# NealLiufighting/hpmpc

Hardware: AMD Instinct MI355X
Metric: Riccati factorisations/sec + IP iters/sec, fp64, N=100 nx=12 nu=4 batch=1024 (higher is better)
Workload: dtype f64

## Files before the change

### hpmpc_amd/build.py

```python
from __future__ import annotations

import os
import subprocess

ROOT = os.path.dirname(os.path.dirname(os.path.abspath(__file__)))
CSRC = os.path.join(ROOT, "hpmpc_amd", "csrc")
LIBDIR = os.path.join(ROOT, "hpmpc_amd", "lib")
HIPCC = os.environ.get("HIPCC", "/opt/rocm/bin/hipcc")
ARCH = os.environ.get("HPMPC_ARCH", "gfx950")
SOURCES = ["hpmpc_kernels.hip", "hk_wide.hip", "hk_wide_ipm.hip", "hk_soft.hip", "hk_soft_ipm.hip", "hk_ocp.hip", "hk_kkt.hip", "hpmpc_capi.cpp",
           "hpmpc_capi_queue.cpp", "hpmpc_capi_dropin.cpp", "hpmpc_capi_soft.cpp", "hpmpc_capi_soft_batch.cpp",
           "hpmpc_capi_wide.cpp", "hpmpc_capi_wide_ipm.cpp", "hpmpc_capi_iface.cpp", "hpmpc_capi_mpc.cpp",
           "hpmpc_capi_ocp.cpp", "hpmpc_capi_kkt.cpp"]
HEADERS = ["hpmpc_api.h", "hk_ipm_body.h", "hk_prims.h", "hk_riccati.h", "hk_ipm.h", "hk_mw.h", "hpmpc_kargs.h", "hk_wide_args.h", "hk_wide_core.h", "hk_wide_host.h", "hk_soft_args.h", "hk_soft_body.h", "hk_launch_guard.h", "hk_launch.h", "hk_host.h", "hk_plan.h", "hk_ocp_args.h", "hk_kkt_args.h", "hk_kkt_body.h"]
KFLAGS = ["-mllvm", "-amdgpu-mfma-vgpr-form"] + os.environ.get("HK_EXTRA_FLAGS", "").split()
SRC_FLAGS = {"hpmpc_kernels.hip": ["-mllvm", "-amdgpu-sched-strategy=max-memory-clause"],
             "hk_kkt.hip": ["-mllvm", "-amdgpu-sched-strategy=max-memory-clause"]}


EXPORTS = os.path.join(CSRC, "exports.map")


def _newer(out, deps):
    if not os.path.exists(out):
# ... 11 lines not shown
            text = open(path).read()
        except OSError:
            continue
        for name in re.findall(r'^\s*#\s*include\s+"([^"]+)"', text, re.M):
            for cand in (os.path.join(os.path.dirname(path), name), os.path.join(CSRC, name),
                         os.path.join(ROOT, "include", os.path.basename(name))):
                if os.path.exists(cand) and cand not in seen:
                    seen.add(cand)
                    todo.append(cand)
                    break
    return sorted(seen | {h for h in hdrs_all if os.path.basename(h) == "hpmpc_mi355x.h"})


def build_hip(force: bool = False, verbose: bool = False, variant: str | None = None, extra=(), sources=()) -> str:
    os.makedirs(LIBDIR, exist_ok=True)
    objdir = os.path.join(ROOT, "build", "obj" if variant is None else f"obj_{variant}")
    os.makedirs(objdir, exist_ok=True)
    out = os.path.join(LIBDIR, "libhpmpc_mi355x.so")
    if variant is not None:
        os.makedirs(os.path.join(LIBDIR, "ab"), exist_ok=True)
        out = os.path.join(LIBDIR, "ab", f"lib{variant}.so")
    hdrs_all = [os.path.join(CSRC, h) for h in HEADERS] + [os.path.join(ROOT, "include", "hpmpc_mi355x.h")]
    common = [HIPCC, f"--offload-arch={ARCH}", "-O3", "-std=c++17", "-fPIC", "-fvisibility=hidden", "-Wall",
              "-Wno-unused-function"] + KFLAGS + list(extra)
    objs, procs = [], []
    for src in SOURCES + list(sources):
        obj = os.path.join(objdir, src + ".o")
        objs.append(obj)
        if force or not _newer(obj, [os.path.join(CSRC, src)] + _deps(src, hdrs_all)):
            cmd = common + SRC_FLAGS.get(src, []) + ["-c", os.path.join(CSRC, src), "-o", obj]
            if verbose:
                print(" ".join(cmd), flush=True)
            procs.append((src, subprocess.Popen(cmd)))
    for src, pr in procs:
        if pr.wait() != 0:
            raise subprocess.CalledProcessError(pr.returncode, src)
    if procs or force or not _newer(out, objs + [EXPORTS]):
        cmd = [HIPCC, f"--offload-arch={ARCH}", "-shared", "-fPIC", f"-Wl,--version-script={EXPORTS}"] + objs + \
              ["-o", out]
        if verbose:
            print(" ".join(cmd), flush=True)
        subprocess.run(cmd, check=True)
    return out


def build_stamps(verbose: bool = False, force: bool = False) -> str:
    out = build_hip(force=force, verbose=verbose, variant="stamps", extra=["-DHK_STAMPS"])
    dst = os.path.join(LIBDIR, "libhpmpc_mi355x_stamps.so")
    if not _newer(dst, [out]):
        import shutil

        shutil.copy2(out, dst)
    return dst


def build_ric2(verbose: bool = False, force: bool = False) -> str:
    return build_hip(force=force, verbose=verbose, variant="ric2", extra=["-DHK_RIC2"], sources=["hk_ric2.hip"])


def build_calib(verbose: bool = False) -> str:
    os.makedirs(LIBDIR, exist_ok=True)
    out = os.path.join(LIBDIR, "libhbm_calib.so")
    src = os.path.join(ROOT, "tools", "hbm_calib.hip")
    if _newer(out, [src, os.path.join(CSRC, "hk_prims.h")]):
        return out
    cmd = [HIPCC, f"--offload-arch={ARCH}", "-O3", "-std=c++17", "-fPIC", "-shared", src, "-o", out]
    if verbose:
        print(" ".join(cmd), flush=True)
    subprocess.run(cmd, check=True)
    return out


def build_oracle(force: bool = False) -> None:
    odir = os.path.join(ROOT, "oracle")
    targets = ["oracle", "oracle_fma"]
    if os.path.isdir(os.environ.get("HPMPC_REF", "/root/reference")):
        targets += ["ref", "ref_avx"]
    subprocess.run(["make", "-s", "-C", odir] + (["-B"] if force else []) + targets, check=True)
    if "ref" in targets:
        subprocess.run(["make", "-s", "-C", os.path.join(ROOT, "tools", "relink"), "drivers"], check=True)


def build_all(force: bool = False, verbose: bool = False) -> None:
    build_hip(force=force, verbose=verbose)
    build_stamps(verbose=verbose, force=force)
    build_ric2(verbose=verbose, force=force)
    build_calib(verbose=verbose)
    build_oracle(force=force)


if __name__ == "__main__":
    build_all(force=True, verbose=True)
```

### hpmpc_amd/csrc/hk_ipm.h

```cpp
#pragma once
#include "hk_riccati.h"

namespace hk {

struct BoxTab {
    const signed char* tileslot;
    const signed char* slotvar;
};

#define HK_FOR_BOX(io, KV, ...)                                                       \
    for (int j4_ = 0; j4_ <= (io).N; j4_ += 4) {                                       \
        const int KV = j4_ + (lane_id() >> 4);                                         \
        const int slot = lane_id() & 15;                                               \
        if (KV <= (io).N) {                                                            \
            const int nb_ = (io).st[KV].nb, pnb_ = (io).st[KV].pnb;                    \
            if (slot < nb_) {                                                          \
                const int lo = KV * V32 + slot, up = KV * V32 + pnb_ + slot;           \
                (void)lo; (void)up;                                                    \
                __VA_ARGS__                                                            \
            }                                                                          \
        }                                                                              \
    }

#define HK_FOR_GEN(io, KV, ...)                                                       \
    for (int j4_ = 0; j4_ <= (io).N; j4_ += 4) {                                       \
        const int KV = j4_ + (lane_id() >> 4);                                         \
        const int gl_ = lane_id() & 15;                                                \
        if (KV <= (io).N) {                                                            \
            const int ng_ = (io).st[KV].ng, pnb_ = (io).st[KV].pnb;                    \
            if (gl_ < ng_) {                                                           \
                const int png_ = (ng_ + 3) & ~3;                                       \
                const int lo = KV * V32 + 2 * pnb_ + gl_, up = lo + png_;               \
                const int s16 = KV * V16 + pnb_ + gl_;                                 \
                (void)lo; (void)up; (void)s16;                                         \
                __VA_ARGS__                                                            \
            }                                                                          \
        }                                                                              \
    }

struct QuadLane {
    int lo, up;
    bool ok;
    bool box;
};

__device__ __forceinline__ QuadLane quad_lane(const RicIO& io, int q) {
    const int l = lane_id(), g = l >> 4, c = l & 15;
    const int k = 4 * q + g;
    const bool kv = k <= io.N;
    const int kc = kv ? k : io.N;
    const StageInfo& s = io.st[kc];
    QuadLane b;
    b.ok = kv && c < s.nb + s.ng;
    b.box = c < s.nb;
    const int png = (s.ng + 3) & ~3;
    b.lo = kc * V32 + (b.box ? c : 2 * s.pnb + (c - s.nb));
    b.up = b.lo + (b.box ? s.pnb : png);
    return b;
}

typedef __attribute__((address_space(3))) double lds_f64;

struct MwSplit {
    int w;
    lds_f64* red;
};

template <int NW>
__device__ __forceinline__ double mw_quad_sum(const MwSplit& ms, int nq_pad, double ms_local) {
    if constexpr (NW == 1) {
        return ms_local;
    } else {
        const int l = lane_id();
        __syncthreads();
        double m = 0.0;
        for (int q = 0; q < nq_pad; q++) m += ms.red[q * 64 + l];
        __syncthreads();
        return m;
    }
}

template <int CH>
__device__ double mu_aff_pass(const RicIO& io, const BoxCtx& bc, double alpha, double mu_scal) {
    const int nq = (io.N + 4) / 4;
    double ms = 0.0;
    for (int q0 = 0; q0 < nq; q0 += CH) {
        double v[CH][8];
#pragma unroll
        for (int j = 0; j < CH; j++) {
            const QuadLane b = quad_lane(io, q0 + j);
            v[j][0] = gld(bc.lam, b.lo, b.ok);
            v[j][1] = gld(bc.dlam, b.lo, b.ok);
            v[j][2] = gld(bc.t, b.lo, b.ok);
            v[j][3] = gld(bc.dt, b.lo, b.ok);
            v[j][4] = gld(bc.lam, b.up, b.ok);
            v[j][5] = gld(bc.dlam, b.up, b.ok);
            v[j][6] = gld(bc.t, b.up, b.ok);
            v[j][7] = gld(bc.dt, b.up, b.ok);
        }
#pragma unroll
        for (int j = 0; j < CH; j++)
            ms += (v[j][0] + alpha * v[j][1]) * (v[j][2] + alpha * v[j][3]) +
                  (v[j][4] + alpha * v[j][5]) * (v[j][6] + alpha * v[j][7]);
    }
    return wave_sum(ms) * mu_scal;
}

template <int CH, int NW = 1>
__device__ double update_p1_pass(const RicIO& io, const BoxCtx& bc, double alpha, double mu_scal, double* ux,
                                 double* pi, const double* dux, const double* dpi, double* ux_bkp, double* pi_bkp,
                                 double* lam_bkp, double* t_bkp, const MwSplit& mws = MwSplit{0, nullptr}) {
    const int l = lane_id(), g = l >> 4, c = l & 15;
    const int nq = (io.N + 4) / 4;
    double ms = 0.0;
    for (int q0 = NW > 1 ? mws.w * CH : 0; q0 < nq; q0 += NW * CH) {
        double v[CH][12];
        int i16[CH];
        bool oku[CH], okp[CH];
        QuadLane bl[CH];
#pragma unroll
        for (int j = 0; j < CH; j++) {
            const int k = 4 * (q0 + j) + g;
            const bool kv = k <= io.N;
            const StageInfo& s = io.st[kv ? k : io.N];
            i16[j] = (kv ? k : io.N) * V16 + c;
            oku[j] = kv && c < s.nu + s.nx;
            okp[j] = kv && k < io.N && c < s.nx1;
            bl[j] = quad_lane(io, q0 + j);
            const QuadLane& b = bl[j];
            v[j][0] = gld(ux, i16[j], oku[j]);
            v[j][1] = gld(dux, i16[j], oku[j]);
            v[j][2] = gld(pi, i16[j], okp[j]);
            v[j][3] = gld(dpi, i16[j], okp[j]);
            v[j][4] = gld(bc.lam, b.lo, b.ok);
            v[j][5] = gld(bc.dlam, b.lo, b.ok);
            v[j][6] = gld(bc.t, b.lo, b.ok);
            v[j][7] = gld(bc.dt, b.lo, b.ok);
            v[j][8] = gld(bc.lam, b.up, b.ok);
            v[j][9] = gld(bc.dlam, b.up, b.ok);
            v[j][10] = gld(bc.t, b.up, b.ok);
            v[j][11] = gld(bc.dt, b.up, b.ok);
        }
#pragma unroll
        for (int j = 0; j < CH; j++) {
            const QuadLane& b = bl[j];
            const double x = v[j][0], y = v[j][2];
            gst(ux_bkp, i16[j], x, oku[j]);
            gst(ux, i16[j], x + alpha * (v[j][1] - x), oku[j]);
            gst(pi_bkp, i16[j], y, okp[j]);
            gst(pi, i16[j], y + alpha * (v[j][3] - y), okp[j]);
            gst(lam_bkp, b.lo, v[j][4], b.ok);
            gst(lam_bkp, b.up, v[j][8], b.ok);
            gst(t_bkp, b.lo, v[j][6], b.ok);
            gst(t_bkp, b.up, v[j][10], b.ok);
            const double ll = v[j][4] + alpha * v[j][5], lu = v[j][8] + alpha * v[j][9];
            const double tl = v[j][6] + alpha * v[j][7], tu = v[j][10] + alpha * v[j][11];
            gst(bc.lam, b.lo, ll, b.ok);
            gst(bc.lam, b.up, lu, b.ok);
            gst(bc.t, b.lo, tl, b.ok);
            gst(bc.t, b.up, tu, b.ok);
            const double mc = b.ok ? ll * tl + lu * tu : 0.0;
            if constexpr (NW > 1)
                mws.red[(q0 + j) * 64 + l] = mc;
            else
                ms += mc;
        }
    }
    ms = mw_quad_sum<NW>(mws, (nq + CH - 1) / CH * CH, ms);
    return wave_sum(ms) * mu_scal;
}

template <int CH, bool UPD, bool BKP = true, int NW = 1>
__device__ double update_p2_pass(const RicIO& io, const BoxCtx& bc, const signed char* slotvar, double alpha,
                                 double mu_scal, double* ux, double* pi, const double* dux, const double* dpi,
                                 double* ux_bkp, double* pi_bkp, double* lam_bkp, double* t_bkp, double* res_d,
                                 double* res_m, const MwSplit& mws = MwSplit{0, nullptr}) {
    const int l = lane_id(), g = l >> 4, c = l & 15;
    const int nq = (io.N + 4) / 4;
    double ms = 0.0;
    for (int q0 = NW > 1 ? mws.w * CH : 0; q0 < nq; q0 += NW * CH) {
        double v[CH][16];
        int i16[CH], iv[CH];
        bool oku[CH], okp[CH];
        QuadLane bl[CH];
#pragma unroll
        for (int j = 0; j < CH; j++) {
            const int k = 4 * (q0 + j) + g;
            const bool kv = k <= io.N;
// ... 50 lines not shown
            }
            const double rml = ll * tl, rmu = lu * tu;
            gst(res_d, b.lo, v[j][14] - x + tl, b.ok && b.box);
            gst(res_d, b.up, v[j][15] - x - tu, b.ok && b.box);
            if (BKP) {
                gst(res_m, b.lo, rml, b.ok);
                gst(res_m, b.up, rmu, b.ok);
            }
            const double mc = b.ok ? rml + rmu : 0.0;
            if constexpr (NW > 1)
                mws.red[(q0 + j) * 64 + l] = mc;
            else
                ms += mc;
        }
    }
    ms = mw_quad_sum<NW>(mws, (nq + CH - 1) / CH * CH, ms);
    return wave_sum(ms) * mu_scal;
}

struct ResIO {
    const double *bsrc, *qsrc;
    double *ux, *pi;
    const double *dux, *dpi;
    double *ux_bkp, *pi_bkp;
    double *lam_bkp, *t_bkp;
    double *rq, *rb, *rd, *rm;
    double alpha;
};

template <bool UPD>
struct ResFrag {
    d4 Mi;
    double q;
    d4 bop;
    d4 bt;
    double bval;
    double uc, duc;
    double ur[4], dur[4];
    double pr[4], dpr[4];
    double pc, dpc;
    double x1, dx1;
    double bx[10];
    BoxLane bl;
};

template <bool UPD, class SH>
__device__ __forceinline__ void res_fetch(const RicIO& io, const SH& si, const BoxCtx& bc, const ResIO& ro, int k,
                                          ResFrag<UPD>& f) {
    const int l = lane_id(), g = l >> 4, c = l & 15;
    const int nu = si.nu, nx = si.nx, xo = si.xo, nux = nu + nx;
    const double* R = stage_R(io, si);
    const int vc = tile_var(c, nu, nx, xo);
    const bool live = SH::fixed || k < io.N;
#pragma unroll
    for (int r = 0; r < 4; r++) {
        const int vi = tile_var(g + 4 * r, nu, nx, xo);
        const int hi = vi > vc ? vi : vc, lo = vi > vc ? vc : vi;
        f.Mi[r] = ldsel(R, lib4_idx(si.sdR, hi, lo), vi >= 0 && vc >= 0);
        f.ur[r] = ldsel(ro.ux, k * V16 + vi, vi >= 0);
        f.dur[r] = UPD ? ldsel(ro.dux, k * V16 + vi, vi >= 0) : 0.0;
    }
    f.q = ro.qsrc ? ldsel(ro.qsrc, k * V16 + vc, vc >= 0) : ldsel(R, lib4_idx(si.sdR, nux, vc), vc >= 0);
    f.uc = ldsel(ro.ux, k * V16 + vc, vc >= 0);
    f.duc = UPD ? ldsel(ro.dux, k * V16 + vc, vc >= 0) : 0.0;
    const double* Bk = stage_B(io, si);
    const int nx1 = si.nx1, xo1 = si.xo1;
    const int s = c - xo1;
    const bool oks = live && s >= 0 && s < nx1;
#pragma unroll
    for (int r = 0; r < 4; r++) {
        const int sr = g + 4 * r - xo1;
        const bool okr = live && sr >= 0 && sr < nx1;
        const int vi = tile_var(g + 4 * r, nu, nx, xo);
        f.bop[r] = ldsel(Bk, lib4_idx(si.sdB, vc, sr), okr && vc >= 0);
        f.bt[r] = ldsel(Bk, lib4_idx(si.sdB, vi, s), oks && vi >= 0);
        f.pr[r] = ldsel(ro.pi, k * V16 + sr, okr);
        f.dpr[r] = UPD ? ldsel(ro.dpi, k * V16 + sr, okr) : 0.0;
    }
    f.bval = ro.bsrc ? ldsel(ro.bsrc, k * V16 + s, oks) : ldsel(Bk, lib4_idx(si.sdB, nux, s), oks);
    f.pc = ldsel(ro.pi, k * V16 + s, oks);
    f.dpc = UPD ? ldsel(ro.dpi, k * V16 + s, oks) : 0.0;
    f.x1 = ldsel(ro.ux, (k + 1) * V16 + si.nu1 + s, oks);
    f.dx1 = UPD ? ldsel(ro.dux, (k + 1) * V16 + si.nu1 + s, oks) : 0.0;
    const BoxLane b = box_lane(io.tileslot, si.pnb, k);
    f.bl = b;
    f.bx[0] = ldsel(bc.d, b.lo, b.ok);
    f.bx[1] = ldsel(bc.d, b.up, b.ok);
    f.bx[2] = ldsel(bc.lam, b.lo, b.ok);
    f.bx[3] = ldsel(bc.lam, b.up, b.ok);
    f.bx[4] = ldsel(bc.t, b.lo, b.ok);
    f.bx[5] = ldsel(bc.t, b.up, b.ok);
    f.bx[6] = UPD ? ldsel(bc.dlam, b.lo, b.ok) : 0.0;
    f.bx[7] = UPD ? ldsel(bc.dlam, b.up, b.ok) : 0.0;
    f.bx[8] = UPD ? ldsel(bc.dt, b.lo, b.ok) : 0.0;
    f.bx[9] = UPD ? ldsel(bc.dt, b.up, b.ok) : 0.0;
}

template <bool UPD, class SH>
__device__ __forceinline__ void res_step(const RicIO& io, const SH& sh, int k, const ResFrag<UPD>& cur,
                                         const BoxCtx& bc, const ResIO& ro, double& pim1, double& ms) {
    const int l = lane_id(), g = l >> 4, c = l & 15;
    const double al = ro.alpha;
    const bool live = SH::fixed || k < io.N;
    const int nu = sh.nu;
    const int vc = tile_var(c, sh.nu, sh.nx, sh.xo);
    const int s = c - sh.xo1;
    const bool oks = live && s >= 0 && s < sh.nx1;
    const double ucn = UPD ? cur.uc + al * cur.duc : cur.uc;
    double urn[4], prn[4];
#pragma unroll
    for (int r = 0; r < 4; r++) {
        urn[r] = UPD ? cur.ur[r] + al * cur.dur[r] : cur.ur[r];
        prn[r] = UPD ? cur.pr[r] + al * cur.dpr[r] : cur.pr[r];
    }
    const double pcn = UPD ? cur.pc + al * cur.dpc : cur.pc;
    const double x1n = UPD ? cur.x1 + al * cur.dx1 : cur.x1;
    const BoxLane& b = cur.bl;
    const double lml = UPD ? cur.bx[2] + al * cur.bx[6] : cur.bx[2];
    const double lmu = UPD ? cur.bx[3] + al * cur.bx[7] : cur.bx[3];
    const double tl = UPD ? cur.bx[4] + al * cur.bx[8] : cur.bx[4];
    const double tu = UPD ? cur.bx[5] + al * cur.bx[9] : cur.bx[5];
    const bool st0 = g == 0;
    if (UPD) {
        gst(ro.ux_bkp, k * V16 + vc, cur.uc, st0 && vc >= 0);
        gst(ro.ux, k * V16 + vc, ucn, st0 && vc >= 0);
        gst(ro.pi_bkp, k * V16 + s, cur.pc, st0 && oks);
        gst(ro.pi, k * V16 + s, pcn, st0 && oks);
        gst(ro.lam_bkp, b.lo, cur.bx[2], st0 && b.ok);
        gst(ro.lam_bkp, b.up, cur.bx[3], st0 && b.ok);
        gst(ro.t_bkp, b.lo, cur.bx[4], st0 && b.ok);
        gst(ro.t_bkp, b.up, cur.bx[5], st0 && b.ok);
        gst(bc.lam, b.lo, lml, st0 && b.ok);
        gst(bc.lam, b.up, lmu, st0 && b.ok);
        gst(bc.t, b.lo, tl, st0 && b.ok);
        gst(bc.t, b.up, tu, st0 && b.ok);
    }
    double h = cur.q;
    if (k > 0 && vc >= nu) h -= pim1;
    if (b.ok) h += -lml + lmu;
    double part = 0.0;
#pragma unroll
    for (int r = 0; r < 4; r++) part += cur.Mi[r] * urn[r];
    h += xrow_sum(part);
    double p2 = 0.0, p3 = 0.0;
#pragma unroll
    for (int r = 0; r < 4; r++) {
        p2 += cur.bop[r] * prn[r];
        p3 += cur.bt[r] * urn[r];
    }
    const double bpi = xrow_sum(p2);
    const double atu = xrow_sum(p3);
    if (live) h += bpi;
    gst(ro.rq, k * V16 + vc, h, st0 && vc >= 0);
    gst(ro.rb, k * V16 + s, cur.bval - x1n + atu, st0 && oks);
    const double x = ucn;
    const double rml = lml * tl, rmu = lmu * tu;
    gst(ro.rd, b.lo, cur.bx[0] - x + tl, st0 && b.ok);
    gst(ro.rd, b.up, cur.bx[1] - x - tu, st0 && b.ok);
    gst(ro.rm, b.lo, rml, st0 && b.ok);
    gst(ro.rm, b.up, rmu, st0 && b.ok);
    ms += (st0 && b.ok) ? rml + rmu : 0.0;
    if constexpr (!SH::fixed) {
        if (sh.ng > 0) {
            static_assert(!UPD || SH::fixed, "the update pass handles general slots element-wise");
            const double tq = gen_rq(io, sh, k, bc.lam);
            gst(ro.rq, k * V16 + vc, h + tq, st0 && vc >= 0);
            double dg[4];
            gen_dg(io, sh, dg);
#pragma unroll
            for (int lc = 0; lc < 4; lc++) {
                if (4 * lc >= sh.ng) continue;
                const GenLane q = gen_lane(k, sh.pnb, sh.ng, lc);
                const bool st = q.ok && c == 0;
                const double dx = row_sum16(dg[lc] * x);
                const double tgl = gld(bc.t, q.lo, q.ok), tgu = gld(bc.t, q.up, q.ok);
                const double lgl = gld(bc.lam, q.lo, q.ok), lgu = gld(bc.lam, q.up, q.ok);
                gst(ro.rd, q.lo, gld(bc.d, q.lo, q.ok) - dx + tgl, st);
                gst(ro.rd, q.up, gld(bc.d, q.up, q.ok) - dx - tgu, st);
                const double gml = lgl * tgl, gmu = lgu * tgu;
                gst(ro.rm, q.lo, gml, st);
                gst(ro.rm, q.up, gmu, st);
                ms += st ? gml + gmu : 0.0;
            }
        }
    }
    pim1 = pcn;
}

template <bool UPD, class FX>
__device__ bool residual_pass(const RicIO& io, const BoxCtx& bc, const ResIO& ro, double& mu_out) {
    double ms = 0.0, pim1 = 0.0;
    int nbt = 0;
    ResFrag<UPD> cur, nxt;
    {
        const StageRef s0{io.st, 0};
        with_shape<FX>(s0, [&](const auto& sh) { res_fetch<UPD>(io, sh, bc, ro, 0, cur); });
    }
    for (int k = 0; k <= io.N; k++) {
        const int kn = k < io.N ? k + 1 : io.N;
        const StageRef sn{io.st, kn};
        with_shape<FX>(sn, [&](const auto& sh) { res_fetch<UPD>(io, sh, bc, ro, kn, nxt); });
        asm volatile("" ::: "memory");
        const StageRef si{io.st, k};
        nbt += srd(si, &StageInfo::nb) + srd(si, &StageInfo::ng);
        with_shape<FX>(si, [&](const auto& sh) { res_step<UPD>(io, sh, k, cur, bc, ro, pim1, ms); });
        cur = nxt;
    }
    ms = wave_sum(ms);
    if (nbt != 0) {
        mu_out = ms / (2.0 * nbt);
        return true;
    }
    return false;
}

}
```

### hpmpc_amd/csrc/hk_ipm_body.h

```cpp
#pragma once
#include "hk_ipm.h"
#include "hk_launch_guard.h"
#include "hpmpc_kargs.h"

using namespace hk;

#ifndef HK_WAVES
#define HK_WAVES 2
#endif
#define HK_TWO_WAVES __attribute__((amdgpu_waves_per_eu(HK_WAVES)))

namespace {

struct Ws {
    double *F, *dux, *dpi, *Pb, *Qx, *qx, *res_q, *res_b, *ux_bkp, *pi_bkp;
    double *dlam, *dt, *t_inv, *lamt, *res_d, *res_m, *t_bkp, *lam_bkp;
    double* state;
    double* cert;
};

enum { S_MU = 0, S_ALPHA, S_SIGMA, S_SMU, S_KK, S_PHASE, S_ACTIVE, S_MUSCAL, S_RET };

__device__ __forceinline__ Ws carve(double* W, int N) {
    Ws w;
    const long n1 = N + 1, a = n1 * V16, b = n1 * V32;
    w.F = W;
    W += n1 * FSTRIDE;
    w.dux = W;
    w.dpi = W + a;
    w.Pb = W + 2 * a;
    w.Qx = W + 3 * a;
    w.qx = W + 4 * a;
    w.res_q = W + 5 * a;
    w.res_b = W + 6 * a;
    w.ux_bkp = W + 7 * a;
    w.pi_bkp = W + 8 * a;
    W += 9 * a;
    w.dlam = W;
    w.dt = W + b;
    w.t_inv = W + 2 * b;
    w.lamt = W + 3 * b;
    w.res_d = W + 4 * b;
    w.res_m = W + 5 * b;
    w.t_bkp = W + 6 * b;
    w.lam_bkp = W + 7 * b;
    w.state = W + 8 * b;
    w.cert = w.state + 16;
    return w;
}

extern __shared__ __attribute__((aligned(16))) char hk_smem[];

struct LdsTabs {
    Scratch* sm;
    const StageInfo* st;
    const signed char* tileslot;
    const signed char* slotvar;
    double* gc;
};

__device__ __forceinline__ LdsTabs lds_tables(const KArgs& a) {
    LdsTabs T;
    T.sm = reinterpret_cast<Scratch*>(hk_smem);
    StageInfo* st = reinterpret_cast<StageInfo*>(hk_smem + sizeof(Scratch));
    signed char* ts = reinterpret_cast<signed char*>(st + (a.N + 1));
    signed char* sv = ts + (a.N + 1) * 16;
    const int l = lane_id(), n1 = a.N + 1;
    const int* gst = reinterpret_cast<const int*>(a.st);
    int* lst = reinterpret_cast<int*>(st);
    for (int i = l; i < n1 * 16; i += 64) lst[i] = gst[i];
    const int* gts = reinterpret_cast<const int*>(a.tileslot);
    const int* gsv = reinterpret_cast<const int*>(a.slotvar);
    int* lts = reinterpret_cast<int*>(ts);
    int* lsv = reinterpret_cast<int*>(sv);
    for (int i = l; i < n1 * 4; i += 64) {
        lts[i] = gts[i];
        lsv[i] = gsv[i];
    }
    __syncthreads();
    T.st = st;
    T.tileslot = ts;
    T.slotvar = sv;
    T.gc = reinterpret_cast<double*>(sv + n1 * 16);
    return T;
}

__device__ __forceinline__ RicIO make_io(const KArgs& a, const LdsTabs& T, int p, double* F) {
    RicIO io;
    io.N = a.N;
    io.st = T.st;
    io.tileslot = T.tileslot;
    io.BAbt = a.BAbt + (long)p * a.sB;
    io.RSQ = a.RSQ + (long)p * a.sR;
    io.BAbtS = a.BAbt;
    io.RSQS = a.RSQ;
    io.F = F;
    io.DCt = a.DCt ? a.DCt + (long)p * a.sG : a.RSQ;
    return io;
}

__device__ __forceinline__ void wsync() { __syncthreads(); }

}

namespace {

template <int CH>
__device__ void init_var(const RicIO& io, const double* dv, double* ux, double* pi, double* dpi, double* lam,
                         double* t, double mu0, int warm_start) {
    const int l = lane_id(), g = l >> 4, c = l & 15;
    const double thr0 = 0.1;
    const int nq = (io.N + 4) / 4;
    for (int q0 = 0; q0 < nq; q0 += CH) {
        double dl[CH], du[CH], xv[CH];
        int lo[CH], up[CH], iv[CH];
        bool kv[CH], bx[CH], kp[CH];
#pragma unroll
        for (int j = 0; j < CH; j++) {
            const int k = 4 * (q0 + j) + g;
            kv[j] = k <= io.N;
            kp[j] = k < io.N;
            const int kc = kv[j] ? k : io.N;
            const StageInfo& si = io.st[kc];
            const bool okv = c < si.nu + si.nx;
            const int tile = c < si.nu ? c : si.xo + (c - si.nu);
            const int slot = okv ? io.tileslot[kc * 16 + (okv ? tile : 0)] : -1;
            bx[j] = kv[j] && slot >= 0;
            lo[j] = kc * V32 + (slot >= 0 ? slot : 0);
            up[j] = lo[j] + si.pnb;
            iv[j] = kc * V16 + c;
            dl[j] = gld(dv, lo[j], bx[j]);
            du[j] = gld(dv, up[j], bx[j]);
            xv[j] = warm_start ? gld(ux, iv[j], kv[j]) : 0.0;
        }
#pragma unroll
        for (int j = 0; j < CH; j++) {
            double x = xv[j];
            double tl = -dl[j] + x, tu = du[j] - x;
            if (tl < thr0) {
                if (tu < thr0) {
                    x = (-du[j] + dl[j]) * 0.5;
                    tl = thr0;
                    tu = thr0;
                } else {
                    tl = thr0;
                    x = dl[j] + thr0;
                }
            } else if (tu < thr0) {
                tu = thr0;
                x = du[j] - thr0;
            }
            x = bx[j] ? x : xv[j];
            gst(ux, iv[j], x, kv[j]);
            gst(pi, iv[j], 0.0, kp[j]);
            gst(dpi, iv[j], 0.0, kv[j]);
            gst(t, lo[j], tl, bx[j]);
            gst(t, up[j], tu, bx[j]);
            gst(lam, lo[j], mu0 / tl, bx[j]);
            gst(lam, up[j], mu0 / tu, bx[j]);
        }
    }
}

__device__ void init_var_gen(const RicIO& io, const double* dv, const double* ux, double* lam, double* t,
                             double mu0) {
    const int l = lane_id(), c = l & 15;
    const double thr0 = 0.1;
    for (int k = 0; k <= io.N; k++) {
        const StageInfo si = load_stage(io.st, k);
        if (si.ng == 0) continue;
        const DynSh sh(si);
        const int vc = tile_var(c, sh.nu, sh.nx, sh.xo);
        const double x = gld(ux, k * V16 + vc, vc >= 0);
        double dg[4];
        gen_dg(io, sh, dg);
#pragma unroll
        for (int lc = 0; lc < 4; lc++) {
            if (4 * lc >= sh.ng) continue;
            const GenLane q = gen_lane(k, sh.pnb, sh.ng, lc);
            const bool st = q.ok && c == 0;
            const double dx = row_sum16(dg[lc] * x);
            const double tl = fmax(thr0, dx + (-gld(dv, q.lo, q.ok)));
            const double tu = fmax(thr0, -dx + gld(dv, q.up, q.ok));
            gst(t, q.lo, tl, st);
            gst(t, q.up, tu, st);
            gst(lam, q.lo, mu0 / tl, st);
            gst(lam, q.up, mu0 / tu, st);
        }
    }
}

__device__ __forceinline__ BoxCtx box_ctx(const Ws& w, const double* dv, double* lam, double* t) {
    BoxCtx bc{};
    bc.d = dv;
    bc.lam = lam;
    bc.t = t;
    bc.dlam = w.dlam;
    bc.dt = w.dt;
    bc.t_inv = w.t_inv;
    bc.lamt = w.lamt;
    bc.res_d = w.res_d;
    bc.res_m = w.res_m;
    bc.qxs = w.qx;
    bc.Qx = w.Qx;
    bc.qx = w.qx;
    bc.cert = w.cert;
    bc.cert_out = w.cert;
    bc.cert_new = 0;
    bc.res_q = w.res_q;
    bc.res_b = w.res_b;
    return bc;
}

}

namespace {

struct IpmView {
    int N, q, l;
    Ws w;
    RicIO io;
    BoxTab bt;
    double *ux, *pi, *lam, *t, *stat;
    const double* dv;
    BoxCtx bc;
};

__device__ __forceinline__ int* qcount(const KArgs& a, int p) { return a.qctl + 2 + a.nslots + p; }
__device__ __forceinline__ int* qlist(const KArgs& a, int p) { return a.qctl + 4 + a.nslots + p * a.nslots; }
__device__ __forceinline__ void qlist_push(const KArgs& a, int p, int s) {
    if (lane_id() == 0) qlist(a, p)[atomicAdd(qcount(a, p), 1)] = s;
}

struct Who {
    int s, q, d;
};

__device__ __forceinline__ bool who_am_i(const KArgs& a, Who& w) {
    if (a.nq == 0) {
        const int p = blockIdx.x + a.p0;
        w.s = w.q = w.d = p;
        return p < a.nprob;
    }
    const int n = __builtin_amdgcn_readfirstlane(*qcount(a, a.qpar));
    if ((int)blockIdx.x >= n) return false;
    w.s = __builtin_amdgcn_readfirstlane(qlist(a, a.qpar)[blockIdx.x]);
    w.q = __builtin_amdgcn_readfirstlane(a.qctl[2 + w.s]);
    w.d = w.q >= 0 ? w.q % a.nprob : 0;
    return w.q >= 0;
}

__device__ __forceinline__ bool slot_active(const KArgs& a, const Who& who) {
    return carve(a.ws + (long)who.s * a.sW, a.N).state[S_ACTIVE] != 0.0;
}

__device__ __forceinline__ IpmView ipm_view(const KArgs& a, const LdsTabs& T, const Who& who) {
    IpmView v;
    v.N = a.N;
    v.q = who.q;
    v.l = lane_id();
    v.w = carve(a.ws + (long)who.s * a.sW, a.N);
    v.io = make_io(a, T, who.d, v.w.F);
    v.bt = BoxTab{T.tileslot, T.slotvar};
    const long o16 = (long)who.q * a.sV16, o32 = (long)who.q * a.sV32;
    v.ux = a.ux + o16;
    v.pi = a.pi + o16;
    v.lam = a.lam + o32;
    v.t = a.t + o32;
    v.dv = a.d + (long)who.d * a.sV32;
    v.stat = a.stat + (long)who.q * 5 * a.k_max;
    v.bc = box_ctx(v.w, v.dv, v.lam, v.t);
    v.bc.ux = v.ux;
    v.bc.pi = v.pi;
    return v;
}

__device__ __forceinline__ ResIO res_io(const IpmView& v) {
    ResIO ro{};
    ro.ux = v.ux;
    ro.pi = v.pi;
    ro.dux = v.w.dux;
    ro.dpi = v.w.dpi;
    ro.ux_bkp = v.w.ux_bkp;
    ro.pi_bkp = v.w.pi_bkp;
    ro.lam_bkp = v.w.lam_bkp;
    ro.t_bkp = v.w.t_bkp;
    ro.rq = v.w.res_q;
    ro.rb = v.w.res_b;
    ro.rd = v.w.res_d;
    ro.rm = v.w.res_m;
    return ro;
}

template <class FX, int CI, int NW = 1>
__device__ double p2_start(const KArgs& a, IpmView& v, const MwSplit& mws = MwSplit{0, nullptr}) {
    const double mu = update_p2_pass<CI, false, true, NW>(v.io, v.bc, v.bt.slotvar, 0.0, 1.0 / (2.0 * a.nbt), v.ux,
                                                          v.pi, nullptr, nullptr, nullptr, nullptr, nullptr, nullptr,
                                                          v.w.res_d, v.w.res_m, mws);
    wsync();
    return mu;
}

template <class FX, int CI, int NW = 1>
__device__ bool ipm_continue(const KArgs& a, IpmView& v, int kk, double mu, double alpha, double sigma, int phase,
                             const MwSplit& mws = MwSplit{0, nullptr}) {
    const bool sn = a.single_newton != 0;
    bool active;
    if (a.phase1_only) {
        active = kk < a.k_max && mu > a.mu_tol && alpha >= a.alpha_min;
    } else {
        if (phase == 1) {
            const double mu_tol_low = a.mu_tol < 1e-5 ? 1e-5 : a.mu_tol;
            if (!(kk < a.k_max && mu > mu_tol_low && alpha >= a.alpha_min)) {
                mu = p2_start<FX, CI, NW>(a, v, mws);
                phase = 2;
            }
        }
        active = phase == 1;
        if (phase == 2) active = kk < a.k_max && (sn || (mu > a.mu_tol && alpha >= a.alpha_min));
    }
    int ret = 0;
    if (!active) {
        if (!sn && mu <= a.mu_tol)
            ret = 0;
        else if (kk >= a.k_max)
            ret = 1;
        else if (alpha < a.alpha_min)
            ret = 2;
        else
            ret = -1;
    }
    if (v.l == 0) {
        double* st = v.w.state;
        st[S_MU] = mu;
        st[S_ALPHA] = alpha;
        st[S_SIGMA] = sigma;
        st[S_KK] = kk;
        st[S_PHASE] = phase;
        st[S_ACTIVE] = active ? 1.0 : 0.0;
        if (!active) {
            a.kk[v.q] = kk;
            a.ret[v.q] = ret;
        }
    }
    return active;
}

template <class FX, int CI, bool SHORTCUT>
__device__ bool ipm_start(const KArgs& a, const LdsTabs& T, IpmView& v) {
    Scratch& sm = *T.sm;
    const int N = v.N, l = v.l;
    const int nbt = a.nbt;
    if (!SHORTCUT && nbt == 0) return false;
    if (SHORTCUT && nbt == 0 && a.phase1_only) {
        ric_backward<true, BX_NONE, FX>(v.io, &sm, 0, nullptr, 0, nullptr, v.bc, 1, v.w.Pb);
        wsync();
        ric_forward_sv<FX>(v.io, &sm, 0, nullptr, v.w.dux, a.compute_mult, v.w.dpi);
        if (l == 0) {
            v.w.state[S_ACTIVE] = 0.0;
            a.kk[v.q] = 0;
            a.ret[v.q] = 0;
        }
        return false;
    }
    if (SHORTCUT && nbt == 0) {
        ric_backward<true, BX_NONE, FX>(v.io, &sm, 0, nullptr, 0, nullptr, v.bc, 1, v.w.Pb);
        wsync();
        ric_forward_sv<FX>(v.io, &sm, 0, nullptr, v.ux, a.compute_mult, v.pi);
        wsync();
        for (int i = l; i < (N + 1) * V16; i += 64) {
            v.w.ux_bkp[i] = v.ux[i];
            v.w.pi_bkp[i] = v.pi[i];
        }
        if (l == 0) {
            v.w.state[S_ACTIVE] = 0.0;
            a.kk[v.q] = 0;
            a.ret[v.q] = 0;
        }
        return false;
    }
    const bool sn = a.single_newton != 0;
    if (!sn) {
        init_var<CI>(v.io, v.dv, v.ux, v.pi, v.w.dpi, v.lam, v.t, a.mu0, a.warm_start);
        if (a.ngt) {
            wsync();
            init_var_gen(v.io, v.dv, v.ux, v.lam, v.t, a.mu0);
        }
    } else {
        for (int i = l; i < (N + 1) * V16; i += 64) v.w.dpi[i] = 0.0;
    }
    if (l == 0) v.w.state[S_MUSCAL] = 1.0 / (2.0 * nbt);
    wsync();
    double mu = a.mu0;
    if (sn) mu = p2_start<FX, CI>(a, v);
    return ipm_continue<FX, CI>(a, v, 0, mu, 1.0, 0.0, sn ? 2 : 1);
}

template <class FX, int CI, bool SHORTCUT>
__device__ bool ipm_refill(const KArgs& a, const LdsTabs& T, int s) {
    const bool l0 = lane_id() == 0;
    for (;;) {
        int q = 0;
        if (l0) q = atomicAdd(a.qnext, 1);
        q = __builtin_amdgcn_readfirstlane(q);
        if (q >= a.nq) {
            if (l0) a.qctl[2 + s] = -1;
            return false;
        }
        if (l0) a.qctl[2 + s] = q;
        const Who who{s, q, q % a.nprob};
        IpmView v = ipm_view(a, T, who);
        if (ipm_start<FX, CI, SHORTCUT>(a, T, v)) return true;
        if (l0) atomicAdd(&a.qctl[1], 1);
    }
}

}

namespace {

template <class FX>
__device__ __forceinline__ void fact_body(const KArgs& a, const LdsTabs& T, IpmView& v) {
    Scratch& sm = *T.sm;
    const double* st = v.w.state;
    const bool sn = a.single_newton != 0;
    const bool first = st[S_KK] == 0.0;
    if (first && st[S_PHASE] != 1.0) {
        cert_pass(v.io, v.w.cert);
        wsync();
    }
    if (!first || st[S_PHASE] != 1.0)
        for (int i = v.l; i <= v.N; i += 64) T.gc[i] = v.w.cert[i];
    wsync();
    v.bc.cert = T.gc;
    if (st[S_PHASE] == 1.0) {
        if (first)
            ric_backward<true, BX_P1, FX, CERT_FORM>(v.io, &sm, 0, nullptr, 0, nullptr, v.bc, 1, v.w.Pb);
        else
            ric_backward<true, BX_P1, FX, CERT_LOAD>(v.io, &sm, 0, nullptr, 0, nullptr, v.bc, 1, v.w.Pb);
    } else {
        v.bc.res_rhs = !sn;
        v.bc.no_tinv = a.no_bkp;
        ric_backward<true, BX_P2R, FX, CERT_LOAD>(v.io, &sm, 0, nullptr, 0, nullptr, v.bc, 1, v.w.Pb);
    }
}

template <class FX>
__device__ __forceinline__ void pred_body(const KArgs& a, const LdsTabs& T, IpmView& v) {
    Scratch& sm = *T.sm;
    double* st = v.w.state;
    const bool sn = a.single_newton != 0;
    const int phase = (int)st[S_PHASE], kk = (int)st[S_KK];
    const double mu = st[S_MU];
    double sigma = st[S_SIGMA];
    double al = 1.0;
    if (phase == 1) {
        v.bc.pred = 1;
        ric_forward<0, BX_P1, FX, true>(v.io, &sm, nullptr, 0, v.w.dux, 0, v.w.dpi, v.bc, al);
    } else {
        ric_forward<0, BX_P2, FX, true>(v.io, &sm, v.w.res_b, !sn, v.w.dux, 0, v.w.dpi, v.bc, al);
    }
    al = wave_min(al);
    wsync();
    const double alpha = al * 0.995;
    const double mu_aff = mu_aff_pass<7>(v.io, v.bc, alpha, st[S_MUSCAL]);
    double smu = a.mu0;
    if (!sn) {
        sigma = mu_aff / mu;
        sigma = sigma * sigma * sigma;
        smu = sigma * mu;
    }
    if (v.l == 0) {
        v.stat[5 * kk] = st[S_SIGMA];
        v.stat[5 * kk + 1] = al;
        v.stat[5 * kk + 2] = mu_aff;
        st[S_SIGMA] = sigma;
        st[S_SMU] = smu;
    }
}

template <class FX>
__device__ __forceinline__ void corr_body(const KArgs& a, const LdsTabs& T, IpmView& v) {
    Scratch& sm = *T.sm;
    double* st = v.w.state;
    const int phase = (int)st[S_PHASE], kk = (int)st[S_KK];
    v.bc.smu = st[S_SMU];
    double al = 1.0;
    if (phase == 1)
        ric_trs<BX_P1, BX_P1, FX, false>(v.io, &sm, nullptr, nullptr, v.bc, v.w.dux, a.compute_mult, v.w.dpi, 0, v.w.Pb,
                                         al);
    else
        ric_trs<BX_P2, BX_P2, FX, false>(v.io, &sm, v.w.res_b, v.w.res_q, v.bc, v.w.dux, a.compute_mult, v.w.dpi, 0,
                                         v.w.Pb, al);
    al = wave_min(al);
    if (v.l == 0) {
        v.stat[5 * kk] = st[S_SIGMA];
        v.stat[5 * kk + 3] = al;
        st[S_ALPHA] = al * 0.995;
    }
}

template <class FX, int CI>
__device__ __forceinline__ bool update_body(const KArgs& a, IpmView& v) {
    double* st = v.w.state;
    const int phase = (int)st[S_PHASE];
    int kk = (int)st[S_KK];
    const double alpha = st[S_ALPHA];
    double mu;
    if (phase == 1) {
        mu = update_p1_pass<CI>(v.io, v.bc, alpha, st[S_MUSCAL], v.ux, v.pi, v.w.dux, v.w.dpi, v.w.ux_bkp,
                                v.w.pi_bkp, v.w.lam_bkp, v.w.t_bkp);
    } else {
        if (a.no_bkp)
            mu = update_p2_pass<CI, true, false>(v.io, v.bc, v.bt.slotvar, alpha, st[S_MUSCAL], v.ux, v.pi, v.w.dux,
                                                 v.w.dpi, v.w.ux_bkp, v.w.pi_bkp, v.w.lam_bkp, v.w.t_bkp, v.w.res_d,
                                                 v.w.res_m);
        else
            mu = update_p2_pass<CI, true>(v.io, v.bc, v.bt.slotvar, alpha, st[S_MUSCAL], v.ux, v.pi, v.w.dux, v.w.dpi,
                                          v.w.ux_bkp, v.w.pi_bkp, v.w.lam_bkp, v.w.t_bkp, v.w.res_d, v.w.res_m);
    }
    wsync();
    if (v.l == 0) v.stat[5 * kk + 4] = mu;
    kk++;
    return ipm_continue<FX, CI>(a, v, kk, mu, alpha, st[S_SIGMA], phase);
}

}
```

### hpmpc_amd/csrc/hk_kkt_body.h

```cpp
#pragma once
#include "hk_ipm_body.h"

namespace {

struct KktIO {
    const double *vb, *vq;
    long o16;
    const double* d;
    double *ux, *pi, *lam, *t;
};

template <class FX, bool NULLABLE>
__device__ __forceinline__ void kkt_body(const KArgs& a, const RicIO& io, Scratch* sm, const BoxTab& bt, const Ws& w,
                                         const KktIO& v) {
    const int N = a.N;
    double* ux = v.ux;
    double* pi = v.pi;
    double* lam = v.lam;
    double* t = v.t;
    const int l = lane_id();
    BoxCtx bc = box_ctx(w, v.d, lam, t);
    for (int i = l; i < (N + 1) * V16; i += 64) {
        ux[i] = w.ux_bkp[i];
        pi[i] = w.pi_bkp[i];
    }
    for (int i = l; i < (N + 1) * V32; i += 64) {
        t[i] = w.t_bkp[i];
        lam[i] = w.lam_bkp[i];
    }
    wsync();
    double mu = 0.0;
    ResIO ro{};
    ro.bsrc = v.vb + v.o16;
    ro.qsrc = v.vq + v.o16;
    if constexpr (NULLABLE) {
        if (!v.vb) ro.bsrc = nullptr;
        if (!v.vq) ro.qsrc = nullptr;
    }
    ro.ux = ux;
    ro.pi = pi;
    ro.rq = w.res_q;
    ro.rb = w.res_b;
    ro.rd = w.res_d;
    ro.rm = w.res_m;
    residual_pass<false, FX>(io, bc, ro, mu);
    wsync();
    HK_FOR_BOX(io, k, {
        w.qx[k * V16 + slot] = w.t_inv[lo] * (w.res_m[lo] - lam[lo] * w.res_d[lo]) -
                               w.t_inv[up] * (w.res_m[up] + lam[up] * w.res_d[up]);
    });
    HK_FOR_GEN(io, k, {
        w.qx[s16] = w.t_inv[lo] * (w.res_m[lo] - lam[lo] * w.res_d[lo]) -
                    w.t_inv[up] * (w.res_m[up] + lam[up] * w.res_d[up]);
    });
    wsync();
    double al = 1.0;
    ric_trs<BX_GIVEN, BX_NONE, FX>(io, sm, w.res_b, w.res_q, bc, w.dux, a.compute_mult, w.dpi, 1, w.Pb, al);
    wsync();
    HK_FOR_BOX(io, k, {
        const int vi = bt.slotvar[k * 16 + slot];
        const double x = w.dux[k * V16 + vi];
        const double dtl = x - w.res_d[lo], dtu = -x + w.res_d[up];
        const double dll = -w.t_inv[lo] * (lam[lo] * dtl + w.res_m[lo]);
        const double dlu = -w.t_inv[up] * (lam[up] * dtu + w.res_m[up]);
        w.dt[lo] = dtl;
        w.dt[up] = dtu;
        w.dlam[lo] = dll;
        w.dlam[up] = dlu;
    });
    if (a.ngt) {
        for (int k = 0; k <= N; k++) {
            const StageInfo si = load_stage(io.st, k);
            if (si.ng == 0) continue;
            const DynSh sh(si);
            const int vc = tile_var(l & 15, sh.nu, sh.nx, sh.xo);
            double dummy = 1.0;
            gen_alpha<BX_P2>(io, sh, k, bc, gld(w.dux, k * V16 + vc, vc >= 0), dummy);
        }
    }
    wsync();
    for (int k = 0; k <= N; k++) {
        const StageInfo si = load_stage(io.st, k);
        if (l < si.nu + si.nx) ux[k * V16 + l] += 1.0 * w.dux[k * V16 + l];
        if (k < N && l < si.nx1) pi[k * V16 + l] += 1.0 * w.dpi[k * V16 + l];
    }
    HK_FOR_BOX(io, k, {
        lam[lo] += 1.0 * w.dlam[lo];
        lam[up] += 1.0 * w.dlam[up];
        t[lo] += 1.0 * w.dt[lo];
        t[up] += 1.0 * w.dt[up];
    });
    HK_FOR_GEN(io, k, {
        lam[lo] += 1.0 * w.dlam[lo];
        lam[up] += 1.0 * w.dlam[up];
        t[lo] += 1.0 * w.dt[lo];
        t[up] += 1.0 * w.dt[up];
    });
}

}
```

### hpmpc_amd/csrc/hk_mw.h

```cpp
#pragma once
#include "hk_ipm.h"

namespace hk {

constexpr int MW_WAVES = 4, MW_HELP = 3;
constexpr int MW_D = 6;
constexpr int MW_SLOT = 16;
constexpr int MW_DP = 6;
constexpr int MW_NMAX = 300;
constexpr int MW_RED = ((MW_NMAX + 4) / 4 + 3) / 4 * 4;
constexpr int HK_MW_ERR = -20;

struct MwShared {
    double ring[MW_D][MW_SLOT][64];
    double red[MW_RED][64];
    Scratch sm[MW_WAVES];
    double al[MW_WAVES];
    int full[MW_D], freed[MW_D];
    int freedB[MW_D];
    double ringP[MW_DP][10][64];
    int fullP[MW_DP], freedP[MW_DP];
    int xfacP[MW_DP];
    int err;
    int dbg[4];
// ... 337 lines not shown
        double part = 0.0;
        if (!all) {
#pragma unroll
            for (int r = 0; r < 4; r++) part += (g + 4 * r >= sh.xo) ? lowS(cur.S, r, g, c) * xrow[r] : 0.0;
        }
        const double rc = -rhs - xrow_sum(part);
        double rrow[4];
        col2row(sm, rc, rrow);
#pragma unroll
        for (int r = 0; r < 4; r++) ur[r] = all ? 0.0 : xrow[r];
        solve_lt(sh, cur.S, cur.invd, rrow, ur, all);
    }
    ucol = row2col(sm, ur);
    double gp = 0.0;
#pragma unroll
    for (int r = 0; r < 4; r++) gp += cur.bt[r] * ur[r];
    const int s = c - sh.xo1;
    const bool ok = s >= 0 && s < sh.nx1;
    const double x1 = cur.bval + xrow_sum(gp);
    xcol = ok ? x1 : 0.0;
}

template <int MODE, int FM, class FX, bool PRED = false>
__device__ __forceinline__ int ric_forward_mw(const RicIO& io, int tb, int w, const double* bsrc, int use_bsrc,
                               double* ux, int compute_pi_, double* pi, const BoxCtx& bc, double& al_out) {
    const int N = io.N, l = lane_id(), g = l >> 4, c = l & 15;
    const int compute_pi = PRED ? 0 : compute_pi_;
    Scratch* sm = &hk_mw.sm[w];
    double al = 1.0;
    if (w == 0) {
        double xcol = 0.0;
        FwdFrag f0, f1, f2;
        fwd_fetch_chain_k<MODE, FX>(io, 0, bsrc, use_bsrc, ux, compute_pi, f0);
        fwd_fetch_chain_k<MODE, FX>(io, 1 <= N ? 1 : N, bsrc, use_bsrc, ux, compute_pi, f1);
        auto stage = [&](int k, const FwdFrag& fa, const FwdFrag& fb, FwdFrag& fc) __attribute__((always_inline)) {
            fwd_fetch_chain_k<MODE, FX>(io, k + 2 <= N ? k + 2 : N, bsrc, use_bsrc, ux, compute_pi, fc);
            const StageInfo si = load_stage(io.st, k);
            double ucol = 0.0, p1 = 0.0;
            with_shape<FX>(si, [&](const auto& sh) {
                fwd_chain<MODE>(sm, sh, k, fa, xcol, ucol);
                if (MODE == 1) {
                    const int s = c - sh.xo1;
                    const bool ok = s >= 0 && s < sh.nx1;
                    p1 = std::remove_reference_t<decltype(sh)>::fixed ? (ok ? fb.hc : 0.0) : fa.pk;
                }
            });
            mw_acquire(tb, k);
            mw_put(k, 0, ucol);
            mw_put(k, 1, xcol);
            mw_put(k, 2, p1);
            mw_post(k % MW_D, tb + k + 1);
        };
        for (int k = 0;;) {
            if (k >= N) break;
            stage(k, f0, f1, f2);
            if (++k >= N) break;
            stage(k, f1, f2, f0);
            if (++k >= N) break;
            stage(k, f2, f0, f1);
            ++k;
        }
        mw_acquire(tb, N);
        mw_put(N, 0, xcol);
        mw_put(N, 1, 0.0);
        mw_put(N, 2, 0.0);
        mw_post(N % MW_D, tb + N + 1);
    } else {
        auto fetch = [&](int k, FwdFrag& fc, FwdFrag& fn) __attribute__((always_inline)) {
            fwd_fetch_k<MODE, FM, FX, PRED>(io, k, bsrc, use_bsrc, ux, 0, bc, fc);
            if (compute_pi && k < N) fwd_fetch_k<MODE, FM, FX, PRED>(io, k + 1, bsrc, use_bsrc, ux, compute_pi, bc, fn);
        };
        auto work = [&](int k, const FwdFrag& fc, const FwdFrag& fn) __attribute__((always_inline)) {
            mw_wait(k % MW_D, tb + k + 1);
            const double ucol = mw_get(k, 0), x1 = mw_get(k, 1), p1 = mw_get(k, 2);
            mw_post(MW_D + k % MW_D, tb + k + 1);
            if (k < N) {
                const StageInfo si = load_stage(io.st, k);
                with_shape<FX>(si, [&](const auto& sh) {
                    using SHT = std::remove_reference_t<decltype(sh)>;
                    const int vcs = tile_var(c, sh.nu, sh.nx, sh.xo);
                    if (!PRED) gst(ux, k * V16 + vcs, ucol, g == 0 && vcs >= 0);
                    box_alpha<FM, PRED>(bc, fc, ucol, al);
                    if constexpr (!SHT::fixed && FM != BX_NONE) {
                        if (sh.ng > 0) gen_alpha<FM>(io, sh, k, bc, ucol, al);
                    }
                    const int s = c - sh.xo1;
                    const bool ok = s >= 0 && s < sh.nx1;
                    double pv = 0.0;
                    if (compute_pi) {
                        double x1row[4];
                        col2row(sm, x1, x1row);
                        pv = pi_from_x(fn.S, sh.xo1, x1row, MODE == 0 ? fn.lc : p1);
                    }
                    gst(pi, k * V16 + s, pv, compute_pi && g == 0 && ok);
                });
            } else {
                const StageInfo sN = load_stage(io.st, N);
                const int v = tile_var(c, sN.nu, sN.nx, sN.xo);
                if (!PRED) gst(ux, N * V16 + v, ucol, g == 0 && v >= 0);
                box_alpha<FM, PRED>(bc, fc, ucol, al);
                if (FM != BX_NONE && sN.ng > 0) gen_alpha<FM>(io, DynSh(sN), N, bc, ucol, al);
            }
        };
        FwdFrag ca, na, cb, nb;
        int k = w - 1;
        if (k <= N) fetch(k, ca, na);
        for (;;) {
            if (k > N) break;
            if (k + MW_HELP <= N) fetch(k + MW_HELP, cb, nb);
            work(k, ca, na);
            k += MW_HELP;
            if (k > N) break;
            if (k + MW_HELP <= N) fetch(k + MW_HELP, ca, na);
            work(k, cb, nb);
            k += MW_HELP;
        }
    }
    al = wave_min(al);
    if (l == 0) hk_mw.al[w] = al;
    __syncthreads();
    al_out = fmin(fmin(hk_mw.al[0], hk_mw.al[1]), fmin(hk_mw.al[2], hk_mw.al[3]));
    return tb + N + 2;
}

template <int TM, int FM, class FX>
__device__ __forceinline__ int ric_trs_mw(const RicIO& io, int tb, int w, const double* hb, const double* hq,
                           const BoxCtx& bc, double* ux, int compute_pi, double* pi, double* Pb, double& al) {
    const int N = io.N, l = lane_id(), g = l >> 4, c = l & 15;
    Scratch* sm = &hk_mw.sm[w];
    if (w > 0) {
        auto fetch = [&](int j, TrsFrag& f) __attribute__((always_inline)) {
            const int k = N - j;
            const StageInfo si = load_stage(io.st, k);
            with_shape<FX>(si, [&](const auto& sh) { trs_fetch<TM, false>(io, sh, k, hb, hq, bc, 0, Pb, f); });
        };
        auto work = [&](int j, const TrsFrag& f) __attribute__((always_inline)) {
            const int k = N - j;
            const StageInfo si = load_stage(io.st, k);
            double hpre = 0.0;
            with_shape<FX>(si, [&](const auto& sh) {
                using SHT = std::remove_reference_t<decltype(sh)>;
                hpre = f.h0 + box_gradient<TM>(bc, f);
                if constexpr (!SHT::fixed) {
                    if (sh.ng > 0) hpre += gen_gradient<TM>(io, sh, k, bc);
                }
            });
            mw_acquire(tb, j);
            mw_put(j, 0, hpre);
#pragma unroll
            for (int r = 0; r < 4; r++) {
                mw_put(j, 1 + r, f.bop[r]);
                mw_put(j, 5 + r, f.S[r]);
            }
            mw_put(j, 9, f.invd);
            mw_put(j, 10, f.pbc);
            mw_post(j % MW_D, tb + j + 1);
        };
        TrsFrag fa, fb;
        int j = w - 1;
        if (j <= N) fetch(j, fa);
        for (;;) {
            if (j > N) break;
            if (j + MW_HELP <= N) fetch(j + MW_HELP, fb);
            work(j, fa);
            j += MW_HELP;
            if (j > N) break;
            if (j + MW_HELP <= N) fetch(j + MW_HELP, fa);
            work(j, fb);
            j += MW_HELP;
        }
    } else {
        double pcol = 0.0;
        double hn, invdn, pbcn;
        d4 bopn, Sn;
        auto take = [&](int j) __attribute__((always_inline)) {
            mw_wait(j % MW_D, tb + j + 1);
            hn = mw_get(j, 0);
#pragma unroll
            for (int r = 0; r < 4; r++) {
                bopn[r] = mw_get(j, 1 + r);
                Sn[r] = mw_get(j, 5 + r);
            }
            invdn = mw_get(j, 9);
            pbcn = mw_get(j, 10);
// ... 44 lines not shown
```

### hpmpc_amd/csrc/hk_plan.h

```cpp
#pragma once
#include <mutex>
#include <vector>

#include "hk_host.h"
#include "hk_soft_args.h"
#include "hpmpc_kargs.h"

struct StageInfoH {
    int nu, nx, nb, ng, xo, nx1, nu1, xo1, sdB, sdR, oB, oR, oD, pnb, r0, oG;
};

struct hpmpc_mi355x_plan {
    int N = 0;
    std::vector<int> nx, nu, nb, ng;
    std::vector<std::vector<int>> idxb;
    std::vector<StageInfoH> st;
    std::vector<signed char> tileslot, slotvar;
    std::vector<long long> offB, offR;
    long long packB = 0, packR = 0;
    void* d_st = nullptr;
    signed char *d_tileslot = nullptr, *d_slotvar = nullptr;
    struct LayoutTable {
        std::vector<StageInfoH> st;
        void* d = nullptr;
    };
    std::vector<LayoutTable> ltabs;
    std::mutex ltabs_mu;
    int fixcls = 0;
    int nbt = 0;
    int ngt = 0;
    std::vector<long long> offG;
    long long packG = 0;
};

inline long long ws_doubles(int N) {
    const long long n = (long long)(N + 1) * (FSTRIDE + 9 * V16 + 8 * V32 + 1) + 16;
    return (n + 31) / 32 * 32;
}

bool plan_supported(int N, const int* nx, const int* nu, const int* nb, const int* const* idxb, const int* ng,
                    const char** why);
KArgs base_args(const hpmpc_mi355x_plan* P, int nprob, int p0);
bool layout_apply(hpmpc_mi355x_plan* P, const hpmpc_mi355x_layout* lay, KArgs& a);
bool layout_set(hpmpc_mi355x_plan* P, const hpmpc_mi355x_layout* lay, KArgs& a);
int launch(int which, const KArgs* a, int count, hipStream_t s);
int ipm_run(KArgs& a, int count, const double* BAbt, const double* RSQrq, const double* d, double* ux, double* pi,
            double* lam, double* t, double* ws, int k_max, double mu0, double mu_tol, double alpha_min, int warm_start,
            int compute_mult, int* kk, int* ret, double* stat, int which, void* stream);
hpmpc_mi355x_plan* thread_plan(int N, const int* nx, const int* nu, const int* nb, int** idxb, const int* ng);

struct Arena {
    size_t BAbt, RSQ, DCt, d, ux, pi, lam, t, ws, vb, vq, vQx, vqx, vPb, stat, ints, qctl, total;
};
Arena arena(const hpmpc_mi355x_plan* P, int k_max);
KArgs arena_args(const hpmpc_mi355x_plan* P, const Arena& A, double* dev);
void stage_BAbt(const hpmpc_mi355x_plan* P, double* H, const Arena& A, double** hpBAbt);
void stage_RSQ(const hpmpc_mi355x_plan* P, double* H, const Arena& A, double** hpQ);
bool run(int which, const KArgs& a, const char* name);
enum VecKind { VEC_UX, VEC_PI, VEC_CV };
void vec_in(const hpmpc_mi355x_plan* P, VecKind kind, double* H, size_t off, double** v);
void vec_out(const hpmpc_mi355x_plan* P, VecKind kind, double** v, const double* H, size_t off);

struct SoftLayout {
    std::vector<SoftStage> st;
    long sC = 0, sD = 0, sZ = 0;
    long sF = 0;
};
const char* soft_unsupported(int N, const int* nx, const int* nu, const int* ng);
const char* soft_layout(int N, const int* nx, const int* nu, const int* nb, const int* ns, SoftLayout& L);
```

### hpmpc_amd/csrc/hk_ric2.hip

```cpp
#include "hk_mw.h"
#include "hk_launch.h"
#include "hk_launch_guard.h"
#include "hpmpc_kargs.h"

using namespace hk;

namespace {

constexpr int R2_D = 3;
constexpr int R2_ROWS = 10;
constexpr int R2_DP = 2;
constexpr int R2_PROWS = 10;
constexpr int R2_H = 6;

struct R2Shared {
    union {
        double mring[R2_D][R2_ROWS][64];
        double fring[2 * R2_H][2][64];
    };
    double pring[R2_DP][R2_PROWS][64];
    Scratch sm[2];
    double mgc[R2_D];
    int xfac[R2_DP];
};
// ... 251 lines not shown
        auto stage = [&](int k, const FwdFrag& fa, FwdFrag& fc) __attribute__((always_inline)) {
            fwd_fetch_chain_k<0, FX>(io, k + 2 <= N ? k + 2 : N, bsrc, update_b, ux, compute_pi, fc);
            const double xk = xcol;
            double ucol = 0.0;
            with_shape<FX>(StageRef{io.st, k}, [&](const auto& sh) { fwd_chain<0>(sm, sh, k, fa, xcol, ucol); });
            put(k, ucol, xk);
        };
        R2_T0(tp);
        int k = 0, r = 0;
        for (int b = 0; b <= nblk; b++) {
            const int kend = (b + 1) * R2_H < N + 1 ? (b + 1) * R2_H : N + 1;
            for (; k < kend; k++) {
                if (k == N) {
                    put(N, xcol, xcol);
                } else if (r == 0) {
                    stage(k, f0, f2);
                } else if (r == 1) {
                    stage(k, f1, f0);
                } else {
                    stage(k, f2, f1);
                }
                r = r == 2 ? 0 : r + 1;
            }
            R2_STEP_BAR(tp, 5);
        }
    } else {
        Scratch* sm = &r2.sm[1];
        struct PiFrag {
            d4 S;
            double lc;
        };
        auto fetch = [&](int k, PiFrag& f) __attribute__((always_inline)) {
            const double* Fk = io.F + (long)k * FSTRIDE;
            with_shape<FX>(StageRef{io.st, k < N ? k : N - 1}, [&](const auto& sh) {
                using SHT = std::remove_reference_t<decltype(sh)>;
                if constexpr (SHT::fixed) {
                    f.S[0] = 0.0;
                    load_p_fixed<SHT::nx>(Fk, f.S, compute_pi && k > 0);
                    f.lc = gld(Fk, FXR_L + c);
                } else {
#pragma unroll
                    for (int r = 0; r < 4; r++) f.S[r] = gld(Fk, r * 64 + l, compute_pi && k > 0);
                    f.lc = gld(Fk, 256 + c);
                }
            });
        };
        auto work = [&](int k, const PiFrag& f) __attribute__((always_inline)) {
            const int s = k % (2 * R2_H);
            const double ucol = r2.fring[s][0][l], xk = r2.fring[s][1][l];
            const DynSh sk(StageRef{io.st, k});
            if (compute_pi && k > 0) {
                double xrow[4];
                col2row(sm, xk, xrow);
                fwd_pi<0>(sk.xo, sk.nx, k, f.S, xrow, f.lc, compute_pi, pi);
            }
            const int v = tile_var(c, sk.nu, sk.nx, sk.xo);
            gst(ux, k * V16 + v, k < N ? ucol : xk, g == 0 && v >= 0);
        };
        R2_T0(tp);
        PiFrag fa, fb;
        fetch(0, fa);
        int k = 0;
        bool alt = false;
        for (int b = 0; b <= nblk; b++) {
            const int kend = b * R2_H < N + 1 ? b * R2_H : N + 1;
            for (; k < kend; k++) {
                if (!alt) {
                    if (k + 1 <= N) fetch(k + 1, fb);
                    work(k, fa);
                } else {
                    if (k + 1 <= N) fetch(k + 1, fa);
                    work(k, fb);
                }
                alt = !alt;
            }
            R2_STEP_BAR(tp, 7);
        }
    }
}

__device__ __forceinline__ RicIO r2_io(const KArgs& a, const R2Tabs& T, int p) {
    RicIO io;
    io.N = a.N;
    io.st = T.st;
    io.tileslot = T.tileslot;
    io.BAbt = a.BAbt + (long)p * a.sB;
    io.RSQ = a.RSQ + (long)p * a.sR;
    io.BAbtS = a.BAbt;
    io.RSQS = a.RSQ;
    io.F = a.ws + (long)p * a.sW;
    io.DCt = a.DCt ? a.DCt + (long)p * a.sG : a.RSQ;
    return io;
}

}

template <class FX>
__global__ __launch_bounds__(128) __attribute__((amdgpu_waves_per_eu(2))) void hk_ric_sv2(KArgs a) {
    const R2Tabs T = r2_tables(a);
    const int p = blockIdx.x + a.p0;
    if (p >= a.nprob) return;
    const int w = threadIdx.x >> 6;
    const RicIO io = r2_io(a, T, p);
    const long o16 = (long)p * a.sV16;
    const double* b = a.vb ? a.vb + o16 : nullptr;
    const double* q = a.vq ? a.vq + o16 : nullptr;
    BoxCtx bc{};
    bc.Qx = a.vQx ? a.vQx + o16 : nullptr;
    bc.qx = a.vqx ? a.vqx + o16 : nullptr;
    double* Pb = a.vPb ? a.vPb + o16 : nullptr;
    if (a.use_box)
        ric_backward2<BX_GIVEN, FX>(io, w, a.update_b, b, a.update_q, q, bc, a.compute_Pb, Pb);
    else
        ric_backward2<BX_NONE, FX>(io, w, a.update_b, b, a.update_q, q, bc, a.compute_Pb, Pb);
    __syncthreads();
    ric_forward2<FX>(io, w, a.update_b, b, a.ux + o16, a.compute_pi, a.pi + o16);
}

template <class FX>
static int launch2_t(const KArgs* a, int count, hipStream_t stream) {
#ifdef HK_STAMPS
    (void)hipMemcpyToSymbol(HIP_SYMBOL(r2_dbg), &a->dbg, sizeof(a->dbg));
#endif
    static const HkKernelLimits lim(reinterpret_cast<const void*>(&hk_ric_sv2<FX>));
    const size_t lds = r2_lds_bytes(a->N);
    if (lim.check(lds, 128) != 0) return HK_LAUNCH_REFUSED;
    hipLaunchKernelGGL(hk_ric_sv2<FX>, dim3(count), dim3(128), lds, stream, *a);
    return (int)hipGetLastError();
}

extern "C" int hk_launch_ric2(int which, const KArgs* a, int count, hipStream_t stream) {
    if (count <= 0) return 0;
    if (which != K_SV) return HK_LAUNCH_REFUSED;
    switch (a->fixcls) {
        case 1: return launch2_t<FixSh<4, 12>>(a, count, stream);
        case 2: return launch2_t<FixSh<3, 8>>(a, count, stream);
        default: return launch2_t<NoFix>(a, count, stream);
    }
}
```

### hpmpc_amd/csrc/hk_riccati.h

```cpp
#pragma once

#include "hk_prims.h"
#include "hpmpc_kargs.h"

namespace hk {

struct StageInfo {
    int nu, nx, nb, ng;
    int xo;
    int nx1, nu1, xo1;
    int sdB, sdR;
    int oB, oR, oD;
    int pnb;
    int r0;
    int oG;
};

using ::FSTRIDE;
using ::V16;
using ::V32;

__device__ __forceinline__ bool tile_active(int t, int nu, int nx, int xo) {
    return t < nu || (t >= xo && t < xo + nx);
}
// ... 291 lines not shown

__device__ __forceinline__ void xblocks_chol_row(const d4& L, double invd, double& ml, int nx, int xo) {
    const int hi = xo + nx;
    if (0 >= xo && 0 < hi) chol_block_row<0, true, false>(L, invd, ml, nullptr);
    if (4 >= xo && 4 < hi) chol_block_row<1, true, false>(L, invd, ml, nullptr);
    if (8 >= xo && 8 < hi) chol_block_row<2, true, false>(L, invd, ml, nullptr);
    if (12 >= xo && 12 < hi) chol_block_row<3, true, false>(L, invd, ml, nullptr);
}

struct XFac {
    d4 L;
    double invd;
};

template <bool AUG, bool KGEN = false>
__device__ __forceinline__ void stage_chol(d4& M, double& ml, double& invd, int nu, int nx, int xo, bool full,
                                           bool transpose, double* kg = nullptr, int kdbg = -1, bool xfac = false,
                                           XFac* xf = nullptr) {
    const int l = lane_id(), g = l >> 4, c = l & 15;
    (void)kdbg;
    invd = 0.0;
    const int hi = full ? xo + nx : nu;
    if (0 < nu || (full && 3 >= xo && 0 < hi)) chol_block<0, AUG, KGEN>(M, ml, invd, kg, kdbg);
    HK_STAMP(16, kdbg);
    if (4 < nu || (full && 7 >= xo && 4 < hi)) chol_block<1, AUG>(M, ml, invd, nullptr, kdbg);
    HK_STAMP(18, kdbg);
    if (8 < nu || (full && 11 >= xo && 8 < hi)) chol_block<2, AUG>(M, ml, invd, nullptr, kdbg);
    HK_STAMP(20, kdbg);
    if (12 < nu || (full && 15 >= xo && 12 < hi)) chol_block<3, AUG>(M, ml, invd, nullptr, kdbg);
    HK_STAMP(22, kdbg);
    const bool xf_now = xfac;
#ifdef HK_COUNT_NOFALLBACK
    asm volatile("" ::"s"(__builtin_amdgcn_readfirstlane((int)xf_now)));
    if (false) {
#else
    if (!full && xf_now) {
#endif
        d4 L = M;
        double lx = ml, ivx = invd;
        xblocks_chol<AUG>(L, lx, ivx, nx, xo);
        pform_eff_tile(L, nx, xo, M);
        if (AUG) pform_eff_row(L, lx, nx, xo, ml);
        if (xf) {
            xf->L = L;
            xf->invd = ivx;
        }
    }
    if (!transpose) return;
    const d4 z = {0.0, 0.0, 0.0, 0.0};
    d4 T0 = mfma(M[0], (c == g) ? 1.0 : 0.0, z);
    d4 T1 = mfma(M[1], (c == 4 + g) ? 1.0 : 0.0, z);
    T0 = mfma(M[2], (c == 8 + g) ? 1.0 : 0.0, T0);
    T1 = mfma(M[3], (c == 12 + g) ? 1.0 : 0.0, T1);
    const d4 T = T0 + T1;
#pragma unroll
    for (int r = 0; r < 4; r++) M[r] = (g + 4 * r > c) ? T[r] : M[r];
}

template <class SH>
__device__ __forceinline__ double cert_g_shift(const d4& Mi, const SH& sh) {
    const int l = lane_id(), g = l >> 4, c = l & 15;
    const bool act = tile_active(c, sh.nu, sh.nx, sh.xo);
    const double dm = -wave_min((diag_lane() && act) ? -diag_sel(Mi) : 0.0);
    const double tau = dm * 0x1p-10;
    d4 A = Mi;
#pragma unroll
    for (int r = 0; r < 4; r++) A[r] -= (g + 4 * r == c && act) ? tau : 0.0;
    double ml = 0.0, invd = 0.0;
    stage_chol<false, false>(A, ml, invd, sh.nu, sh.nx, sh.xo, true, false);
    const bool ok = dm > 0.0 && __builtin_amdgcn_ballot_w64(act && !(invd > 0.0)) == 0;
    return ok ? tau - 1e-12 * dm : -1.0;
}

template <class SH>
__device__ __forceinline__ double cert_g(const d4& Mi, const SH& sh) {
    const double g = cert_g_gersh(Mi, sh);
#ifdef HK_COUNT_NOSHIFT
    return g;
#endif
    if (g > 0.0) return g;
    return cert_g_shift(Mi, sh);
}

struct RicIO {
    int N;
    const StageInfo* st;
    const signed char* tileslot;
    const double* BAbt;
    const double* RSQ;
    const double* BAbtS;
    const double* RSQS;
    double* F;
    const double* DCt;
};

__device__ __forceinline__ StageInfo load_stage(const StageInfo* st, int k) {
    const StageInfo v = st[k];
    StageInfo u;
    u.nu = __builtin_amdgcn_readfirstlane(v.nu);
    u.nx = __builtin_amdgcn_readfirstlane(v.nx);
    u.nb = __builtin_amdgcn_readfirstlane(v.nb);
    u.ng = __builtin_amdgcn_readfirstlane(v.ng);
    u.xo = __builtin_amdgcn_readfirstlane(v.xo);
    u.nx1 = __builtin_amdgcn_readfirstlane(v.nx1);
    u.nu1 = __builtin_amdgcn_readfirstlane(v.nu1);
    u.xo1 = __builtin_amdgcn_readfirstlane(v.xo1);
    u.sdB = __builtin_amdgcn_readfirstlane(v.sdB);
    u.sdR = __builtin_amdgcn_readfirstlane(v.sdR);
    u.oB = __builtin_amdgcn_readfirstlane(v.oB);
    u.oR = __builtin_amdgcn_readfirstlane(v.oR);
    u.oD = __builtin_amdgcn_readfirstlane(v.oD);
    u.pnb = __builtin_amdgcn_readfirstlane(v.pnb);
    u.r0 = __builtin_amdgcn_readfirstlane(v.r0);
    u.oG = __builtin_amdgcn_readfirstlane(v.oG);
    return u;
}

struct StageRef {
    const StageInfo* p;
    int k;
};
__device__ __forceinline__ int srd(const StageRef& s, int StageInfo::*m) {
    return __builtin_amdgcn_readfirstlane(s.p[s.k].*m);
}

struct DynSh {
    static constexpr bool fixed = false;
    int nu, nx, xo, nx1, nu1, xo1, sdB, sdR, nb, pnb, oB, oR, ng, oG, fl;
    __device__ __forceinline__ explicit DynSh(const StageInfo& s)
        : nu(s.nu), nx(s.nx), xo(s.xo), nx1(s.nx1), nu1(s.nu1), xo1(s.xo1), sdB(s.sdB), sdR(s.sdR), nb(s.nb),
          pnb(s.pnb), oB(s.oB), oR(s.oR), ng(s.ng), oG(s.oG), fl(s.r0) {}
    __device__ __forceinline__ explicit DynSh(const StageRef& s)
        : nu(srd(s, &StageInfo::nu)), nx(srd(s, &StageInfo::nx)), xo(srd(s, &StageInfo::xo)),
          nx1(srd(s, &StageInfo::nx1)), nu1(srd(s, &StageInfo::nu1)), xo1(srd(s, &StageInfo::xo1)),
          sdB(srd(s, &StageInfo::sdB)), sdR(srd(s, &StageInfo::sdR)), nb(srd(s, &StageInfo::nb)),
          pnb(srd(s, &StageInfo::pnb)), oB(srd(s, &StageInfo::oB)), oR(srd(s, &StageInfo::oR)),
          ng(srd(s, &StageInfo::ng)), oG(srd(s, &StageInfo::oG)), fl(srd(s, &StageInfo::r0)) {}
};

template <int NU, int NX>
struct FixSh {
    static constexpr bool fixed = true, enabled = true;
    static constexpr int nu = NU, nx = NX, xo = (NU + 3) / 4 * 4, nx1 = NX, nu1 = NU, xo1 = xo,
                         sdB = (NX + 1) / 2 * 2, sdR = (NU + NX + 1) / 2 * 2;
    int nb, pnb, oB, oR, fl;
    __device__ __forceinline__ explicit FixSh(const StageInfo& s)
        : nb(s.nb), pnb(s.pnb), oB(s.oB), oR(s.oR), fl(s.r0) {}
    __device__ __forceinline__ explicit FixSh(const StageRef& s)
        : nb(srd(s, &StageInfo::nb)), pnb(srd(s, &StageInfo::pnb)), oB(srd(s, &StageInfo::oB)),
          oR(srd(s, &StageInfo::oR)), fl(srd(s, &StageInfo::r0)) {}
};


__device__ __forceinline__ int stage_flags(const StageInfo& s) { return s.r0; }
template <class SH>
__device__ __forceinline__ int stage_flags(const SH& s) { return s.fl; }
template <class SH>
__device__ __forceinline__ const double* stage_B(const RicIO& io, const SH& sh) {
    return ((stage_flags(sh) & 2) ? io.BAbtS : io.BAbt) + sh.oB;
}
template <class SH>
__device__ __forceinline__ const double* stage_R(const RicIO& io, const SH& sh) {
    return ((stage_flags(sh) & 4) ? io.RSQS : io.RSQ) + sh.oR;
}

struct NoFix {
    static constexpr bool enabled = false;
    __device__ __forceinline__ explicit NoFix(const StageInfo&) {}
// ... 25 lines not shown
        }
    }
    f(DynSh(s));
}

__device__ __forceinline__ double lowS(const d4& S, int r, int g, int c) { return (g + 4 * r >= c) ? S[r] : 0.0; }

__device__ __forceinline__ void load_factor(const double* Fk, d4& S, double& lc, double& invd) {
    const int l = lane_id(), c = l & 15;
#pragma unroll
    for (int r = 0; r < 4; r++) S[r] = Fk[r * 64 + l];
    lc = Fk[256 + c];
    invd = Fk[272 + c];
}

__device__ __forceinline__ void store_factor(double* Fk, const d4& S, double lc, double invd, double kg,
                                             bool ok = true) {
    const int l = lane_id(), g = l >> 4, c = l & 15;
#pragma unroll
    for (int r = 0; r < 4; r++) gst(Fk, r * 64 + l, S[r], ok);
    gst(Fk, 256 + 16 * g + c, g == 0 ? lc : invd, ok && g < 2);
    gst(Fk, 288 + l, kg, ok);
}

constexpr int FXR_L = 64, FXR_INVD = 80, FXR_KG = 96, FXR_P = 160;

__device__ __forceinline__ int fxr_pidx(int i, int j) {
    const int a = i > j ? i : j, b = i > j ? j : i;
    return FXR_P + (a * (a + 1) >> 1) + b;
}

template <int NX>
__device__ __forceinline__ void store_factor_fixed(double* Fk, const d4& S, double lc, double invd, double kg,
                                                   bool ok) {
    const int l = lane_id(), g = l >> 4, c = l & 15;
    gst(Fk, l, S[0], false);
    gst(Fk, FXR_L + 16 * g + c, g == 0 ? lc : invd, ok && g < 2);
    gst(Fk, FXR_KG + l, kg, ok);
    const int j = c - 4;
#pragma unroll
    for (int r = 1; r < 4; r++) {
        const int i = g + 4 * r - 4;
        gst(Fk, fxr_pidx(i, j), S[r], ok && j >= 0 && j <= i && i < NX);
    }
}

template <int NX>
__device__ __forceinline__ void load_p_fixed(const double* Fk, d4& S, bool ok) {
    const int l = lane_id(), g = l >> 4, c = l & 15;
    const int j = c - 4;
#pragma unroll
    for (int r = 1; r < 4; r++) {
        const int i = g + 4 * r - 4;
        S[r] = gld(Fk, fxr_pidx(i, j), ok && j >= 0 && i < NX && j < NX);
    }
}

enum BoxMode { BX_NONE = 0, BX_GIVEN = 1, BX_P1 = 2, BX_P2 = 3, BX_P2R = 4 };

constexpr bool cert_loaded(int bm) { return bm == BX_P1 || bm == BX_P2 || bm == BX_P2R; }

struct BoxCtx {
    const double* d;
    double *lam, *t;
    double *dlam, *dt, *t_inv, *lamt, *res_d, *res_m;
    double* qxs;
    const double *Qx, *qx;
    double smu;
    int pred;
    const double *ux, *pi;
    double *res_q, *res_b;
    int res_rhs;
    int no_tinv;
    const double* cert;
    double* cert_out;
    int cert_new;
};

struct BoxLane {
    int lo, up, s16;
    bool ok;
};

__device__ __forceinline__ BoxLane box_lane(const signed char* tileslot, int pnb, int k) {
    const int c = lane_id() & 15;
    const int slot = tileslot[k * 16 + c];
    BoxLane b;
    b.ok = slot >= 0;
    b.lo = k * V32 + slot;
    b.up = b.lo + pnb;
    b.s16 = k * V16 + slot;
    return b;
}

__device__ __forceinline__ void ld_lu(const double* p, const BoxLane& b, double& vlo, double& vup) {
    const bool odd = (lane_id() & 16) != 0;
    const int m = -(int)odd;
    const double x = gld(p, (b.up & m) | (b.lo & ~m), b.ok);
    const int xl = __double2loint(x), xh = __double2hiint(x);
    const auto cl = __builtin_amdgcn_permlane16_swap(xl, xl, false, false);
    const auto ch = __builtin_amdgcn_permlane16_swap(xh, xh, false, false);
    vlo = mk((int)ch[0], (int)cl[0]);
    vup = mk((int)ch[1], (int)cl[1]);
}

__device__ __forceinline__ void fetch_pair(const double* p, const BoxLane& b, double& e0, double& e1) {
    e0 = gld(p, b.lo, b.ok);
    e1 = gld(p, b.up, b.ok);
}
__device__ __forceinline__ void use_pair(double e0, double e1, double& vlo, double& vup) {
    vlo = e0;
    vup = e1;
}

__device__ __forceinline__ void st_lu(double* p, const BoxLane& b, double vlo, double vup, bool ok) {
    const bool odd = (lane_id() & 16) != 0;
    const int m = -(int)odd;
    gst(p, (b.up & m) | (b.lo & ~m), odd ? vup : vlo, ok && lane_id() < 32);
}

__device__ __forceinline__ void alpha_rule(double& al, double v, double dv) {
    const double cand = -v * rcp_nr(dv);
    al = (-al * dv > v) ? cand : al;
}


struct GenLane {
    int lo, up, s16;
    bool ok;
};

__device__ __forceinline__ GenLane gen_lane(int k, int pnb, int ng, int lc) {
    const int gl = 4 * lc + (lane_id() >> 4);
    const int png = (ng + 3) & ~3;
    GenLane q;
    q.ok = gl < ng;
    q.lo = k * V32 + 2 * pnb + gl;
    q.up = q.lo + png;
    q.s16 = k * V16 + pnb + gl;
    return q;
}

__device__ __forceinline__ void gen_dg(const RicIO& io, const DynSh& sh, double dg[4]) {
    const int l = lane_id(), g = l >> 4, c = l & 15;
    const int vc = tile_var(c, sh.nu, sh.nx, sh.xo);
    const int cng = (sh.ng + 1) & ~1;
    const double* D = io.DCt + sh.oG;
#pragma unroll
    for (int lc = 0; lc < 4; lc++) {
        const int gl = 4 * lc + g;
        dg[lc] = (4 * lc < sh.ng) ? gld(D, lib4_idx(cng, vc, gl), vc >= 0 && gl < sh.ng) : 0.0;
    }
}

template <int BM>
__device__ void gen_hessian(const RicIO& io, const DynSh& sh, int k, const BoxCtx& bc, double x, d4& M, double& ml,
                            bool aug) {
    const int c = lane_id() & 15;
    double dg[4];
    gen_dg(io, sh, dg);
    double part = 0.0;
#pragma unroll
    for (int lc = 0; lc < 4; lc++) {
        if (4 * lc >= sh.ng) continue;
        const GenLane q = gen_lane(k, sh.pnb, sh.ng, lc);
        const bool st = q.ok && c == 0;
        double Q = 0.0, qv = 0.0;
        if (BM == BX_GIVEN) {
            Q = gld(bc.Qx, q.s16, q.ok);
            qv = aug ? gld(bc.qx, q.s16, q.ok) : 0.0;
        } else if (BM == BX_P1) {
            const double lml = gld(bc.lam, q.lo, q.ok), lmu = gld(bc.lam, q.up, q.ok);
            const double tl = gld(bc.t, q.lo, q.ok), tu = gld(bc.t, q.up, q.ok);
            const double dl = gld(bc.d, q.lo, q.ok), du = gld(bc.d, q.up, q.ok);
            const double til = rcp_nr(tl), tiu = rcp_nr(tu);
            const double ltl = lml * til, ltu = lmu * tiu;
            const double dll = til * 0.0, dlu = tiu * 0.0;
            qv = lmu - ltu * du + dlu - lml - ltl * dl - dll;
            Q = ltl + ltu;
            gst(bc.t_inv, q.lo, til, st);
            gst(bc.t_inv, q.up, tiu, st);
            gst(bc.lamt, q.lo, ltl, st);
            gst(bc.lamt, q.up, ltu, st);
            gst(bc.qxs, q.s16, qv, st);
        } else if (BM == BX_P2 || BM == BX_P2R) {
            const double lml = gld(bc.lam, q.lo, q.ok), lmu = gld(bc.lam, q.up, q.ok);
            const double tl = gld(bc.t, q.lo, q.ok), tu = gld(bc.t, q.up, q.ok);
            const double rml = gld(bc.res_m, q.lo, q.ok), rmu = gld(bc.res_m, q.up, q.ok);
            double rdl, rdu;
            if (BM == BX_P2R) {
                const double dx = row_sum16(dg[lc] * x);
                rdl = gld(bc.d, q.lo, q.ok) - dx + tl;
                rdu = gld(bc.d, q.up, q.ok) - dx - tu;
                gst(bc.res_d, q.lo, rdl, st);
                gst(bc.res_d, q.up, rdu, st);
            } else {
                rdl = gld(bc.res_d, q.lo, q.ok);
                rdu = gld(bc.res_d, q.up, q.ok);
            }
            const double til = rcp_nr(tl), tiu = rcp_nr(tu);
            qv = til * (rml - lml * rdl) - tiu * (rmu + lmu * rdu);
            Q = til * lml + tiu * lmu;
            gst(bc.t_inv, q.lo, til, st);
            gst(bc.t_inv, q.up, tiu, st);
        }
        Q = q.ok ? Q : 0.0;
        qv = q.ok ? qv : 0.0;
        M = mfma(dg[lc] * Q, dg[lc], M);
        part += dg[lc] * qv;
    }
    if (aug) ml += xrow_sum(part);
}

__device__ double gen_rq(const RicIO& io, const DynSh& sh, int k, const double* lam) {
    double dg[4];
    gen_dg(io, sh, dg);
    double part = 0.0;
#pragma unroll
    for (int lc = 0; lc < 4; lc++) {
        if (4 * lc >= sh.ng) continue;
        const GenLane q = gen_lane(k, sh.pnb, sh.ng, lc);
        const double w = gld(lam, q.up, q.ok) - gld(lam, q.lo, q.ok);
        part += dg[lc] * (q.ok ? w : 0.0);
    }
    return xrow_sum(part);
}

template <int FM>
__device__ void gen_alpha(const RicIO& io, const DynSh& sh, int k, const BoxCtx& bc, double x, double& al) {
    if (FM == BX_NONE) return;
    const int c = lane_id() & 15;
    double dg[4];
    gen_dg(io, sh, dg);
#pragma unroll
    for (int lc = 0; lc < 4; lc++) {
        if (4 * lc >= sh.ng) continue;
        const GenLane q = gen_lane(k, sh.pnb, sh.ng, lc);
        const bool st = q.ok && c == 0;
        const double dx = row_sum16(dg[lc] * x);
        const double lml = gld(bc.lam, q.lo, q.ok), lmu = gld(bc.lam, q.up, q.ok);
        const double tl = gld(bc.t, q.lo, q.ok), tu = gld(bc.t, q.up, q.ok);
        double dtl, dtu, dll, dlu;
        if (FM == BX_P1) {
            dtl = dx - gld(bc.d, q.lo, q.ok) - tl;
            dtu = -dx + gld(bc.d, q.up, q.ok) - tu;
            const double d0l = gld(bc.dlam, q.lo, q.ok && !bc.pred), d0u = gld(bc.dlam, q.up, q.ok && !bc.pred);
            dll = d0l - (gld(bc.lamt, q.lo, q.ok) * dtl + lml);
            dlu = d0u - (gld(bc.lamt, q.up, q.ok) * dtu + lmu);
        } else {
            dtl = dx - gld(bc.res_d, q.lo, q.ok);
            dtu = -dx + gld(bc.res_d, q.up, q.ok);
            dll = -gld(bc.t_inv, q.lo, q.ok) * (lml * dtl + gld(bc.res_m, q.lo, q.ok));
            dlu = -gld(bc.t_inv, q.up, q.ok) * (lmu * dtu + gld(bc.res_m, q.up, q.ok));
        }
        gst(bc.dt, q.lo, dtl, st);
        gst(bc.dt, q.up, dtu, st);
        gst(bc.dlam, q.lo, dll, st);
        gst(bc.dlam, q.up, dlu, st);
        if (q.ok) {
            alpha_rule(al, lml, dll);
            alpha_rule(al, lmu, dlu);
            alpha_rule(al, tl, dtl);
            alpha_rule(al, tu, dtu);
        }
    }
}

template <int TM>
__device__ double gen_gradient(const RicIO& io, const DynSh& sh, int k, const BoxCtx& bc) {
    if (TM == BX_NONE) return 0.0;
    const int c = lane_id() & 15;
    double dg[4];
    gen_dg(io, sh, dg);
    double part = 0.0;
#pragma unroll
    for (int lc = 0; lc < 4; lc++) {
        if (4 * lc >= sh.ng) continue;
        const GenLane q = gen_lane(k, sh.pnb, sh.ng, lc);
        const bool st = q.ok && c == 0;
        double qv = 0.0;
        if (TM == BX_GIVEN) {
            qv = gld(bc.qx, q.s16, q.ok);
        } else if (TM == BX_P1) {
            const double dll = gld(bc.t_inv, q.lo, q.ok) * (bc.smu - gld(bc.dlam, q.lo, q.ok) * gld(bc.dt, q.lo, q.ok));
            const double dlu = gld(bc.t_inv, q.up, q.ok) * (bc.smu - gld(bc.dlam, q.up, q.ok) * gld(bc.dt, q.up, q.ok));
            gst(bc.dlam, q.lo, dll, st);
            gst(bc.dlam, q.up, dlu, st);
            qv = gld(bc.qxs, q.s16, q.ok) + (dlu - dll);
        } else if (TM == BX_P2) {
            const double rml = gld(bc.res_m, q.lo, q.ok) + (gld(bc.dt, q.lo, q.ok) * gld(bc.dlam, q.lo, q.ok) - bc.smu);
            const double rmu = gld(bc.res_m, q.up, q.ok) + (gld(bc.dt, q.up, q.ok) * gld(bc.dlam, q.up, q.ok) - bc.smu);
            gst(bc.res_m, q.lo, rml, st);
            gst(bc.res_m, q.up, rmu, st);
            qv = gld(bc.t_inv, q.lo, q.ok) * (rml - gld(bc.lam, q.lo, q.ok) * gld(bc.res_d, q.lo, q.ok)) -
                 gld(bc.t_inv, q.up, q.ok) * (rmu + gld(bc.lam, q.up, q.ok) * gld(bc.res_d, q.up, q.ok));
        }
        part += dg[lc] * (q.ok ? qv : 0.0);
    }
    return xrow_sum(part);
}

struct BwdFrag {
    d4 Mi;
    double mlq;
    d4 bop;
    d4 brow;
    double bx[8];
    BoxLane bl;
    double uc, pc, pim1;
    double gc;
};

template <class SH>
__device__ __forceinline__ void load_rsq_tile(const double* R, const SH& sh, d4& Mi) {
    const int l = lane_id(), g = l >> 4, c = l & 15;
    const int vc = tile_var(c, sh.nu, sh.nx, sh.xo);
#pragma unroll
    for (int r = 0; r < 4; r++) {
        const int vi = tile_var(g + 4 * r, sh.nu, sh.nx, sh.xo);
        const int hi = vi > vc ? vi : vc, lo = vi > vc ? vc : vi;
        Mi[r] = ldsel(R, lib4_idx(sh.sdR, hi, lo), vi >= 0 && vc >= 0);
    }
}

__device__ void cert_pass(const RicIO& io, double* cert) {
    const int l = lane_id(), g = l >> 4, c = l & 15;
    for (int k0 = 0; k0 <= io.N; k0 += 8) {
        d4 Mi[8], bop[8];
#pragma unroll
        for (int j = 0; j < 8; j++) {
            const int k = k0 + j <= io.N ? k0 + j : io.N;
            const DynSh sh(StageRef{io.st, k});
            load_rsq_tile(stage_R(io, sh), sh, Mi[j]);
            const int vc = tile_var(c, sh.nu, sh.nx, sh.xo);
            const double* Bk = stage_B(io, sh);
#pragma unroll
            for (int r = 0; r < 4; r++) {
                const int s = 4 * r + g - sh.xo1;
                bop[j][r] = ldsel(Bk, lib4_idx(sh.sdB, vc, s), k < io.N && s >= 0 && s < sh.nx1 && vc >= 0);
            }
        }
#pragma unroll
        for (int j = 0; j < 8; j++) {
            const int k = k0 + j <= io.N ? k0 + j : io.N;
            const DynSh sh(StageRef{io.st, k});
            const double tau = cert_form(Mi[j], 0.0, sh);
            gst(cert, k0 + j, tau, lane_id() == 0 && k0 + j <= io.N);
        }
    }
}

template <bool AUG, int BM, class SH>
__device__ __forceinline__ void bwd_fetch(const RicIO& io, const SH& sh, int k, int update_b, const double* bsrc,
                                          int update_q, const double* qsrc, const BoxCtx& bc, BwdFrag& f) {
    const int l = lane_id(), g = l >> 4, c = l & 15;
    const int nux = sh.nu + sh.nx;
    const double* R = stage_R(io, sh);
    const int vc = tile_var(c, sh.nu, sh.nx, sh.xo);
    load_rsq_tile(R, sh, f.Mi);
    f.mlq = 0.0;
    if (AUG) {
        const double* qp = update_q ? qsrc + k * V16 : R;
        const int qi = update_q ? vc : lib4_idx(sh.sdR, nux, vc);
        f.mlq = ldsel(qp, qi, vc >= 0);
    }
    const BoxLane b = box_lane(io.tileslot, sh.pnb, k);
    f.bl = b;
    f.gc = cert_loaded(BM) ? bc.cert[k] : 0.0;
#pragma unroll
    for (int i = 0; i < 8; i++) f.bx[i] = 0.0;
    if (BM == BX_GIVEN) {
        f.bx[0] = ldsel(bc.Qx, b.s16, b.ok);
        f.bx[1] = AUG ? ldsel(bc.qx, b.s16, b.ok) : 0.0;
    } else if (BM == BX_P1) {
        f.bx[0] = ldsel(bc.lam, b.lo, b.ok);
        f.bx[1] = ldsel(bc.lam, b.up, b.ok);
        f.bx[2] = ldsel(bc.t, b.lo, b.ok);
        f.bx[3] = ldsel(bc.t, b.up, b.ok);
        f.bx[4] = ldsel(bc.d, b.lo, b.ok);
        f.bx[5] = ldsel(bc.d, b.up, b.ok);
    } else if (BM == BX_P2 || BM == BX_P2R) {
        ld_lu(bc.lam, b, f.bx[0], f.bx[1]);
        ld_lu(bc.t, b, f.bx[2], f.bx[3]);
        if (BM == BX_P2) ld_lu(bc.res_m, b, f.bx[4], f.bx[5]);
        ld_lu(bc.res_d, b, f.bx[6], f.bx[7]);
    }
    const bool live = SH::fixed || k < io.N;
    const double* Bk = stage_B(io, sh);
    const double* bp = update_b ? bsrc + k * V16 : Bk;
#pragma unroll
    for (int r = 0; r < 4; r++) {
        const int s = 4 * r + g - sh.xo1;
        const bool ok = live && s >= 0 && s < sh.nx1;
        f.bop[r] = ldsel(Bk, lib4_idx(sh.sdB, vc, s), ok && vc >= 0);
        if (BM != BX_P2R) f.brow[r] = AUG ? ldsel(bp, update_b ? s : lib4_idx(sh.sdB, nux, s), ok) : 0.0;
    }
    if (BM == BX_P2R) {
        static_assert(BM != BX_P2R || AUG, "residual right-hand sides need the augmented row");
        const int sc = c - sh.xo1;
        const bool oks = live && sc >= 0 && sc < sh.nx1;
        f.uc = ldsel(bc.ux, k * V16 + vc, vc >= 0);
        f.pc = ldsel(bc.pi, k * V16 + sc, oks);
        f.pim1 = ldsel(bc.pi, (k - 1) * V16 + (vc - sh.nu), k > 0 && vc >= sh.nu);
        f.brow[0] = ldsel(Bk, lib4_idx(sh.sdB, nux, sc), oks);
    }
}

template <bool AUG, int BM>
__device__ __forceinline__ void box_hessian(const BoxCtx& bc, const BwdFrag& f, double& dq, double& qxv) {
    const int g = lane_id() >> 4;
    const BoxLane& b = f.bl;
    const bool st = b.ok && g == 0;
    dq = 0.0;
    qxv = 0.0;
    if (BM == BX_GIVEN) {
        dq = f.bx[0];
        qxv = f.bx[1];
    } else if (BM == BX_P1) {
        const double til = rcp_nr(f.bx[2]), tiu = rcp_nr(f.bx[3]);
        const double ltl = f.bx[0] * til, ltu = f.bx[1] * tiu;
        const double dll = til * 0.0, dlu = tiu * 0.0;
        const double q = f.bx[1] - ltu * f.bx[5] + dlu - f.bx[0] - ltl * f.bx[4] - dll;
        gst(bc.t_inv, b.lo, til, st);
        gst(bc.t_inv, b.up, tiu, st);
        gst(bc.lamt, b.lo, ltl, st);
        gst(bc.lamt, b.up, ltu, st);
        gst(bc.qxs, b.s16, q, st);
        dq = b.ok ? ltl + ltu : 0.0;
        qxv = (AUG && b.ok) ? q : 0.0;
    } else if (BM == BX_P2 || BM == BX_P2R) {
        const double til = rcp_nr(f.bx[2]), tiu = rcp_nr(f.bx[3]);
        const double rml = BM == BX_P2R ? f.bx[0] * f.bx[2] : f.bx[4];
        const double rmu = BM == BX_P2R ? f.bx[1] * f.bx[3] : f.bx[5];
        const double q = til * (rml - f.bx[0] * f.bx[6]) - tiu * (rmu + f.bx[1] * f.bx[7]);
        if (!bc.no_tinv) st_lu(bc.t_inv, b, til, tiu, b.ok);
        dq = b.ok ? til * f.bx[0] + tiu * f.bx[1] : 0.0;
        qxv = (AUG && b.ok) ? q : 0.0;
    }
}

template <class SH>
__device__ __forceinline__ void bwd_residual(const RicIO& io, Scratch* sm, const SH& sh, int k, const BoxCtx& bc,
                                             BwdFrag& f, double x1c, bool store) {
    const int l = lane_id(), g = l >> 4, c = l & 15;
    const bool live = SH::fixed || k < io.N;
    const int vc = tile_var(c, sh.nu, sh.nx, sh.xo);
    const int sc = c - sh.xo1;
    const bool oks = live && sc >= 0 && sc < sh.nx1;
    double h = f.mlq;
// ... 271 lines not shown
        h = (c == p) ? y : ((c > p) ? h - colp * y : h);
    }
    return h;
}

template <class SH>
__device__ __forceinline__ double trs_usolve(const SH& sh, const d4& S, double invd, double h, bool all) {
    if constexpr (SH::fixed) {
        static_assert(SH::xo == 4, "gain form needs the u block in tile block 0");
        const int c = lane_id() & 15;
        const double hg = sel_g(row_bcast<0>(h), row_bcast<1>(h), row_bcast<2>(h), row_bcast<3>(h));
        const double t = xrow_sum(S[0] * hg);
        return c < 4 ? -t : h + t;
    } else {
        return solve_ln(sh, S, invd, h, all);
    }
}

__device__ __forceinline__ double pi_from_x(const d4& S1, int xo1, const double x1row[4], double pcol) {
    (void)xo1;
    double part = 0.0;
#pragma unroll
    for (int r = 0; r < 4; r++) part += S1[r] * x1row[r];
    return xrow_sum(part) + pcol;
}

struct FwdFrag {
    d4 S;
    double lc, invd;
    double kg;
    d4 bt;
    double bval;
    double hc;
    double pk;
    double bx[10];
    BoxLane bl;
};

template <int MODE, int FM, bool PRED, class SH>
__device__ __forceinline__ void fwd_fetch(const RicIO& io, const SH& sh, int k, int pnbk, const double* bsrc,
                                          int use_bsrc, const double* ux, int compute_pi_, const BoxCtx& bc,
                                          FwdFrag& f) {
    const int compute_pi = PRED ? 0 : compute_pi_;
    const int l = lane_id(), g = l >> 4, c = l & 15;
    const double* Fk = io.F + (long)k * FSTRIDE;
    const bool needS = !SH::fixed || compute_pi;
    if constexpr (SH::fixed) {
        f.S[0] = 0.0;
        if (PRED) {
            f.S[1] = f.S[2] = f.S[3] = 0.0;
        } else {
            load_p_fixed<SH::nx>(Fk, f.S, needS);
        }
        f.lc = MODE == 0 ? gld(Fk, FXR_L + c) : 0.0;
        f.invd = 0.0;
        f.kg = gld(Fk, FXR_KG + l);
    } else {
#pragma unroll
        for (int r = 0; r < 4; r++) f.S[r] = gld(Fk, r * 64 + l, needS);
        f.lc = MODE == 0 ? gld(Fk, 256 + c) : 0.0;
        f.invd = gld(Fk, 272 + c);
        f.kg = gld(Fk, 288 + l);
    }
    const int kk = k < io.N ? k : io.N - 1;
    const bool live = k < io.N;
    const double* Bk = stage_B(io, sh);
    const int s = c - sh.xo1;
    const bool ok = live && s >= 0 && s < sh.nx1;
#pragma unroll
    for (int r = 0; r < 4; r++) {
        const int vi = tile_var(g + 4 * r, sh.nu, sh.nx, sh.xo);
        f.bt[r] = ldsel(Bk, lib4_idx(sh.sdB, vi, s), vi >= 0 && ok);
    }
    f.bval = use_bsrc ? ldsel(bsrc + kk * V16, s, ok) : ldsel(Bk, lib4_idx(sh.sdB, sh.nu + sh.nx, s), ok);
    f.hc = 0.0;
    f.pk = 0.0;
    if (MODE == 1) {
        const int vc = tile_var(c, sh.nu, sh.nx, sh.xo);
        f.hc = ldsel(ux + kk * V16, vc, live && vc >= 0);
    }
#pragma unroll
    for (int i = 0; i < 10; i++) f.bx[i] = 0.0;
    if (FM != BX_NONE) {
        const BoxLane b = box_lane(io.tileslot, pnbk, k);
        f.bl = b;
        if (FM == BX_P1) {
            f.bx[0] = ldsel(bc.d, b.lo, b.ok);
            f.bx[1] = ldsel(bc.d, b.up, b.ok);
            f.bx[2] = ldsel(bc.t, b.lo, b.ok);
            f.bx[3] = ldsel(bc.t, b.up, b.ok);
            f.bx[4] = ldsel(bc.lamt, b.lo, b.ok);
            f.bx[5] = ldsel(bc.lamt, b.up, b.ok);
            f.bx[6] = ldsel(bc.lam, b.lo, b.ok);
            f.bx[7] = ldsel(bc.lam, b.up, b.ok);
            f.bx[8] = ldsel(bc.dlam, b.lo, b.ok && !bc.pred);
            f.bx[9] = ldsel(bc.dlam, b.up, b.ok && !bc.pred);
        } else if (FM == BX_P2) {
            fetch_pair(bc.res_d, b, f.bx[0], f.bx[1]);
            fetch_pair(bc.lam, b, f.bx[4], f.bx[5]);
            if (!PRED) fetch_pair(bc.res_m, b, f.bx[6], f.bx[7]);
            fetch_pair(bc.t, b, f.bx[8], f.bx[9]);
        }
    }
}

template <int MODE, int FM, class FX, bool PRED>
__device__ __forceinline__ void fwd_fetch_k(const RicIO& io, int k, const double* bsrc, int use_bsrc,
                                            const double* ux, int compute_pi, const BoxCtx& bc, FwdFrag& f) {
    const int kk = k < io.N ? k : io.N - 1;
    const StageRef sk{io.st, kk};
    const int pnbk = srd(StageRef{io.st, k}, &StageInfo::pnb);
    with_shape<FX>(sk, [&](const auto& sh) {
        fwd_fetch<MODE, FM, PRED>(io, sh, k, pnbk, bsrc, use_bsrc, ux, compute_pi, bc, f);
    });
}

template <int FM, bool PRED>
__device__ __forceinline__ void box_alpha(const BoxCtx& bc, const FwdFrag& f, double x, double& al) {
    if (FM == BX_NONE) return;
    const BoxLane& b = f.bl;
    double dtl, dtu, dll, dlu, lml, lmu, tl, tu;
    if (FM == BX_P1) {
        dtl = x - f.bx[0] - f.bx[2];
        dtu = -x + f.bx[1] - f.bx[3];
        dll = f.bx[8] - (f.bx[4] * dtl + f.bx[6]);
        dlu = f.bx[9] - (f.bx[5] * dtu + f.bx[7]);
        lml = f.bx[6];
        lmu = f.bx[7];
        tl = f.bx[2];
        tu = f.bx[3];
    } else {
        double bx[10];
        use_pair(f.bx[0], f.bx[1], bx[0], bx[1]);
        use_pair(f.bx[4], f.bx[5], bx[4], bx[5]);
        if (!PRED) use_pair(f.bx[6], f.bx[7], bx[6], bx[7]);
        use_pair(f.bx[8], f.bx[9], bx[8], bx[9]);
        const double til = rcp_nr(bx[8]), tiu = rcp_nr(bx[9]);
        const double rml = PRED ? __dmul_rn(bx[4], bx[8]) : bx[6];
        const double rmu = PRED ? __dmul_rn(bx[5], bx[9]) : bx[7];
        dtl = x - bx[0];
        dtu = -x + bx[1];
        dll = -til * (bx[4] * dtl + rml);
        dlu = -tiu * (bx[5] * dtu + rmu);
        lml = bx[4];
        lmu = bx[5];
        tl = bx[8];
        tu = bx[9];
    }
    st_lu(bc.dt, b, dtl, dtu, b.ok);
    st_lu(bc.dlam, b, dll, dlu, b.ok);
    if (b.ok) {
        alpha_rule(al, lml, dll);
        alpha_rule(al, lmu, dlu);
        alpha_rule(al, tl, dtl);
        alpha_rule(al, tu, dtu);
    }
}

template <int MODE>
__device__ __forceinline__ void fwd_pi(int xo, int nx, int k, const d4& S, const double xrow[4], double pc,
                                       int compute_pi, double* pi) {
    const int g = lane_id() >> 4, c = lane_id() & 15;
    const int s = c - xo;
    const bool okp = s >= 0 && s < nx;
    double pv = 0.0;
    if (compute_pi && k > 0) pv = pi_from_x(S, xo, xrow, okp ? pc : 0.0);
    gst(pi, (k - 1) * V16 + s, pv, compute_pi && k > 0 && g == 0 && okp);
}

template <int MODE, int FM, bool PRED, class SH>
__device__ __forceinline__ void fwd_step(const RicIO& io, Scratch* sm, const SH& sh, int k, const FwdFrag& cur,
                                         double& xcol, double* ux, int compute_pi, double* pi, const BoxCtx& bc,
                                         double& al) {
    const int l = lane_id(), g = l >> 4, c = l & 15;
    const bool all = !SH::fixed && k == 0;
    double xrow[4];
    col2row(sm, xcol, xrow);
    if constexpr (!PRED) fwd_pi<MODE>(sh.xo, sh.nx, k, cur.S, xrow, MODE == 0 ? cur.lc : cur.hc, compute_pi, pi);
    const double rhs = (MODE == 0) ? cur.lc : cur.hc;
    double ur[4];
    if constexpr (SH::fixed) {
        const double v = (c < sh.xo) ? rhs : xcol;
        ur[0] = row_sum16(cur.kg * v);
#pragma unroll
        for (int r = 1; r < 4; r++) ur[r] = xrow[r];
        static_assert(SH::xo <= 4, "gain form needs the u block in tile block 0");
    } else {
        double part = 0.0;
        if (!all) {
#pragma unroll
            for (int r = 0; r < 4; r++) part += (g + 4 * r >= sh.xo) ? lowS(cur.S, r, g, c) * xrow[r] : 0.0;
        }
        const double rc = -rhs - xrow_sum(part);
        double rrow[4];
        col2row(sm, rc, rrow);
#pragma unroll
        for (int r = 0; r < 4; r++) ur[r] = all ? 0.0 : xrow[r];
        HK_STAMP(9, k);
        solve_lt(sh, cur.S, cur.invd, rrow, ur, all);
        HK_STAMP(10, k);
    }
    const double ucol = row2col(sm, ur);
    const int vcs = tile_var(c, sh.nu, sh.nx, sh.xo);
    if (!PRED) gst(ux, k * V16 + vcs, ucol, g == 0 && vcs >= 0);
    box_alpha<FM, PRED>(bc, cur, ucol, al);
    if constexpr (!SH::fixed && FM != BX_NONE) {
        if (sh.ng > 0) gen_alpha<FM>(io, sh, k, bc, ucol, al);
    }
    double gp = 0.0;
#pragma unroll
    for (int r = 0; r < 4; r++) gp += cur.bt[r] * ur[r];
    const int s = c - sh.xo1;
    const bool ok = s >= 0 && s < sh.nx1;
    const double x1 = cur.bval + xrow_sum(gp);
    xcol = ok ? x1 : 0.0;
    HK_STAMP(11, k);
}

template <int MODE, int FM, class FX, bool PRED = false>
__device__ void ric_forward(const RicIO& io, Scratch* sm, const double* bsrc, int use_bsrc, double* ux,
                            int compute_pi, double* pi, const BoxCtx& bc, double& al) {
    const int l = lane_id(), g = l >> 4, c = l & 15;
    double xcol = 0.0;
    FwdFrag f0, f1, f2;
    fwd_fetch_k<MODE, FM, FX, PRED>(io, 0, bsrc, use_bsrc, ux, compute_pi, bc, f0);
    fwd_fetch_k<MODE, FM, FX, PRED>(io, 1, bsrc, use_bsrc, ux, compute_pi, bc, f1);
    auto stage = [&](int k, const FwdFrag& fa, const FwdFrag& fb, FwdFrag& fc) __attribute__((always_inline)) {
        (void)fb;
        HK_STAMP(8, k);
        fwd_fetch_k<MODE, FM, FX, PRED>(io, k + 2 <= io.N ? k + 2 : io.N, bsrc, use_bsrc, ux, compute_pi, bc, fc);
        const StageRef si{io.st, k};
        with_shape<FX>(si, [&](const auto& sh) {
            fwd_step<MODE, FM, PRED>(io, sm, sh, k, fa, xcol, ux, compute_pi, pi, bc, al);
        });
        HK_STAMP(12, k);
    };
    auto finish = [&](const FwdFrag& fN) __attribute__((always_inline)) {
        const DynSh sN(StageRef{io.st, io.N});
        const int v = tile_var(c, sN.nu, sN.nx, sN.xo);
        if constexpr (!PRED) {
            double pc = MODE == 0 ? fN.lc : ldsel(ux + io.N * V16, v, compute_pi && v >= 0);
            double xrow[4] = {0.0, 0.0, 0.0, 0.0};
            if (compute_pi) col2row(sm, xcol, xrow);
            fwd_pi<MODE>(sN.xo, sN.nx, io.N, fN.S, xrow, pc, compute_pi, pi);
            gst(ux, io.N * V16 + v, xcol, g == 0 && v >= 0);
        }
        box_alpha<FM, PRED>(bc, fN, xcol, al);
    };
    for (int k = 0;;) {
        if (k >= io.N) { finish(f0); break; }
        stage(k, f0, f1, f2);
        if (++k >= io.N) { finish(f1); break; }
        stage(k, f1, f2, f0);
        if (++k >= io.N) { finish(f2); break; }
        stage(k, f2, f0, f1);
        ++k;
    }
    if (FM != BX_NONE) {
        const DynSh sN(StageRef{io.st, io.N});
        if (sN.ng > 0) gen_alpha<FM>(io, sN, io.N, bc, xcol, al);
    }
}

template <class FX>
__device__ __forceinline__ void ric_forward_sv(const RicIO& io, Scratch* sm, int update_b, const double* bsrc,
                                               double* ux, int compute_pi, double* pi) {
    BoxCtx bc{};
    double al = 1.0;
    ric_forward<0, BX_NONE, FX>(io, sm, bsrc, update_b, ux, compute_pi, pi, bc, al);
}

struct TrsFrag {
    d4 S;
    double invd;
    d4 bop;
    d4 brow;
    double h0;
    double pbc;
    double bx[12];
    BoxLane bl;
};

template <int TM, bool RPB, class SH>
__device__ __forceinline__ void trs_fetch(const RicIO& io, const SH& sh, int k, const double* hb, const double* hq,
                                          const BoxCtx& bc, int compute_Pb_, const double* Pb, TrsFrag& f) {
    const int compute_Pb = RPB ? compute_Pb_ : 0;
    const int l = lane_id(), g = l >> 4, c = l & 15;
    const double* Fk = io.F + (long)k * FSTRIDE;
    if constexpr (SH::fixed) {
        f.S[0] = gld(Fk, FXR_KG + l);
        if (RPB) {
            load_p_fixed<SH::nx>(Fk, f.S, compute_Pb);
        } else {
            f.S[1] = f.S[2] = f.S[3] = 0.0;
        }
        f.invd = 0.0;
    } else {
#pragma unroll
        for (int r = 0; r < 4; r++) f.S[r] = gld(Fk, r * 64 + l);
        f.invd = gld(Fk, 272 + c);
    }
    const int nux = sh.nu + sh.nx;
    const int vc = tile_var(c, sh.nu, sh.nx, sh.xo);
    const double* R = stage_R(io, sh);
    f.h0 = hq ? ldsel(hq + k * V16, vc, vc >= 0) : ldsel(R, lib4_idx(sh.sdR, nux, vc), vc >= 0);
    const BoxLane b = box_lane(io.tileslot, sh.pnb, k);
    f.bl = b;
#pragma unroll
    for (int i = 0; i < 12; i++) f.bx[i] = 0.0;
    if (TM == BX_GIVEN) {
        f.bx[0] = ldsel(bc.qx, b.s16, b.ok);
    } else if (TM == BX_P1) {
        f.bx[0] = ldsel(bc.t_inv, b.lo, b.ok);
        f.bx[1] = ldsel(bc.t_inv, b.up, b.ok);
        f.bx[2] = ldsel(bc.dlam, b.lo, b.ok);
        f.bx[3] = ldsel(bc.dlam, b.up, b.ok);
        f.bx[4] = ldsel(bc.dt, b.lo, b.ok);
        f.bx[5] = ldsel(bc.dt, b.up, b.ok);
        f.bx[6] = ldsel(bc.qxs, b.s16, b.ok);
    } else if (TM == BX_P2) {
        fetch_pair(bc.t, b, f.bx[0], f.bx[1]);
        fetch_pair(bc.dt, b, f.bx[2], f.bx[3]);
        fetch_pair(bc.dlam, b, f.bx[4], f.bx[5]);
        fetch_pair(bc.lam, b, f.bx[8], f.bx[9]);
        fetch_pair(bc.res_d, b, f.bx[10], f.bx[11]);
    }
    const bool live = SH::fixed || k < io.N;
    const double* Bk = stage_B(io, sh);
    const double* bp = hb ? hb + k * V16 : Bk;
#pragma unroll
    for (int r = 0; r < 4; r++) {
        const int sr = g + 4 * r - sh.xo1;
        const bool ok = live && sr >= 0 && sr < sh.nx1;
        f.bop[r] = ldsel(Bk, lib4_idx(sh.sdB, vc, sr), ok && vc >= 0);
        f.brow[r] = RPB ? ldsel(bp, hb ? sr : lib4_idx(sh.sdB, nux, sr), ok && compute_Pb) : 0.0;
    }
    const int s = c - sh.xo1;
    f.pbc = ldsel(Pb + k * V16, s, !compute_Pb && live && s >= 0 && s < sh.nx1);
}

template <int TM>
__device__ __forceinline__ double box_gradient(const BoxCtx& bc, const TrsFrag& f) {
    const int g = lane_id() >> 4;
    const BoxLane& b = f.bl;
    const bool st = b.ok && g == 0;
    if (TM == BX_GIVEN) return f.bx[0];
    if (TM == BX_P1) {
        const double dll = f.bx[0] * (bc.smu - f.bx[2] * f.bx[4]);
        const double dlu = f.bx[1] * (bc.smu - f.bx[3] * f.bx[5]);
        gst(bc.dlam, b.lo, dll, st);
        gst(bc.dlam, b.up, dlu, st);
        return b.ok ? f.bx[6] + (dlu - dll) : 0.0;
    }
    if (TM == BX_P2) {
        double bx[12];
        use_pair(f.bx[0], f.bx[1], bx[0], bx[1]);
        use_pair(f.bx[2], f.bx[3], bx[2], bx[3]);
        use_pair(f.bx[4], f.bx[5], bx[4], bx[5]);
        use_pair(f.bx[8], f.bx[9], bx[8], bx[9]);
        use_pair(f.bx[10], f.bx[11], bx[10], bx[11]);
        const double til = rcp_nr(bx[0]), tiu = rcp_nr(bx[1]);
        const double rml = __dmul_rn(bx[8], bx[0]) + (bx[2] * bx[4] - bc.smu);
        const double rmu = __dmul_rn(bx[9], bx[1]) + (bx[3] * bx[5] - bc.smu);
        st_lu(bc.res_m, b, rml, rmu, b.ok);
        return b.ok ? til * (rml - bx[8] * bx[10]) - tiu * (rmu + bx[9] * bx[11]) : 0.0;
    }
    return 0.0;
}

template <int TM, bool RPB, class SH>
__device__ __forceinline__ void trs_step(const RicIO& io, Scratch* sm, const SH& sh, int k, const TrsFrag& cur,
                                         const BoxCtx& bc, double* ux, int compute_Pb_, double* Pb, d4& S1,
                                         double& pcol) {
    const int compute_Pb = RPB ? compute_Pb_ : 0;
    const int l = lane_id(), g = l >> 4, c = l & 15;
    const int xo1 = sh.xo1, nx1 = sh.nx1;
    const int vc = tile_var(c, sh.nu, sh.nx, sh.xo);
    const int s = c - xo1;
    double pbc = cur.pbc;
    if (compute_Pb) {
        double part = 0.0;
#pragma unroll
        for (int r = 0; r < 4; r++) part += S1[r] * cur.brow[r];
        pbc = xrow_sum(part);
    }
    gst(Pb, k * V16 + s, pbc, compute_Pb && g == 0 && s >= 0 && s < nx1);
    const double wc = (s >= 0 && s < nx1) ? pbc + pcol : 0.0;
    double wrow[4];
    col2row(sm, wc, wrow);
// ... 53 lines not shown
```

### hpmpc_amd/csrc/hpmpc_capi.cpp

```cpp
#include <cstdlib>

#include "hk_launch_guard.h"
#include "hk_plan.h"

thread_local int g_err = 0;
thread_local DevCtx g_dev;

extern "C" void hk_set_error(int code, const char* what) {
    g_err = code;
    if (code) fprintf(stderr, "[hpmpc_mi355x] %s (code %d)\n", what, code);
}

int launch(int which, const KArgs* a, int count, hipStream_t s) {
#ifdef HK_RIC2
    if (which == K_SV) {
        const char* e = getenv("HPMPC_MI355X_RIC_WAVES");
        if (e && e[0] == '2') {
            const int r = hk_launch_ric2(which, a, count, s);
            if (r != HK_LAUNCH_REFUSED) return r;
        }
    }
#endif
    return hk_launch(which, a, count, s);
}
// ... 54 lines not shown
    constexpr size_t kMaxLayouts = 64;
    if (P->ltabs.size() >= kMaxLayouts) {
        hk_set_error(HPMPC_MI355X_EUNSUPPORTED, "more than 64 distinct stage layouts on one plan (create a plan per layout "
                                           "family, or keep the offsets fixed)");
        return nullptr;
    }
    void* d = nullptr;
    if (!hip_ok(hipMalloc(&d, bytes), "layout stage table")) return nullptr;
    if (!hip_ok(hipMemcpy(d, st.data(), bytes, hipMemcpyHostToDevice), "layout stage table")) {
        (void)hipFree(d);
        return nullptr;
    }
    P->ltabs.push_back({std::move(st), d});
    return d;
}

extern "C" hpmpc_mi355x_plan* hpmpc_mi355x_plan_create(int N, const int* nx, const int* nu, const int* nb,
                                                       const int* const* idxb, const int* ng) {
    const char* why = nullptr;
    if (!plan_supported(N, nx, nu, nb, idxb, ng, &why)) {
        hk_set_error(HPMPC_MI355X_EUNSUPPORTED, why);
        return nullptr;
    }
    auto* P = new hpmpc_mi355x_plan();
    P->N = N;
    P->nx.assign(nx, nx + N + 1);
    P->nu.assign(nu, nu + N + 1);
    P->nu[N] = 0;
    P->nb.assign(nb, nb + N + 1);
    P->ng.assign(ng, ng + N + 1);
    P->idxb.resize(N + 1);
    P->st.resize(N + 1);
    P->tileslot.assign((N + 1) * 16, -1);
    P->slotvar.assign((N + 1) * 16, 0);
    P->offB.resize(N);
    P->offR.resize(N + 1);
    P->offG.resize(N + 1);
    for (int k = 0; k <= N; k++) {
        StageInfoH& s = P->st[k];
        s.nu = P->nu[k];
        s.nx = nx[k];
        s.nb = nb[k];
        s.ng = ng[k];
        s.xo = rup(s.nu, 4);
        s.nx1 = k < N ? nx[k + 1] : 0;
        s.nu1 = k + 1 < N ? P->nu[k + 1] : 0;
        s.xo1 = rup(s.nu1, 4);
        s.sdB = rup(s.nx1, NCL);
        s.sdR = rup(s.nu + s.nx, NCL);
        s.pnb = rup(nb[k], BS);
        s.oD = k * V32;
        s.r0 = 0;
        s.oG = (int)P->packG;
        P->offG[k] = P->packG;
        if (ng[k] > 0) P->packG += (long long)rup(s.nu + s.nx, BS) * rup(ng[k], NCL);
        P->nbt += ng[k];
        P->ngt += ng[k];
        const int nux = s.nu + s.nx;
        if (k < N) {
            P->offB[k] = P->packB;
            P->packB += (long long)rup(nux + 1, BS) * s.sdB;
        }
        P->offR[k] = P->packR;
        P->packR += (long long)rup(nux + 1, BS) * s.sdR;
        if (nb[k] > 0) P->idxb[k].assign(idxb[k], idxb[k] + nb[k]);
        P->nbt += nb[k];
        for (int l = 0; l < nb[k]; l++) {
            const int v = idxb[k][l];
            const int t = v < s.nu ? v : s.xo + (v - s.nu);
            P->tileslot[k * 16 + t] = (signed char)l;
            P->slotvar[k * 16 + l] = (signed char)v;
        }
    }
    if (N >= 3) {
        const int nuc = P->nu[1], nxc = nx[1];
        P->fixcls = hk_fixcls(nuc, nxc);
        if (P->fixcls)
            for (int k = 1; k <= N - 2; k++)
                P->st[k].r0 = (P->nu[k] == nuc && nx[k] == nxc && P->nu[k + 1] == nuc && nx[k + 1] == nxc &&
                               ng[k] == 0)
                                  ? 1
                                  : 0;
    }
    for (int k = 0; k <= N; k++) {
        P->st[k].oB = k < N ? (int)P->offB[k] : 0;
        P->st[k].oR = (int)P->offR[k];
    }
    bool ok = hip_ok(hipMalloc(&P->d_st, sizeof(StageInfoH) * (N + 1)), "plan alloc") &&
              hip_ok(hipMalloc((void**)&P->d_tileslot, (N + 1) * 16), "plan alloc") &&
              hip_ok(hipMalloc((void**)&P->d_slotvar, (N + 1) * 16), "plan alloc") &&
              hip_ok(hipMemcpy(P->d_tileslot, P->tileslot.data(), (N + 1) * 16, hipMemcpyHostToDevice), "plan") &&
              hip_ok(hipMemcpy(P->d_slotvar, P->slotvar.data(), (N + 1) * 16, hipMemcpyHostToDevice), "plan") &&
              hip_ok(hipMemcpy(P->d_st, P->st.data(), sizeof(StageInfoH) * (N + 1), hipMemcpyHostToDevice), "plan");
    if (!ok) {
        hpmpc_mi355x_plan_destroy(P);
        return nullptr;
    }
    g_err = 0;
    return P;
}

extern "C" void hpmpc_mi355x_plan_destroy(hpmpc_mi355x_plan* P) {
    if (!P) return;
    if (P->d_st) (void)hipFree(P->d_st);
    for (auto& t : P->ltabs) (void)hipFree(t.d);
    if (P->d_tileslot) (void)hipFree(P->d_tileslot);
    if (P->d_slotvar) (void)hipFree(P->d_slotvar);
    delete P;
}

extern "C" long long hpmpc_mi355x_ws_doubles(const hpmpc_mi355x_plan* P) { return P ? ws_doubles(P->N) : 0; }

extern "C" int hpmpc_mi355x_last_error(void) { return g_err; }

static unsigned long long* g_dbg_buf = nullptr;
#ifdef HK_STAMPS
extern "C" __attribute__((visibility("default"))) void hpmpc_mi355x_debug_buffer(void* dev_ptr) {
    g_dbg_buf = (unsigned long long*)dev_ptr;
}
#endif

extern "C" const char* hpmpc_mi355x_version(void) {
    return "hpmpc_mi355x 0.1 gfx950 (wave-per-problem, f64 MFMA 16x16x4 stage contractions)";
}

KArgs base_args(const hpmpc_mi355x_plan* P, int nprob, int p0) {
    KArgs a;
    memset(&a, 0, sizeof a);
    a.N = P->N;
    a.nprob = nprob;
    a.p0 = p0;
    a.st = P->d_st;
    a.tileslot = P->d_tileslot;
    a.slotvar = P->d_slotvar;
    a.sV16 = (long long)(P->N + 1) * V16;
    a.sV32 = (long long)(P->N + 1) * V32;
    a.sW = ws_doubles(P->N);
    a.fixcls = P->fixcls;
    a.nbt = P->nbt;
    a.ngt = P->ngt;
    a.sG = P->packG;
    a.dbg = g_dbg_buf;
    return a;
}

bool layout_apply(hpmpc_mi355x_plan* P, const hpmpc_mi355x_layout* lay, KArgs& a) {
    if (P->ngt) {
        hk_set_error(HPMPC_MI355X_EUNSUPPORTED, "batched entry points: general constraints (ng > 0) need the "
                                           "reference-named entry points");
        return false;
    }
    return layout_set(P, lay, a);
}

bool layout_set(hpmpc_mi355x_plan* P, const hpmpc_mi355x_layout* lay, KArgs& a) {
    if (lay && lay->BAbt_off && lay->RSQrq_off) {
        a.st = plan_stage_table(P, lay->BAbt_off, lay->RSQrq_off, lay->BAbt_shared, lay->RSQrq_shared);
        if (!a.st) return false;
    }
    a.sB = lay ? lay->BAbt_stride : P->packB;
    a.sR = lay ? lay->RSQrq_stride : P->packR;
    return true;
}

hpmpc_mi355x_plan* thread_plan(int N, const int* nx, const int* nu, const int* nb, int** idxb, const int* ng) {
    struct Cache {
        hpmpc_mi355x_plan* plan = nullptr;
        std::vector<int> key;
        ~Cache() {
            if (plan) hpmpc_mi355x_plan_destroy(plan);
        }
    };
    thread_local Cache c;
    std::vector<int> k;
    k.push_back(N);
    for (int i = 0; i <= N; i++) {
        k.push_back(nx[i]);
        k.push_back(i < N ? nu[i] : 0);
        k.push_back(nb[i]);
        k.push_back(ng[i]);
        for (int l = 0; l < nb[i]; l++) k.push_back(idxb[i][l]);
    }
    if (c.plan && k == c.key) return c.plan;
    if (c.plan) hpmpc_mi355x_plan_destroy(c.plan);
    c.plan = hpmpc_mi355x_plan_create(N, nx, nu, nb, idxb, ng);
    c.key = c.plan ? k : std::vector<int>();
    return c.plan;
}

int ipm_run(KArgs& a, int count, const double* BAbt, const double* RSQrq, const double* d, double* ux, double* pi,
            double* lam, double* t, double* ws, int k_max, double mu0, double mu_tol, double alpha_min, int warm_start,
            int compute_mult, int* kk, int* ret, double* stat, int which, void* stream) {
    a.BAbt = BAbt;
    a.RSQ = RSQrq;
    a.d = d;
    a.ux = ux;
    a.pi = pi;
    a.lam = lam;
    a.t = t;
    a.ws = ws;
    a.k_max = k_max;
    a.mu0 = mu0;
    a.mu_tol = mu_tol;
    a.alpha_min = alpha_min;
    a.warm_start = warm_start;
    a.compute_mult = compute_mult;
    a.kk = kk;
    a.ret = ret;
    a.stat = stat;
    int e = hk_launch(which, &a, count, (hipStream_t)stream);
    if (e) {
        hk_set_error(HPMPC_MI355X_EHIP, "hk_ipm launch failed");
        return HPMPC_MI355X_EHIP;
    }
    return g_err = 0;
}

namespace {

int ipm_launch(const hpmpc_mi355x_plan* plan, const hpmpc_mi355x_layout* lay, int nprob, int p0, int count,
               const double* BAbt, const double* RSQrq, const double* d, double* ux, double* pi, double* lam,
               double* t, double* ws, int k_max, double mu0, double mu_tol, double alpha_min, int warm_start,
               int compute_mult, int* kk, int* ret, double* stat, int which, void* stream) {
    auto* P = const_cast<hpmpc_mi355x_plan*>(plan);
    if (!P) return g_err = HPMPC_MI355X_EUNSUPPORTED;
// ... 153 lines not shown
```

### hpmpc_amd/csrc/hpmpc_kargs.h

```cpp
#pragma once

constexpr int FSTRIDE = 352;
constexpr int V16 = 16;
constexpr int V32 = 32;

enum HkLaunch {
    K_SV = 0,
    K_TRF = 1,
    K_TRS = 2,
    K_RES = 3,
    K_IPM = 4,
    K_KKT = 5,
    K_KKT_P1 = 6,
    K_PASS_INIT = 10,
    K_PASS_FACT = 11,
    K_PASS_PRED = 12,
    K_PASS_CORR = 13,
    K_PASS_UPDATE = 14,
    K_SOLO = 15,
    K_SOLO_1W = 16,
    K_QDRAIN = 17,
    K_PASS_PREDCORR = 18,
};
static_assert(K_PASS_FACT == K_PASS_INIT + 1 && K_PASS_PRED == K_PASS_INIT + 2 && K_PASS_CORR == K_PASS_INIT + 3 &&
                  K_PASS_UPDATE == K_PASS_INIT + 4,
              "the pass ids are consecutive: the host computes them as K_PASS_INIT + pass and K_PASS_FACT + i % 4");

struct KArgs {
    int N, nprob, p0;
    int nbt;
    int ngt;
    int fixcls;
    const void* st;
    const signed char* tileslot;
    const signed char* slotvar;
    const double* BAbt;
    long long sB;
    const double* RSQ;
    long long sR;
    const double* d;
    const double* DCt;
    long long sG;
    double* ws;
    long long sW;
    double *ux, *pi;
    double *lam, *t;
    long long sV16, sV32;
    const double *vb, *vq, *vQx, *vqx;
    double* vPb;
    int update_b, update_q, use_box, compute_pi, compute_Pb;
    int k_max, warm_start, compute_mult, single_newton;
    int phase1_only;
    int res_plain;
    double mu0, mu_tol, alpha_min;
    int *kk, *ret;
    double* stat;
    double* mu_out;
    int nq;
    int* qctl;
    unsigned long long* dbg;
    int nslots;
    int no_bkp;
    int qpar;
    int* dctr;
    int* qnext;
};
```

### hpmpc_amd/csrc/hpmpc_kernels.hip

```cpp
#include "hk_ipm_body.h"
#include "hk_kkt_body.h"
#include "hk_launch.h"
#include "hk_mw.h"
#include <cstdlib>

template <class FX>
__global__ __launch_bounds__(64) void hk_ric_sv(KArgs a) {
    const LdsTabs T = lds_tables(a);
    Scratch& sm = *T.sm;
    const int p = blockIdx.x + a.p0;
    if (p >= a.nprob) return;
    double* F = a.ws + (long)p * a.sW;
    RicIO io = make_io(a, T, p, F);
    const long o16 = (long)p * a.sV16;
    const double* b = a.vb ? a.vb + o16 : nullptr;
    const double* q = a.vq ? a.vq + o16 : nullptr;
    BoxCtx bc{};
    bc.Qx = a.vQx ? a.vQx + o16 : nullptr;
    bc.qx = a.vqx ? a.vqx + o16 : nullptr;
    double* Pb = a.vPb ? a.vPb + o16 : nullptr;
#ifdef HK_STAMPS
    const unsigned long long t0 = mw_clock();
#endif
    if (a.use_box)
        ric_backward<true, BX_GIVEN, FX, CERT_LOAD>(io, &sm, a.update_b, b, a.update_q, q, bc, a.compute_Pb, Pb);
    else
        ric_backward<true, BX_NONE, FX, CERT_LOAD>(io, &sm, a.update_b, b, a.update_q, q, bc, a.compute_Pb, Pb);
    wsync();
#ifdef HK_STAMPS
    const unsigned long long t1 = mw_clock();
#endif
    ric_forward_sv<FX>(io, &sm, a.update_b, b, a.ux + o16, a.compute_pi, a.pi + o16);
#ifdef HK_STAMPS
    const unsigned long long t2 = mw_clock();
    if (a.dbg && p == 0 && lane_id() == 0) {
        a.dbg[60] = t1 - t0;
        a.dbg[61] = t2 - t1;
    }
#endif
}

template <class FX>
__global__ __launch_bounds__(64) void hk_ric_trf(KArgs a) {
    const LdsTabs T = lds_tables(a);
    Scratch& sm = *T.sm;
    const int p = blockIdx.x + a.p0;
    if (p >= a.nprob) return;
    double* F = a.ws + (long)p * a.sW;
    RicIO io = make_io(a, T, p, F);
    const long o16 = (long)p * a.sV16;
    BoxCtx bc{};
    bc.Qx = a.vQx ? a.vQx + o16 : nullptr;
    if (a.use_box)
        ric_backward<false, BX_GIVEN, FX, CERT_LOAD>(io, &sm, 0, nullptr, 0, nullptr, bc, 0, nullptr);
    else
        ric_backward<false, BX_NONE, FX, CERT_LOAD>(io, &sm, 0, nullptr, 0, nullptr, bc, 0, nullptr);
}

template <class FX>
__global__ __launch_bounds__(64) void hk_ric_trs(KArgs a) {
    const LdsTabs T = lds_tables(a);
    Scratch& sm = *T.sm;
    const int p = blockIdx.x + a.p0;
    if (p >= a.nprob) return;
    double* F = a.ws + (long)p * a.sW;
    RicIO io = make_io(a, T, p, F);
    const long o16 = (long)p * a.sV16;
    BoxCtx bc{};
    bc.qx = a.vqx ? a.vqx + o16 : nullptr;
    double al = 1.0;
    if (a.use_box)
        ric_trs<BX_GIVEN, BX_NONE, FX>(io, &sm, a.vb + o16, a.vq + o16, bc, a.ux + o16, a.compute_pi, a.pi + o16,
                                   a.compute_Pb, a.vPb + o16, al);
    else
        ric_trs<BX_NONE, BX_NONE, FX>(io, &sm, a.vb + o16, a.vq + o16, bc, a.ux + o16, a.compute_pi, a.pi + o16,
                                  a.compute_Pb, a.vPb + o16, al);
}

template <class FX>
__global__ __launch_bounds__(64) void hk_res(KArgs a) {
    const LdsTabs T = lds_tables(a);
    const int p = blockIdx.x + a.p0;
    if (p >= a.nprob) return;
    RicIO io = make_io(a, T, p, nullptr);
    const long o16 = (long)p * a.sV16, o32 = (long)p * a.sV32;
    double* out = a.ws + (long)p * a.sW;
    const long n1 = a.N + 1;
    BoxCtx bc{};
    bc.d = a.d + o32;
    bc.lam = a.lam + o32;
    bc.t = a.t + o32;
    ResIO ro{};
    ro.bsrc = a.vb ? a.vb + o16 : nullptr;
    ro.qsrc = a.vq ? a.vq + o16 : nullptr;
    ro.ux = a.ux + o16;
    ro.pi = a.pi + o16;
    ro.rq = out;
    ro.rb = out + n1 * V16;
    ro.rd = out + 2 * n1 * V16;
    ro.rm = out + 2 * n1 * V16 + n1 * V32;
    double mu = 0.0;
    const bool have = residual_pass<false, FX>(io, bc, ro, mu);
    if (a.res_plain) {
        wsync();
        HK_FOR_BOX(io, k, { ro.rd[up] = -ro.rd[up]; });
        HK_FOR_GEN(io, k, { ro.rd[up] = -ro.rd[up]; });
        if (lane_id() == 0) a.mu_out[p] = have ? mu : 0.0;
        return;
    }
    if (lane_id() == 0 && have) a.mu_out[p] = mu;
}

template <class FX>
__global__ __launch_bounds__(64) HK_TWO_WAVES void hk_ipm_init(KArgs a) {
    const LdsTabs T = lds_tables(a);
    if (a.nq) {
        if (ipm_refill<FX, 7, true>(a, T, blockIdx.x)) qlist_push(a, a.qpar, blockIdx.x);
        return;
    }
    Who who;
    if (!who_am_i(a, who)) return;
    IpmView v = ipm_view(a, T, who);
    ipm_start<FX, 7, true>(a, T, v);
}


template <class FX>
__global__ __launch_bounds__(64) HK_TWO_WAVES void hk_ipm_fact(KArgs a) {
    if (a.nq && blockIdx.x == 0 && lane_id() == 0) *qcount(a, a.qpar ^ 1) = 0;
    Who who;
    if (!who_am_i(a, who) || !slot_active(a, who)) return;
    const LdsTabs T = lds_tables(a);
    IpmView v = ipm_view(a, T, who);
    if (v.w.state[S_ACTIVE] == 0.0) return;
    fact_body<FX>(a, T, v);
}

template <class FX>
__global__ __launch_bounds__(64) HK_TWO_WAVES void hk_ipm_pred(KArgs a) {
    Who who;
    if (!who_am_i(a, who) || !slot_active(a, who)) return;
    const LdsTabs T = lds_tables(a);
    IpmView v = ipm_view(a, T, who);
    if (v.w.state[S_ACTIVE] == 0.0) return;
    pred_body<FX>(a, T, v);
}

template <class FX>
__global__ __launch_bounds__(64) HK_TWO_WAVES void hk_ipm_corr(KArgs a) {
    Who who;
    if (!who_am_i(a, who) || !slot_active(a, who)) return;
    const LdsTabs T = lds_tables(a);
    IpmView v = ipm_view(a, T, who);
    if (v.w.state[S_ACTIVE] == 0.0) return;
    corr_body<FX>(a, T, v);
}

template <class FX>
__global__ __launch_bounds__(64) HK_TWO_WAVES void hk_ipm_predcorr(KArgs a) {
    Who who;
    if (!who_am_i(a, who) || !slot_active(a, who)) return;
    const LdsTabs T = lds_tables(a);
    {
        IpmView v = ipm_view(a, T, who);
        if (v.w.state[S_ACTIVE] == 0.0) return;
        pred_body<FX>(a, T, v);
    }
    wsync();
    int s = who.s, q = who.q, d = who.d;
    asm volatile("" : "+v"(s), "+v"(q), "+v"(d));
    const Who w2{__builtin_amdgcn_readfirstlane(s), __builtin_amdgcn_readfirstlane(q), __builtin_amdgcn_readfirstlane(d)};
    IpmView v = ipm_view(a, T, w2);
    corr_body<FX>(a, T, v);
}

template <class FX>
__global__ __launch_bounds__(64) HK_TWO_WAVES void hk_ipm_update(KArgs a) {
    Who who;
    if (!who_am_i(a, who) || !slot_active(a, who)) return;
    const LdsTabs T = lds_tables(a);
    IpmView v = ipm_view(a, T, who);
    if (v.w.state[S_ACTIVE] == 0.0) return;
    bool again = update_body<FX, 4>(a, v);
    if (!again && a.nq) {
        if (v.l == 0) atomicAdd(&a.qctl[1], 1);
        again = ipm_refill<FX, 4, false>(a, T, who.s);
    }
    if (a.nq && again) qlist_push(a, a.qpar ^ 1, who.s);
}

template <class FX>
__global__ __launch_bounds__(64) void hk_ipm_solo(KArgs a) {
    const LdsTabs T = lds_tables(a);
    const int p = blockIdx.x + a.p0;
    if (p >= a.nprob) return;
    if (carve(a.ws + (long)p * a.sW, a.N).state[S_ACTIVE] == 0.0) return;
    auto view = [&]() __attribute__((always_inline)) {
        int q = p;
        asm volatile("" : "+v"(q));
        q = __builtin_amdgcn_readfirstlane(q);
        const Who w{q, q, q};
        return ipm_view(a, T, w);
    };
    for (int it = 0; it < a.k_max; it++) {
        wsync();
        {
            IpmView v = view();
            fact_body<FX>(a, T, v);
        }
        wsync();
        {
            IpmView v = view();
            pred_body<FX>(a, T, v);
        }
        wsync();
        {
            IpmView v = view();
            corr_body<FX>(a, T, v);
        }
        wsync();
        IpmView v = view();
        if (!update_body<FX, 4>(a, v)) break;
    }
}

namespace {

template <class FX>
__device__ __forceinline__ void fact_body_mw(const KArgs& a, IpmView& v, int& tb, int w) {
    const double* st = v.w.state;
    const bool sn = a.single_newton != 0;
    v.bc.cert_new = st[S_KK] == 0.0;
    if (st[S_PHASE] == 1.0)
        tb = ric_backward_mw<true, BX_P1, FX>(v.io, tb, w, 0, nullptr, 0, nullptr, v.bc, 1, v.w.Pb);
    else {
        v.bc.res_rhs = !sn;
        v.bc.no_tinv = a.no_bkp;
        tb = ric_backward_mw<true, BX_P2R, FX>(v.io, tb, w, 0, nullptr, 0, nullptr, v.bc, 1, v.w.Pb);
    }
}

template <class FX>
__device__ __forceinline__ void pred_body_mw(const KArgs& a, IpmView& v, int& tb, int w) {
    double* st = v.w.state;
    const bool sn = a.single_newton != 0;
    const int phase = (int)st[S_PHASE], kk = (int)st[S_KK];
    const double mu = st[S_MU];
    double sigma = st[S_SIGMA];
    double al = 1.0;
    if (phase == 1) {
        v.bc.pred = 1;
        tb = ric_forward_mw<0, BX_P1, FX, true>(v.io, tb, w, nullptr, 0, v.w.dux, 0, v.w.dpi, v.bc, al);
    } else {
        tb = ric_forward_mw<0, BX_P2, FX, true>(v.io, tb, w, v.w.res_b, !sn, v.w.dux, 0, v.w.dpi, v.bc, al);
    }
    const double alpha = al * 0.995;
    double mu_aff;
    {
        const RicIO io = v.io;
        const BoxCtx bc = v.bc;
        mu_aff = mu_aff_pass<7>(io, bc, alpha, st[S_MUSCAL]);
    }
    double smu = a.mu0;
    if (!sn) {
        sigma = mu_aff / mu;
        sigma = sigma * sigma * sigma;
        smu = sigma * mu;
    }
    __syncthreads();
    if (v.l == 0) {
        v.stat[5 * kk] = st[S_SIGMA];
        v.stat[5 * kk + 1] = al;
        v.stat[5 * kk + 2] = mu_aff;
        st[S_SIGMA] = sigma;
        st[S_SMU] = smu;
    }
}

template <class FX>
__device__ __forceinline__ void corr_body_mw(const KArgs& a, IpmView& v, int& tb, int w) {
    double* st = v.w.state;
    const int phase = (int)st[S_PHASE], kk = (int)st[S_KK];
    v.bc.smu = st[S_SMU];
    double al = 1.0;
    if (phase == 1)
        tb = ric_trs_mw<BX_P1, BX_P1, FX>(v.io, tb, w, nullptr, nullptr, v.bc, v.w.dux, a.compute_mult, v.w.dpi,
                                     v.w.Pb, al);
    else
        tb = ric_trs_mw<BX_P2, BX_P2, FX>(v.io, tb, w, v.w.res_b, v.w.res_q, v.bc, v.w.dux, a.compute_mult, v.w.dpi,
                                     v.w.Pb, al);
    if (v.l == 0) {
        v.stat[5 * kk] = st[S_SIGMA];
        v.stat[5 * kk + 3] = al;
        st[S_ALPHA] = al * 0.995;
    }
}

template <class FX, int CI>
__device__ __forceinline__ bool update_body_mw(const KArgs& a, const IpmView& v0, const MwSplit& mws0) {
    IpmView v = v0;
    const MwSplit mws = mws0;
    double* st = v.w.state;
    const int phase = (int)st[S_PHASE];
    int kk = (int)st[S_KK];
    const double alpha = st[S_ALPHA];
    const double sigma = st[S_SIGMA];
// ... 87 lines not shown
    }
#ifdef HK_STAMPS
    if (a.dbg && p == 0 && threadIdx.x == 0) {
        for (int i = 0; i < 4; i++) a.dbg[32 + i] = tph[i];
        for (int i = 0; i < MW_WAVES; i++) a.dbg[40 + i] = hk_mw.wait_cyc[i];
        for (int i = 0; i < 4; i++) a.dbg[48 + i] = hk_mw.seg[i];
    }
#endif
#undef HK_MW_PHASE
    if (threadIdx.x == 0 && hk_mw.err) {
        a.ret[p] = HK_MW_ERR;
        for (int i = 0; i < 4; i++) a.stat[(long)p * 5 * a.k_max + i] = hk_mw.dbg[i];
    }
}

template <class FX>
__global__ __launch_bounds__(256) void hk_ipm_solo_mw(KArgs a) {
    const LdsTabs T = lds_tables(a);
    const int p = blockIdx.x + a.p0;
    if (p >= a.nprob) return;
    if (carve(a.ws + (long)p * a.sW, a.N).state[S_ACTIVE] == 0.0) return;
    mw_solve<FX>(a, T, Who{p, p, p});
}

template <class FX>
__global__ __launch_bounds__(256) void hk_ipm_qdrain_mw(KArgs a) {
    const LdsTabs T = lds_tables(a);
    const int n = __builtin_amdgcn_readfirstlane(*qcount(a, a.qpar));
    if ((int)blockIdx.x >= n) return;
    const int s = __builtin_amdgcn_readfirstlane(qlist(a, a.qpar)[blockIdx.x]);
    const int q = __builtin_amdgcn_readfirstlane(a.qctl[2 + s]);
    const double* st = carve(a.ws + (long)s * a.sW, a.N).state;
    if (q < 0 || st[S_ACTIVE] == 0.0) return;
    const int kk0 = (int)st[S_KK];
    __syncthreads();
    mw_solve<FX>(a, T, Who{s, q, q % a.nprob});
    __syncthreads();
    if (threadIdx.x == 0) {
        a.qctl[2 + s] = -1;
        atomicAdd(&a.dctr[0], a.kk[q] - kk0);
        atomicAdd(&a.dctr[1], 1);
        atomicAdd(&a.qctl[1], 1);
    }
}

template <class FX>
__global__ __launch_bounds__(64) void hk_kkt_new_rhs(KArgs a) {
    const LdsTabs T = lds_tables(a);
    Scratch& sm = *T.sm;
    const int p = blockIdx.x + a.p0;
    if (p >= a.nprob) return;
    const int N = a.N;
    Ws w = carve(a.ws + (long)p * a.sW, N);
    RicIO io = make_io(a, T, p, w.F);
    BoxTab bt{T.tileslot, T.slotvar};
    const long o16 = (long)p * a.sV16, o32 = (long)p * a.sV32;
    double* ux = a.ux + o16;
    double* pi = a.pi + o16;
    double* lam = a.lam + o32;
    double* t = a.t + o32;
    const double* dv = a.d + o32;
    const KktIO v{a.vb, a.vq, o16, dv, ux, pi, lam, t};
    kkt_body<FX, false>(a, io, &sm, bt, w, v);
}

template <class FX>
__global__ __launch_bounds__(64) void hk_kkt_new_rhs_p1(KArgs a) {
    const LdsTabs T = lds_tables(a);
    Scratch& sm = *T.sm;
    const int p = blockIdx.x + a.p0;
    if (p >= a.nprob) return;
    const int N = a.N;
    Ws w = carve(a.ws + (long)p * a.sW, N);
    RicIO io = make_io(a, T, p, w.F);
    BoxTab bt{T.tileslot, T.slotvar};
    const long o16 = (long)p * a.sV16, o32 = (long)p * a.sV32;
    double* ux = a.ux + o16;
    double* pi = a.pi + o16;
    double* lam = a.lam + o32;
    double* t = a.t + o32;
    const double* rC = a.d + o32;
    const int l = lane_id();
    BoxCtx bc = box_ctx(w, rC, lam, t);
    HK_FOR_BOX(io, k, { w.qx[k * V16 + slot] = -w.lamt[up] * rC[up] - w.lamt[lo] * rC[lo]; });
    HK_FOR_GEN(io, k, { w.qx[s16] = -w.lamt[up] * rC[up] - w.lamt[lo] * rC[lo]; });
    wsync();
    double al = 1.0;
    ric_trs<BX_GIVEN, BX_NONE, FX>(io, &sm, a.vb + o16, a.vq + o16, bc, ux, a.compute_mult, pi, 1, w.Pb, al);
    wsync();
    HK_FOR_BOX(io, k, {
        const double x = ux[k * V16 + bt.slotvar[k * 16 + slot]];
        const double tl = x - rC[lo], tu = -x + rC[up];
        t[lo] = tl;
        t[up] = tu;
        lam[lo] = -w.lamt[lo] * tl;
        lam[up] = -w.lamt[up] * tu;
    });
    if (a.ngt) {
        const int c = l & 15;
        for (int k = 0; k <= N; k++) {
            const StageInfo si = load_stage(io.st, k);
            if (si.ng == 0) continue;
            const DynSh sh(si);
            const int vc = tile_var(c, sh.nu, sh.nx, sh.xo);
            const double x = gld(ux, k * V16 + vc, vc >= 0);
            double dg[4];
            gen_dg(io, sh, dg);
#pragma unroll
            for (int lc = 0; lc < 4; lc++) {
                if (4 * lc >= sh.ng) continue;
                const GenLane q = gen_lane(k, sh.pnb, sh.ng, lc);
                const bool st = q.ok && c == 0;
                const double dx = row_sum16(dg[lc] * x);
                const double tl = dx - gld(rC, q.lo, q.ok), tu = -dx + gld(rC, q.up, q.ok);
                gst(t, q.lo, tl, st);
                gst(t, q.up, tu, st);
                gst(lam, q.lo, -gld(w.lamt, q.lo, q.ok) * tl, st);
                gst(lam, q.up, -gld(w.lamt, q.up, q.ok) * tu, st);
            }
        }
    }
}

template <class FX>
static int launch_t(int which, const KArgs* a, int count, hipStream_t stream) {
    dim3 grid(count), block(64);
    const size_t lds = sizeof(Scratch) + (size_t)(a->N + 1) * (sizeof(StageInfo) + 40);
    switch (which) {
        case K_SV: hipLaunchKernelGGL(hk_ric_sv<FX>, grid, block, lds, stream, *a); break;
        case K_TRF: hipLaunchKernelGGL(hk_ric_trf<FX>, grid, block, lds, stream, *a); break;
        case K_TRS: hipLaunchKernelGGL(hk_ric_trs<FX>, grid, block, lds, stream, *a); break;
        case K_RES: hipLaunchKernelGGL(hk_res<FX>, grid, block, lds, stream, *a); break;
        case K_IPM:
            hipLaunchKernelGGL(hk_ipm_init<FX>, grid, block, lds, stream, *a);
            for (int it = 0; it < a->k_max; it++) {
                hipLaunchKernelGGL(hk_ipm_fact<FX>, grid, block, lds, stream, *a);
                hipLaunchKernelGGL(hk_ipm_pred<FX>, grid, block, lds, stream, *a);
                hipLaunchKernelGGL(hk_ipm_corr<FX>, grid, block, lds, stream, *a);
                hipLaunchKernelGGL(hk_ipm_update<FX>, grid, block, lds, stream, *a);
            }
            break;
        case K_KKT: hipLaunchKernelGGL(hk_kkt_new_rhs<FX>, grid, block, lds, stream, *a); break;
        case K_KKT_P1: hipLaunchKernelGGL(hk_kkt_new_rhs_p1<FX>, grid, block, lds, stream, *a); break;
        case K_PASS_INIT: hipLaunchKernelGGL(hk_ipm_init<FX>, grid, block, lds, stream, *a); break;
        case K_PASS_FACT: hipLaunchKernelGGL(hk_ipm_fact<FX>, grid, block, lds, stream, *a); break;
        case K_PASS_PRED: hipLaunchKernelGGL(hk_ipm_pred<FX>, grid, block, lds, stream, *a); break;
        case K_PASS_CORR: hipLaunchKernelGGL(hk_ipm_corr<FX>, grid, block, lds, stream, *a); break;
        case K_PASS_UPDATE: hipLaunchKernelGGL(hk_ipm_update<FX>, grid, block, lds, stream, *a); break;
        case K_PASS_PREDCORR: hipLaunchKernelGGL(hk_ipm_predcorr<FX>, grid, block, lds, stream, *a); break;
        case K_SOLO:
        case K_SOLO_1W: {
            static const HkKernelLimits lim_mw(reinterpret_cast<const void*>(&hk_ipm_solo_mw<FX>));
            const char* env = getenv("HPMPC_MI355X_SOLO");
            const bool single = which == K_SOLO_1W || (env && env[0] == '1');
            const size_t lds_mw = mw_lds_bytes(a->N);
            hipLaunchKernelGGL(hk_ipm_init<FX>, grid, block, lds, stream, *a);
            if (!single && a->N <= MW_NMAX && lim_mw.check(lds_mw, 256) == 0)
                hipLaunchKernelGGL(hk_ipm_solo_mw<FX>, grid, dim3(256), lds_mw, stream, *a);
            else
                hipLaunchKernelGGL(hk_ipm_solo<FX>, grid, block, lds, stream, *a);
            break;
        }
        case K_QDRAIN: {
            static const HkKernelLimits lim_dr(reinterpret_cast<const void*>(&hk_ipm_qdrain_mw<FX>));
            const size_t lds_mw = mw_lds_bytes(a->N);
            if (a->N > MW_NMAX || lim_dr.check(lds_mw, 256) != 0) return HK_LAUNCH_REFUSED;
            hipLaunchKernelGGL(hk_ipm_qdrain_mw<FX>, grid, dim3(256), lds_mw, stream, *a);
            break;
        }
        default: return -1;
    }
    return (int)hipGetLastError();
}

extern "C" int hk_fixcls(int nu, int nx) {
    if (nu == 4 && nx == 12) return 1;
    if (nu == 3 && nx == 8) return 2;
    return 0;
}

#ifdef HK_STAMPS
extern "C" __attribute__((visibility("default"))) int hpmpc_mi355x_diag_xfac(unsigned long long* out, int reset) {
    if (hipMemcpyFromSymbol(out, HIP_SYMBOL(g_xfac_stat), 6 * sizeof(unsigned long long)) != hipSuccess) return -11;
    if (reset) {
        const unsigned long long z[6] = {0, 0, 0, 0, 0, 0};
        if (hipMemcpyToSymbol(HIP_SYMBOL(g_xfac_stat), z, sizeof(z)) != hipSuccess) return -11;
    }
    return 0;
}
#endif

extern "C" int hk_launch(int which, const KArgs* a, int count, hipStream_t stream) {
    if (count <= 0) return 0;
#ifdef HK_STAMPS
    if (a->dbg) {
        unsigned long long* p = a->dbg;
        int st = 50;
        (void)hipMemcpyToSymbol(HIP_SYMBOL(g_dbg), &p, sizeof(p));
        (void)hipMemcpyToSymbol(HIP_SYMBOL(g_dbg_stage), &st, sizeof(st));
    }
    {
// ... 12 lines not shown
```

Measured before the change: 2.141 million.

## Pack box/general constraint vectors into compact workspace layout during IPM iterations

Adds a configurable packed layout (BoxLay with SB/HB strides) for per-stage constraint vectors. The IPM now keeps private lam, t and d copies in the workspace in that compact layout and copies them back to the caller's padded layout only when the solve finishes. Index helpers (box_lo, gen_lo, box_du, gen_du) replace the fixed V32 stride throughout. The aim is less memory traffic and better locality for constraint data, paid for with extra copy-in/copy-out passes, more index arithmetic, and a wider change to workspace sizing. It also parallelises the build script's library builds.

```diff
diff --git a/hpmpc_amd/build.py b/hpmpc_amd/build.py
--- a/hpmpc_amd/build.py
+++ b/hpmpc_amd/build.py
@@ -117,9 +117,14 @@
 
 
 def build_all(force: bool = False, verbose: bool = False) -> None:
-    build_hip(force=force, verbose=verbose)
-    build_stamps(verbose=verbose, force=force)
-    build_ric2(verbose=verbose, force=force)
+    from concurrent.futures import ThreadPoolExecutor
+
+    with ThreadPoolExecutor(max_workers=3) as pool:
+        jobs = [pool.submit(build_hip, force=force, verbose=verbose),
+                pool.submit(build_stamps, verbose=verbose, force=force),
+                pool.submit(build_ric2, verbose=verbose, force=force)]
+        for j in jobs:
+            j.result()
     build_calib(verbose=verbose)
     build_oracle(force=force)
 
diff --git a/hpmpc_amd/csrc/hk_ipm.h b/hpmpc_amd/csrc/hk_ipm.h
--- a/hpmpc_amd/csrc/hk_ipm.h
+++ b/hpmpc_amd/csrc/hk_ipm.h
@@ -8,31 +8,32 @@
     const signed char* slotvar;
 };
 
-#define HK_FOR_BOX(io, KV, ...)                                                       \
+#define HK_FOR_BOX(io, WY, KV, ...)                                                   \
     for (int j4_ = 0; j4_ <= (io).N; j4_ += 4) {                                       \
         const int KV = j4_ + (lane_id() >> 4);                                         \
         const int slot = lane_id() & 15;                                               \
         if (KV <= (io).N) {                                                            \
             const int nb_ = (io).st[KV].nb, pnb_ = (io).st[KV].pnb;                    \
             if (slot < nb_) {                                                          \
-                const int lo = KV * V32 + slot, up = KV * V32 + pnb_ + slot;           \
-                (void)lo; (void)up;                                                    \
+                const int lo = box_lo((io).lay, KV, slot), up = lo + box_du((io).lay, pnb_); \
+                const int wlo = box_lo(WY, KV, slot), wup = wlo + box_du(WY, pnb_);    \
+                (void)lo; (void)up; (void)wlo; (void)wup;                              \
                 __VA_ARGS__                                                            \
             }                                                                          \
         }                                                                              \
     }
 
-#define HK_FOR_GEN(io, KV, ...)                                                       \
+#define HK_FOR_GEN(io, WY, KV, ...)                                                   \
     for (int j4_ = 0; j4_ <= (io).N; j4_ += 4) {                                       \
         const int KV = j4_ + (lane_id() >> 4);                                         \
         const int gl_ = lane_id() & 15;                                                \
         if (KV <= (io).N) {                                                            \
-            const int ng_ = (io).st[KV].ng, pnb_ = (io).st[KV].pnb;                    \
+            const int ng_ = (io).st[KV].ng, pnb_ = (io).st[KV].pnb, nbg_ = (io).st[KV].nb; \
             if (gl_ < ng_) {                                                           \
-                const int png_ = (ng_ + 3) & ~3;                                       \
-                const int lo = KV * V32 + 2 * pnb_ + gl_, up = lo + png_;               \
+                const int lo = gen_lo((io).lay, KV, nbg_, pnb_, gl_), up = lo + gen_du((io).lay, ng_); \
+                const int wlo = gen_lo(WY, KV, nbg_, pnb_, gl_), wup = wlo + gen_du(WY, ng_); \
                 const int s16 = KV * V16 + pnb_ + gl_;                                 \
-                (void)lo; (void)up; (void)s16;                                         \
+                (void)lo; (void)up; (void)wlo; (void)wup; (void)s16;                   \
                 __VA_ARGS__                                                            \
             }                                                                          \
         }                                                                              \
@@ -44,7 +45,7 @@
     bool box;
 };
 
-__device__ __forceinline__ QuadLane quad_lane(const RicIO& io, int q) {
+__device__ __forceinline__ QuadLane quad_lane(const RicIO& io, int q, const BoxLay& y) {
     const int l = lane_id(), g = l >> 4, c = l & 15;
     const int k = 4 * q + g;
     const bool kv = k <= io.N;
@@ -53,11 +54,11 @@
     QuadLane b;
     b.ok = kv && c < s.nb + s.ng;
     b.box = c < s.nb;
-    const int png = (s.ng + 3) & ~3;
-    b.lo = kc * V32 + (b.box ? c : 2 * s.pnb + (c - s.nb));
-    b.up = b.lo + (b.box ? s.pnb : png);
+    b.lo = b.box ? box_lo(y, kc, c) : gen_lo(y, kc, s.nb, s.pnb, c - s.nb);
+    b.up = b.lo + (b.box ? box_du(y, s.pnb) : gen_du(y, s.ng));
     return b;
 }
+__device__ __forceinline__ QuadLane quad_lane(const RicIO& io, int q) { return quad_lane(io, q, io.lay); }
 
 typedef __attribute__((address_space(3))) double lds_f64;
 
@@ -104,6 +105,31 @@
                   (v[j][4] + alpha * v[j][5]) * (v[j][6] + alpha * v[j][7]);
     }
     return wave_sum(ms) * mu_scal;
+}
+
+template <int CH, int NW = 1>
+__device__ void publish_pass(const RicIO& io, const double* wlam, const double* wt, double* lam, double* t, int w) {
+    const int nq = (io.N + 4) / 4;
+    const BoxLay cy = caller_lay();
+    for (int q0 = NW > 1 ? w * CH : 0; q0 < nq; q0 += NW * CH) {
+        double v[CH][4];
+#pragma unroll
+        for (int j = 0; j < CH; j++) {
+            const QuadLane b = quad_lane(io, q0 + j);
+            v[j][0] = gld(wlam, b.lo, b.ok);
+            v[j][1] = gld(wlam, b.up, b.ok);
+            v[j][2] = gld(wt, b.lo, b.ok);
+            v[j][3] = gld(wt, b.up, b.ok);
+        }
+#pragma unroll
+        for (int j = 0; j < CH; j++) {
+            const QuadLane c = quad_lane(io, q0 + j, cy);
+            gst(lam, c.lo, v[j][0], c.ok);
+            gst(lam, c.up, v[j][1], c.ok);
+            gst(t, c.lo, v[j][2], c.ok);
+            gst(t, c.up, v[j][3], c.ok);
+        }
+    }
 }
 
 template <int CH, int NW = 1>
@@ -320,7 +346,7 @@
     f.dpc = UPD ? ldsel(ro.dpi, k * V16 + s, oks) : 0.0;
     f.x1 = ldsel(ro.ux, (k + 1) * V16 + si.nu1 + s, oks);
     f.dx1 = UPD ? ldsel(ro.dux, (k + 1) * V16 + si.nu1 + s, oks) : 0.0;
-    const BoxLane b = box_lane(io.tileslot, si.pnb, k);
+    const BoxLane b = box_lane(io, si.pnb, k);
     f.bl = b;
     f.bx[0] = ldsel(bc.d, b.lo, b.ok);
     f.bx[1] = ldsel(bc.d, b.up, b.ok);
@@ -408,7 +434,7 @@
 #pragma unroll
             for (int lc = 0; lc < 4; lc++) {
                 if (4 * lc >= sh.ng) continue;
-                const GenLane q = gen_lane(k, sh.pnb, sh.ng, lc);
+                const GenLane q = gen_lane(io.lay, k, sh, lc);
                 const bool st = q.ok && c == 0;
                 const double dx = row_sum16(dg[lc] * x);
                 const double tgl = gld(bc.t, q.lo, q.ok), tgu = gld(bc.t, q.up, q.ok);
diff --git a/hpmpc_amd/csrc/hk_ipm_body.h b/hpmpc_amd/csrc/hk_ipm_body.h
--- a/hpmpc_amd/csrc/hk_ipm_body.h
+++ b/hpmpc_amd/csrc/hk_ipm_body.h
@@ -17,6 +17,7 @@
     double *dlam, *dt, *t_inv, *lamt, *res_d, *res_m, *t_bkp, *lam_bkp;
     double* state;
     double* cert;
+    double *lam, *t, *d;
 };
 
 enum { S_MU = 0, S_ALPHA, S_SIGMA, S_SMU, S_KK, S_PHASE, S_ACTIVE, S_MUSCAL, S_RET };
@@ -46,6 +47,9 @@
     w.lam_bkp = W + 7 * b;
     w.state = W + 8 * b;
     w.cert = w.state + 16;
+    w.lam = w.F + ws_carve_doubles(N);
+    w.t = w.lam + b;
+    w.d = w.lam + 2 * b;
     return w;
 }
 
@@ -88,6 +92,7 @@
 __device__ __forceinline__ RicIO make_io(const KArgs& a, const LdsTabs& T, int p, double* F) {
     RicIO io;
     io.N = a.N;
+    io.lay = caller_lay();
     io.st = T.st;
     io.tileslot = T.tileslot;
     io.BAbt = a.BAbt + (long)p * a.sB;
@@ -107,7 +112,7 @@
 
 template <int CH>
 __device__ void init_var(const RicIO& io, const double* dv, double* ux, double* pi, double* dpi, double* lam,
-                         double* t, double mu0, int warm_start) {
+                         double* t, double* dw, double mu0, int warm_start) {
     const int l = lane_id(), g = l >> 4, c = l & 15;
     const double thr0 = 0.1;
     const int nq = (io.N + 4) / 4;
@@ -126,11 +131,12 @@
             const int tile = c < si.nu ? c : si.xo + (c - si.nu);
             const int slot = okv ? io.tileslot[kc * 16 + (okv ? tile : 0)] : -1;
             bx[j] = kv[j] && slot >= 0;
-            lo[j] = kc * V32 + (slot >= 0 ? slot : 0);
-            up[j] = lo[j] + si.pnb;
+            const int sl = slot >= 0 ? slot : 0;
+            lo[j] = box_lo(io.lay, kc, sl);
+            up[j] = lo[j] + box_du(io.lay, si.pnb);
             iv[j] = kc * V16 + c;
-            dl[j] = gld(dv, lo[j], bx[j]);
-            du[j] = gld(dv, up[j], bx[j]);
+            dl[j] = gld(dv, kc * V32 + sl, bx[j]);
+            du[j] = gld(dv, kc * V32 + sl + si.pnb, bx[j]);
             xv[j] = warm_start ? gld(ux, iv[j], kv[j]) : 0.0;
         }
 #pragma unroll
@@ -158,12 +164,14 @@
             gst(t, up[j], tu, bx[j]);
             gst(lam, lo[j], mu0 / tl, bx[j]);
             gst(lam, up[j], mu0 / tu, bx[j]);
+            gst(dw, lo[j], dl[j], bx[j]);
+            gst(dw, up[j], du[j], bx[j]);
         }
     }
 }
 
 __device__ void init_var_gen(const RicIO& io, const double* dv, const double* ux, double* lam, double* t,
-                             double mu0) {
+                             double* dw, double mu0) {
     const int l = lane_id(), c = l & 15;
     const double thr0 = 0.1;
     for (int k = 0; k <= io.N; k++) {
@@ -177,11 +185,14 @@
 #pragma unroll
         for (int lc = 0; lc < 4; lc++) {
             if (4 * lc >= sh.ng) continue;
-            const GenLane q = gen_lane(k, sh.pnb, sh.ng, lc);
+            const GenLane q = gen_lane(io.lay, k, sh, lc), qc = gen_lane(caller_lay(), k, sh, lc);
             const bool st = q.ok && c == 0;
             const double dx = row_sum16(dg[lc] * x);
-            const double tl = fmax(thr0, dx + (-gld(dv, q.lo, q.ok)));
-            const double tu = fmax(thr0, -dx + gld(dv, q.up, q.ok));
+            const double dgl = gld(dv, qc.lo, q.ok), dgu = gld(dv, qc.up, q.ok);
+            const double tl = fmax(thr0, dx + (-dgl));
+            const double tu = fmax(thr0, -dx + dgu);
+            gst(dw, q.lo, dgl, st);
+            gst(dw, q.up, dgu, st);
             gst(t, q.lo, tl, st);
             gst(t, q.up, tu, st);
             gst(lam, q.lo, mu0 / tl, st);
@@ -221,7 +232,7 @@
     Ws w;
     RicIO io;
     BoxTab bt;
-    double *ux, *pi, *lam, *t, *stat;
+    double *ux, *pi, *stat;
     const double* dv;
     BoxCtx bc;
 };
@@ -262,14 +273,13 @@
     v.w = carve(a.ws + (long)who.s * a.sW, a.N);
     v.io = make_io(a, T, who.d, v.w.F);
     v.bt = BoxTab{T.tileslot, T.slotvar};
-    const long o16 = (long)who.q * a.sV16, o32 = (long)who.q * a.sV32;
+    const long o16 = (long)who.q * a.sV16;
     v.ux = a.ux + o16;
     v.pi = a.pi + o16;
-    v.lam = a.lam + o32;
-    v.t = a.t + o32;
     v.dv = a.d + (long)who.d * a.sV32;
     v.stat = a.stat + (long)who.q * 5 * a.k_max;
-    v.bc = box_ctx(v.w, v.dv, v.lam, v.t);
+    v.io.lay = BoxLay{a.SB, a.HB};
+    v.bc = box_ctx(v.w, v.w.d, v.w.lam, v.w.t);
     v.bc.ux = v.ux;
     v.bc.pi = v.pi;
     return v;
@@ -292,6 +302,13 @@
     return ro;
 }
 
+__device__ __forceinline__ void caller_lam_t(const KArgs& a, int q, double*& lam, double*& t) {
+    asm volatile("" : "+v"(q));
+    const long o32 = (long)__builtin_amdgcn_readfirstlane(q) * a.sV32;
+    lam = a.lam + o32;
+    t = a.t + o32;
+}
+
 template <class FX, int CI, int NW = 1>
 __device__ double p2_start(const KArgs& a, IpmView& v, const MwSplit& mws = MwSplit{0, nullptr}) {
     const double mu = update_p2_pass<CI, false, true, NW>(v.io, v.bc, v.bt.slotvar, 0.0, 1.0 / (2.0 * a.nbt), v.ux,
@@ -301,7 +318,7 @@
     return mu;
 }
 
-template <class FX, int CI, int NW = 1>
+template <class FX, int CI, int NW = 1, bool PUB = true>
 __device__ bool ipm_continue(const KArgs& a, IpmView& v, int kk, double mu, double alpha, double sigma, int phase,
                              const MwSplit& mws = MwSplit{0, nullptr}) {
     const bool sn = a.single_newton != 0;
@@ -321,6 +338,11 @@
     }
     int ret = 0;
     if (!active) {
+        if constexpr (PUB) {
+            double *lam, *t;
+            caller_lam_t(a, v.q, lam, t);
+            publish_pass<CI, NW>(v.io, v.w.lam, v.w.t, lam, t, mws.w);
+        }
         if (!sn && mu <= a.mu_tol)
             ret = 0;
         else if (kk >= a.k_max)
@@ -381,13 +403,32 @@
     }
     const bool sn = a.single_newton != 0;
     if (!sn) {
-        init_var<CI>(v.io, v.dv, v.ux, v.pi, v.w.dpi, v.lam, v.t, a.mu0, a.warm_start);
+        init_var<CI>(v.io, v.dv, v.ux, v.pi, v.w.dpi, v.w.lam, v.w.t, v.w.d, a.mu0, a.warm_start);
         if (a.ngt) {
             wsync();
-            init_var_gen(v.io, v.dv, v.ux, v.lam, v.t, a.mu0);
+            init_var_gen(v.io, v.dv, v.ux, v.w.lam, v.w.t, v.w.d, a.mu0);
         }
     } else {
         for (int i = l; i < (N + 1) * V16; i += 64) v.w.dpi[i] = 0.0;
+        const BoxLay cy = caller_lay();
+        double *lam, *t;
+        caller_lam_t(a, v.q, lam, t);
+        HK_FOR_BOX(v.io, cy, k, {
+            v.w.lam[lo] = lam[wlo];
+            v.w.lam[up] = lam[wup];
+            v.w.t[lo] = t[wlo];
+            v.w.t[up] = t[wup];
+            v.w.d[lo] = v.dv[wlo];
+            v.w.d[up] = v.dv[wup];
+        });
+        HK_FOR_GEN(v.io, cy, k, {
+            v.w.lam[lo] = lam[wlo];
+            v.w.lam[up] = lam[wup];
+            v.w.t[lo] = t[wlo];
+            v.w.t[up] = t[wup];
+            v.w.d[lo] = v.dv[wlo];
+            v.w.d[up] = v.dv[wup];
+        });
     }
     if (l == 0) v.w.state[S_MUSCAL] = 1.0 / (2.0 * nbt);
     wsync();
@@ -500,7 +541,7 @@
     }
 }
 
-template <class FX, int CI>
+template <class FX, int CI, bool PUB = true>
 __device__ __forceinline__ bool update_body(const KArgs& a, IpmView& v) {
     double* st = v.w.state;
     const int phase = (int)st[S_PHASE];
@@ -522,7 +563,7 @@
     wsync();
     if (v.l == 0) v.stat[5 * kk + 4] = mu;
     kk++;
-    return ipm_continue<FX, CI>(a, v, kk, mu, alpha, st[S_SIGMA], phase);
-}
-
-}
+    return ipm_continue<FX, CI, 1, PUB>(a, v, kk, mu, alpha, st[S_SIGMA], phase);
+}
+
+}
diff --git a/hpmpc_amd/csrc/hk_kkt_body.h b/hpmpc_amd/csrc/hk_kkt_body.h
--- a/hpmpc_amd/csrc/hk_kkt_body.h
+++ b/hpmpc_amd/csrc/hk_kkt_body.h
@@ -24,10 +24,19 @@
         ux[i] = w.ux_bkp[i];
         pi[i] = w.pi_bkp[i];
     }
-    for (int i = l; i < (N + 1) * V32; i += 64) {
-        t[i] = w.t_bkp[i];
-        lam[i] = w.lam_bkp[i];
-    }
+    const BoxLay wy{a.SB, a.HB};
+    HK_FOR_BOX(io, wy, k, {
+        t[lo] = w.t_bkp[wlo];
+        t[up] = w.t_bkp[wup];
+        lam[lo] = w.lam_bkp[wlo];
+        lam[up] = w.lam_bkp[wup];
+    });
+    HK_FOR_GEN(io, wy, k, {
+        t[lo] = w.t_bkp[wlo];
+        t[up] = w.t_bkp[wup];
+        lam[lo] = w.lam_bkp[wlo];
+        lam[up] = w.lam_bkp[wup];
+    });
     wsync();
     double mu = 0.0;
     ResIO ro{};
@@ -45,24 +54,24 @@
     ro.rm = w.res_m;
     residual_pass<false, FX>(io, bc, ro, mu);
     wsync();
-    HK_FOR_BOX(io, k, {
-        w.qx[k * V16 + slot] = w.t_inv[lo] * (w.res_m[lo] - lam[lo] * w.res_d[lo]) -
-                               w.t_inv[up] * (w.res_m[up] + lam[up] * w.res_d[up]);
+    HK_FOR_BOX(io, wy, k, {
+        w.qx[k * V16 + slot] = w.t_inv[wlo] * (w.res_m[lo] - lam[lo] * w.res_d[lo]) -
+                               w.t_inv[wup] * (w.res_m[up] + lam[up] * w.res_d[up]);
     });
-    HK_FOR_GEN(io, k, {
-        w.qx[s16] = w.t_inv[lo] * (w.res_m[lo] - lam[lo] * w.res_d[lo]) -
-                    w.t_inv[up] * (w.res_m[up] + lam[up] * w.res_d[up]);
+    HK_FOR_GEN(io, wy, k, {
+        w.qx[s16] = w.t_inv[wlo] * (w.res_m[lo] - lam[lo] * w.res_d[lo]) -
+                    w.t_inv[wup] * (w.res_m[up] + lam[up] * w.res_d[up]);
     });
     wsync();
     double al = 1.0;
     ric_trs<BX_GIVEN, BX_NONE, FX>(io, sm, w.res_b, w.res_q, bc, w.dux, a.compute_mult, w.dpi, 1, w.Pb, al);
     wsync();
-    HK_FOR_BOX(io, k, {
+    HK_FOR_BOX(io, wy, k, {
         const int vi = bt.slotvar[k * 16 + slot];
         const double x = w.dux[k * V16 + vi];
         const double dtl = x - w.res_d[lo], dtu = -x + w.res_d[up];
-        const double dll = -w.t_inv[lo] * (lam[lo] * dtl + w.res_m[lo]);
-        const double dlu = -w.t_inv[up] * (lam[up] * dtu + w.res_m[up]);
+        const double dll = -w.t_inv[wlo] * (lam[lo] * dtl + w.res_m[lo]);
+        const double dlu = -w.t_inv[wup] * (lam[up] * dtu + w.res_m[up]);
         w.dt[lo] = dtl;
         w.dt[up] = dtu;
         w.dlam[lo] = dll;
@@ -75,7 +84,7 @@
             const DynSh sh(si);
             const int vc = tile_var(l & 15, sh.nu, sh.nx, sh.xo);
             double dummy = 1.0;
-            gen_alpha<BX_P2>(io, sh, k, bc, gld(w.dux, k * V16 + vc, vc >= 0), dummy);
+            gen_alpha<BX_P2>(io, sh, k, bc, gld(w.dux, k * V16 + vc, vc >= 0), dummy, wy);
         }
     }
     wsync();
@@ -84,13 +93,13 @@
         if (l < si.nu + si.nx) ux[k * V16 + l] += 1.0 * w.dux[k * V16 + l];
         if (k < N && l < si.nx1) pi[k * V16 + l] += 1.0 * w.dpi[k * V16 + l];
     }
-    HK_FOR_BOX(io, k, {
+    HK_FOR_BOX(io, wy, k, {
         lam[lo] += 1.0 * w.dlam[lo];
         lam[up] += 1.0 * w.dlam[up];
         t[lo] += 1.0 * w.dt[lo];
         t[up] += 1.0 * w.dt[up];
     });
-    HK_FOR_GEN(io, k, {
+    HK_FOR_GEN(io, wy, k, {
         lam[lo] += 1.0 * w.dlam[lo];
         lam[up] += 1.0 * w.dlam[up];
         t[lo] += 1.0 * w.dt[lo];
diff --git a/hpmpc_amd/csrc/hk_mw.h b/hpmpc_amd/csrc/hk_mw.h
--- a/hpmpc_amd/csrc/hk_mw.h
+++ b/hpmpc_amd/csrc/hk_mw.h
@@ -443,7 +443,7 @@
                     if (!PRED) gst(ux, k * V16 + vcs, ucol, g == 0 && vcs >= 0);
                     box_alpha<FM, PRED>(bc, fc, ucol, al);
                     if constexpr (!SHT::fixed && FM != BX_NONE) {
-                        if (sh.ng > 0) gen_alpha<FM>(io, sh, k, bc, ucol, al);
+                        if (sh.ng > 0) gen_alpha<FM>(io, sh, k, bc, ucol, al, io.lay);
                     }
                     const int s = c - sh.xo1;
                     const bool ok = s >= 0 && s < sh.nx1;
@@ -460,7 +460,7 @@
                 const int v = tile_var(c, sN.nu, sN.nx, sN.xo);
                 if (!PRED) gst(ux, N * V16 + v, ucol, g == 0 && v >= 0);
                 box_alpha<FM, PRED>(bc, fc, ucol, al);
-                if (FM != BX_NONE && sN.ng > 0) gen_alpha<FM>(io, DynSh(sN), N, bc, ucol, al);
+                if (FM != BX_NONE && sN.ng > 0) gen_alpha<FM>(io, DynSh(sN), N, bc, ucol, al, io.lay);
             }
         };
         FwdFrag ca, na, cb, nb;
diff --git a/hpmpc_amd/csrc/hk_plan.h b/hpmpc_amd/csrc/hk_plan.h
--- a/hpmpc_amd/csrc/hk_plan.h
+++ b/hpmpc_amd/csrc/hk_plan.h
@@ -31,12 +31,22 @@
     int ngt = 0;
     std::vector<long long> offG;
     long long packG = 0;
+    int HB = 0, SB = 0;
 };
 
-inline long long ws_doubles(int N) {
-    const long long n = (long long)(N + 1) * (FSTRIDE + 9 * V16 + 8 * V32 + 1) + 16;
-    return (n + 31) / 32 * 32;
+struct BoxPack {
+    int HB, SB;
+};
+inline BoxPack box_pack(int N, const int* nb, const int* ng, bool wide) {
+    int hb = 0;
+    for (int k = 0; k <= N; k++) hb = nb[k] + ng[k] > hb ? nb[k] + ng[k] : hb;
+    if (wide) hb = V32 / 2;
+    return BoxPack{hb, 2 * hb};
 }
+inline int box_pair_lo(const BoxPack& bp, int k, int j) { return k * bp.SB + j; }
+inline int box_pair_up(const BoxPack& bp, int k, int j) { return k * bp.SB + bp.HB + j; }
+
+inline long long ws_doubles(int N) { return ws_carve_doubles(N) + 3LL * (N + 1) * V32; }
 
 bool plan_supported(int N, const int* nx, const int* nu, const int* nb, const int* const* idxb, const int* ng,
                     const char** why);
diff --git a/hpmpc_amd/csrc/hk_ric2.hip b/hpmpc_amd/csrc/hk_ric2.hip
--- a/hpmpc_amd/csrc/hk_ric2.hip
+++ b/hpmpc_amd/csrc/hk_ric2.hip
@@ -357,6 +357,7 @@
 __device__ __forceinline__ RicIO r2_io(const KArgs& a, const R2Tabs& T, int p) {
     RicIO io;
     io.N = a.N;
+    io.lay = caller_lay();
     io.st = T.st;
     io.tileslot = T.tileslot;
     io.BAbt = a.BAbt + (long)p * a.sB;
diff --git a/hpmpc_amd/csrc/hk_riccati.h b/hpmpc_amd/csrc/hk_riccati.h
--- a/hpmpc_amd/csrc/hk_riccati.h
+++ b/hpmpc_amd/csrc/hk_riccati.h
@@ -397,8 +397,20 @@
     return cert_g_shift(Mi, sh);
 }
 
+struct BoxLay {
+    int SB, HB;
+};
+__device__ __forceinline__ BoxLay caller_lay() { return BoxLay{V32, -1}; }
+__device__ __forceinline__ int box_lo(const BoxLay& y, int k, int slot) { return k * y.SB + slot; }
+__device__ __forceinline__ int box_du(const BoxLay& y, int pnb) { return y.HB >= 0 ? y.HB : pnb; }
+__device__ __forceinline__ int gen_lo(const BoxLay& y, int k, int nb, int pnb, int gl) {
+    return k * y.SB + (y.HB >= 0 ? nb : 2 * pnb) + gl;
+}
+__device__ __forceinline__ int gen_du(const BoxLay& y, int ng) { return y.HB >= 0 ? y.HB : (ng + 3) & ~3; }
+
 struct RicIO {
     int N;
+    BoxLay lay;
     const StageInfo* st;
     const signed char* tileslot;
     const double* BAbt;
@@ -590,13 +602,13 @@
     bool ok;
 };
 
-__device__ __forceinline__ BoxLane box_lane(const signed char* tileslot, int pnb, int k) {
+__device__ __forceinline__ BoxLane box_lane(const RicIO& io, int pnb, int k) {
     const int c = lane_id() & 15;
-    const int slot = tileslot[k * 16 + c];
+    const int slot = io.tileslot[k * 16 + c];
     BoxLane b;
     b.ok = slot >= 0;
-    b.lo = k * V32 + slot;
-    b.up = b.lo + pnb;
+    b.lo = box_lo(io.lay, k, slot);
+    b.up = b.lo + box_du(io.lay, pnb);
     b.s16 = k * V16 + slot;
     return b;
 }
@@ -638,13 +650,13 @@
     bool ok;
 };
 
-__device__ __forceinline__ GenLane gen_lane(int k, int pnb, int ng, int lc) {
+__device__ __forceinline__ GenLane gen_lane(const BoxLay& y, int k, const DynSh& sh, int lc) {
     const int gl = 4 * lc + (lane_id() >> 4);
-    const int png = (ng + 3) & ~3;
+    const int pnb = sh.pnb;
     GenLane q;
-    q.ok = gl < ng;
-    q.lo = k * V32 + 2 * pnb + gl;
-    q.up = q.lo + png;
+    q.ok = gl < sh.ng;
+    q.lo = gen_lo(y, k, sh.nb, pnb, gl);
+    q.up = q.lo + gen_du(y, sh.ng);
     q.s16 = k * V16 + pnb + gl;
     return q;
 }
@@ -671,7 +683,7 @@
 #pragma unroll
     for (int lc = 0; lc < 4; lc++) {
         if (4 * lc >= sh.ng) continue;
-        const GenLane q = gen_lane(k, sh.pnb, sh.ng, lc);
+        const GenLane q = gen_lane(io.lay, k, sh, lc);
         const bool st = q.ok && c == 0;
         double Q = 0.0, qv = 0.0;
         if (BM == BX_GIVEN) {
@@ -727,7 +739,7 @@
 #pragma unroll
     for (int lc = 0; lc < 4; lc++) {
         if (4 * lc >= sh.ng) continue;
-        const GenLane q = gen_lane(k, sh.pnb, sh.ng, lc);
+        const GenLane q = gen_lane(io.lay, k, sh, lc);
         const double w = gld(lam, q.up, q.ok) - gld(lam, q.lo, q.ok);
         part += dg[lc] * (q.ok ? w : 0.0);
     }
@@ -735,7 +747,8 @@
 }
 
 template <int FM>
-__device__ void gen_alpha(const RicIO& io, const DynSh& sh, int k, const BoxCtx& bc, double x, double& al) {
+__device__ void gen_alpha(const RicIO& io, const DynSh& sh, int k, const BoxCtx& bc, double x, double& al,
+                          const BoxLay& tiy) {
     if (FM == BX_NONE) return;
     const int c = lane_id() & 15;
     double dg[4];
@@ -743,7 +756,7 @@
 #pragma unroll
     for (int lc = 0; lc < 4; lc++) {
         if (4 * lc >= sh.ng) continue;
-        const GenLane q = gen_lane(k, sh.pnb, sh.ng, lc);
+        const GenLane q = gen_lane(io.lay, k, sh, lc);
         const bool st = q.ok && c == 0;
         const double dx = row_sum16(dg[lc] * x);
         const double lml = gld(bc.lam, q.lo, q.ok), lmu = gld(bc.lam, q.up, q.ok);
@@ -758,8 +771,9 @@
         } else {
             dtl = dx - gld(bc.res_d, q.lo, q.ok);
             dtu = -dx + gld(bc.res_d, q.up, q.ok);
-            dll = -gld(bc.t_inv, q.lo, q.ok) * (lml * dtl + gld(bc.res_m, q.lo, q.ok));
-            dlu = -gld(bc.t_inv, q.up, q.ok) * (lmu * dtu + gld(bc.res_m, q.up, q.ok));
+            const GenLane qi = gen_lane(tiy, k, sh, lc);
+            dll = -gld(bc.t_inv, qi.lo, q.ok) * (lml * dtl + gld(bc.res_m, q.lo, q.ok));
+            dlu = -gld(bc.t_inv, qi.up, q.ok) * (lmu * dtu + gld(bc.res_m, q.up, q.ok));
         }
         gst(bc.dt, q.lo, dtl, st);
         gst(bc.dt, q.up, dtu, st);
@@ -784,7 +798,7 @@
 #pragma unroll
     for (int lc = 0; lc < 4; lc++) {
         if (4 * lc >= sh.ng) continue;
-        const GenLane q = gen_lane(k, sh.pnb, sh.ng, lc);
+        const GenLane q = gen_lane(io.lay, k, sh, lc);
         const bool st = q.ok && c == 0;
         double qv = 0.0;
         if (TM == BX_GIVEN) {
@@ -872,7 +886,7 @@
         const int qi = update_q ? vc : lib4_idx(sh.sdR, nux, vc);
         f.mlq = ldsel(qp, qi, vc >= 0);
     }
-    const BoxLane b = box_lane(io.tileslot, sh.pnb, k);
+    const BoxLane b = box_lane(io, sh.pnb, k);
     f.bl = b;
     f.gc = cert_loaded(BM) ? bc.cert[k] : 0.0;
 #pragma unroll
@@ -1310,7 +1324,7 @@
 #pragma unroll
     for (int i = 0; i < 10; i++) f.bx[i] = 0.0;
     if (FM != BX_NONE) {
-        const BoxLane b = box_lane(io.tileslot, pnbk, k);
+        const BoxLane b = box_lane(io, pnbk, k);
         f.bl = b;
         if (FM == BX_P1) {
             f.bx[0] = ldsel(bc.d, b.lo, b.ok);
@@ -1433,7 +1447,7 @@
     if (!PRED) gst(ux, k * V16 + vcs, ucol, g == 0 && vcs >= 0);
     box_alpha<FM, PRED>(bc, cur, ucol, al);
     if constexpr (!SH::fixed && FM != BX_NONE) {
-        if (sh.ng > 0) gen_alpha<FM>(io, sh, k, bc, ucol, al);
+        if (sh.ng > 0) gen_alpha<FM>(io, sh, k, bc, ucol, al, io.lay);
     }
     double gp = 0.0;
 #pragma unroll
@@ -1486,7 +1500,7 @@
     }
     if (FM != BX_NONE) {
         const DynSh sN(StageRef{io.st, io.N});
-        if (sN.ng > 0) gen_alpha<FM>(io, sN, io.N, bc, xcol, al);
+        if (sN.ng > 0) gen_alpha<FM>(io, sN, io.N, bc, xcol, al, io.lay);
     }
 }
 
@@ -1532,7 +1546,7 @@
     const int vc = tile_var(c, sh.nu, sh.nx, sh.xo);
     const double* R = stage_R(io, sh);
     f.h0 = hq ? ldsel(hq + k * V16, vc, vc >= 0) : ldsel(R, lib4_idx(sh.sdR, nux, vc), vc >= 0);
-    const BoxLane b = box_lane(io.tileslot, sh.pnb, k);
+    const BoxLane b = box_lane(io, sh.pnb, k);
     f.bl = b;
 #pragma unroll
     for (int i = 0; i < 12; i++) f.bx[i] = 0.0;
diff --git a/hpmpc_amd/csrc/hpmpc_capi.cpp b/hpmpc_amd/csrc/hpmpc_capi.cpp
--- a/hpmpc_amd/csrc/hpmpc_capi.cpp
+++ b/hpmpc_amd/csrc/hpmpc_capi.cpp
@@ -160,6 +160,12 @@
                                   ? 1
                                   : 0;
     }
+    {
+        const char* e = getenv("HPMPC_MI355X_BOX_PACK");
+        const BoxPack bp = box_pack(N, nb, ng, e && e[0] == '0');
+        P->HB = bp.HB;
+        P->SB = bp.SB;
+    }
     for (int k = 0; k <= N; k++) {
         P->st[k].oB = k < N ? (int)P->offB[k] : 0;
         P->st[k].oR = (int)P->offR[k];
@@ -219,6 +225,8 @@
     a.ngt = P->ngt;
     a.sG = P->packG;
     a.dbg = g_dbg_buf;
+    a.HB = P->HB;
+    a.SB = P->SB;
     return a;
 }
 
diff --git a/hpmpc_amd/csrc/hpmpc_kargs.h b/hpmpc_amd/csrc/hpmpc_kargs.h
--- a/hpmpc_amd/csrc/hpmpc_kargs.h
+++ b/hpmpc_amd/csrc/hpmpc_kargs.h
@@ -3,6 +3,10 @@
 constexpr int FSTRIDE = 352;
 constexpr int V16 = 16;
 constexpr int V32 = 32;
+
+constexpr long long ws_carve_doubles(int N) {
+    return ((long long)(N + 1) * (FSTRIDE + 9 * V16 + 8 * V32 + 1) + 16 + 31) / 32 * 32;
+}
 
 enum HkLaunch {
     K_SV = 0,
@@ -64,4 +68,5 @@
     int qpar;
     int* dctr;
     int* qnext;
+    int HB, SB;
 };
diff --git a/hpmpc_amd/csrc/hpmpc_kernels.hip b/hpmpc_amd/csrc/hpmpc_kernels.hip
--- a/hpmpc_amd/csrc/hpmpc_kernels.hip
+++ b/hpmpc_amd/csrc/hpmpc_kernels.hip
@@ -103,8 +103,8 @@
     const bool have = residual_pass<false, FX>(io, bc, ro, mu);
     if (a.res_plain) {
         wsync();
-        HK_FOR_BOX(io, k, { ro.rd[up] = -ro.rd[up]; });
-        HK_FOR_GEN(io, k, { ro.rd[up] = -ro.rd[up]; });
+        HK_FOR_BOX(io, io.lay, k, { ro.rd[up] = -ro.rd[up]; });
+        HK_FOR_GEN(io, io.lay, k, { ro.rd[up] = -ro.rd[up]; });
         if (lane_id() == 0) a.mu_out[p] = have ? mu : 0.0;
         return;
     }
@@ -220,8 +220,13 @@
         }
         wsync();
         IpmView v = view();
-        if (!update_body<FX, 4>(a, v)) break;
-    }
+        if (!update_body<FX, 4, false>(a, v)) break;
+    }
+    wsync();
+    IpmView v = view();
+    double *lam, *t;
+    caller_lam_t(a, v.q, lam, t);
+    publish_pass<4>(v.io, v.w.lam, v.w.t, lam, t, 0);
 }
 
 namespace {
@@ -475,19 +480,20 @@
     const double* rC = a.d + o32;
     const int l = lane_id();
     BoxCtx bc = box_ctx(w, rC, lam, t);
-    HK_FOR_BOX(io, k, { w.qx[k * V16 + slot] = -w.lamt[up] * rC[up] - w.lamt[lo] * rC[lo]; });
-    HK_FOR_GEN(io, k, { w.qx[s16] = -w.lamt[up] * rC[up] - w.lamt[lo] * rC[lo]; });
+    const BoxLay wy{a.SB, a.HB};
+    HK_FOR_BOX(io, wy, k, { w.qx[k * V16 + slot] = -w.lamt[wup] * rC[up] - w.lamt[wlo] * rC[lo]; });
+    HK_FOR_GEN(io, wy, k, { w.qx[s16] = -w.lamt[wup] * rC[up] - w.lamt[wlo] * rC[lo]; });
     wsync();
     double al = 1.0;
     ric_trs<BX_GIVEN, BX_NONE, FX>(io, &sm, a.vb + o16, a.vq + o16, bc, ux, a.compute_mult, pi, 1, w.Pb, al);
     wsync();
-    HK_FOR_BOX(io, k, {
+    HK_FOR_BOX(io, wy, k, {
         const double x = ux[k * V16 + bt.slotvar[k * 16 + slot]];
         const double tl = x - rC[lo], tu = -x + rC[up];
         t[lo] = tl;
         t[up] = tu;
-        lam[lo] = -w.lamt[lo] * tl;
-        lam[up] = -w.lamt[up] * tu;
+        lam[lo] = -w.lamt[wlo] * tl;
+        lam[up] = -w.lamt[wup] * tu;
     });
     if (a.ngt) {
         const int c = l & 15;
@@ -502,14 +508,14 @@
 #pragma unroll
             for (int lc = 0; lc < 4; lc++) {
                 if (4 * lc >= sh.ng) continue;
-                const GenLane q = gen_lane(k, sh.pnb, sh.ng, lc);
+                const GenLane q = gen_lane(io.lay, k, sh, lc), qw = gen_lane(wy, k, sh, lc);
                 const bool st = q.ok && c == 0;
                 const double dx = row_sum16(dg[lc] * x);
                 const double tl = dx - gld(rC, q.lo, q.ok), tu = -dx + gld(rC, q.up, q.ok);
                 gst(t, q.lo, tl, st);
                 gst(t, q.up, tu, st);
-                gst(lam, q.lo, -gld(w.lamt, q.lo, q.ok) * tl, st);
-                gst(lam, q.up, -gld(w.lamt, q.up, q.ok) * tu, st);
+                gst(lam, q.lo, -gld(w.lamt, qw.lo, q.ok) * tl, st);
+                gst(lam, q.up, -gld(w.lamt, qw.up, q.ok) * tu, st);
             }
         }
     }
```

New measurement: 2.248 million (median of 6 runs). +5.0%, better.
